# speedinghzl/DSRG

Hardware: AMD Instinct MI355X
Metric: images/sec DSRG train step (VGG16 321x321, 21-class) (higher is better)
Workload: dtype bf16 backbone (fp32 master weights) + f32/f64 supervision path

## Files before the change

### dsrg_amd/_lib.py

```python
import ctypes
import os

import torch

_HERE = os.path.dirname(os.path.abspath(__file__))
LIB_PATH = os.path.join(_HERE, os.environ.get("DSRG_LIB") or "libdsrg_hip.so")

OK, ERR_INVALID, ERR_HIP, ERR_UNSUPPORTED, ERR_NOMEM = 0, -1, -2, -3, -4


class DsrgError(RuntimeError):
    def __init__(self, code, msg):
        RuntimeError.__init__(self, "libdsrg_hip error %d: %s" % (code, msg))
        self.code = code


class CrfParams(ctypes.Structure):
    _fields_ = [("w_bilateral", ctypes.c_float), ("theta_alpha_x", ctypes.c_float),
                ("theta_alpha_y", ctypes.c_float), ("theta_beta_r", ctypes.c_float),
                ("theta_beta_g", ctypes.c_float), ("theta_beta_b", ctypes.c_float),
                ("w_gaussian", ctypes.c_float), ("theta_gamma_x", ctypes.c_float),
                ("theta_gamma_y", ctypes.c_float), ("n_iters", ctypes.c_int32)]

    @classmethod
# ... 58 lines not shown
    "dsrg_train_s_input_batch": (_i, [_i, _vp, _sz] + [ctypes.POINTER(ctypes.c_int32)] * 8 + [_i, _i, _i, _i, ctypes.POINTER(_f),
                                      _vp, _vp, _vp, _vp]),
    "dsrg_train_f_input_batch": (_i, [_i, _vp, _sz] + [ctypes.POINTER(ctypes.c_int32)] * 7 + [_i, _i, ctypes.POINTER(_f), _f, _f,
                                      _vp, _vp, _vp]),
    "dsrg_resnet_stem_packed_bytes": (_sz, []),
    "dsrg_pack_resnet_stem_f32": (_i, [_vp, _vp, _vp, _vp]),
    "dsrg_resnet_stem_bf16": (_i, [_vp, _vp, _vp, _vp, _i, _i, _i, _vp]),
    "dsrg_im2col3x3_nhwc16": (_i, [_vp, _vp, _i, _i, _i, _i, _i, _vp]),
    "dsrg_relu_bwd_bias_bf16": (_i, [_vp, _vp, _vp, _vp, _vp, _i, ctypes.c_long, _i, ctypes.c_float, _vp]),
    "dsrg_col2im3x3_nhwc_bf16": (_i, [_vp, _vp, _i, _i, _i, _i, _i, _vp]),
    "dsrg_avgpool3x3_s1_bf16": (_i, [_vp, _vp, _i, _i, _i, _i, _vp]),
    "dsrg_conv_igemm_backward_residual_bf16": (_i, [_vp] * 8 + [_i, _vp, _sz] + [_i] * 6 + [_vp]),
    "dsrg_pack_conv_weight_scaled_f32": (_i, [_vp, _vp, _vp, _vp, _i, _i, _i, _vp]),
    "dsrg_aspp_shift_sum_f32": (_i, [_vp, _vp, _vp, _vp] + [_i] * 6 + [_vp]),
    "dsrg_aspp_shift_gather_bf16": (_i, [_vp, _vp, _vp] + [_i] * 6 + [_vp]),
    "dsrg_defer_reductions": (_i, [_i]),
    "dsrg_flush_reductions": (_i, [_vp]),
    "dsrg_conv_igemm_residual_bf16": (_i, [_vp] * 6 + [_i] * 8 + [_vp]),
    "dsrg_conv_igemm_split_f32": (_i, [_vp, _vp, _vp, _vp] + [_i] * 8 + [_vp]),
    "dsrg_add_relu_bf16": (_i, [_vp, _vp, _vp, _sz, _vp]),
    "dsrg_relu_mask_bf16": (_i, [_vp, _vp, _vp, _vp, _sz, _vp]),
    "dsrg_bias_grad_bf16": (_i, [_vp, _vp, _vp, _i, ctypes.c_long, _i, _vp]),
    "dsrg_heads_forward_bf16": (_i, [_vp, _i, _vp, _vp, _vp, _i, _i, _i, _i, _vp]),
    "dsrg_conv3x3_direct_bf16": (_i, [_vp, _vp, _vp, _vp, _i, _i, _i, _i, _i, _i, _vp]),
    "dsrg_conv3x3_direct_dgrad_workspace": (_sz, [_i]),
    "dsrg_conv3x3_direct_dgrad_bf16": (_i, [_vp] * 6 + [_sz] + [_i] * 5 + [_vp]),
    "dsrg_conv_igemm_supported": (_i, [_i, _i, _i]),
    "dsrg_conv_igemm_bf16": (_i, [_vp, _vp, _vp, _vp, _vp, _i, _i, _i, _i, _i, _i, _i, _i, ctypes.c_float, ctypes.c_ulonglong, _vp, _sz,
                                  _vp]),
    "dsrg_conv_igemm_workspace": (_sz, []),
    "dsrg_conv_igemm_dgrad_workspace": (_sz, [_i] * 5),
    "dsrg_conv_igemm_dgrad_bf16": (_i, [_vp] * 6 + [_i] * 7 + [_f, _vp, _sz, _vp]),
    "dsrg_conv_igemm_workspace_status": (_i, [_vp, _vp, _vp]),
    "dsrg_pack_conv_weight_f32": (_i, [_vp, _vp, _vp, _i, _i, _i, _vp]),
    "dsrg_sgd_pack_f32": (_i, [_i] + [_vp] * 9 + [_f, _vp]),
    "dsrg_conv_igemm_wgrad_workspace": (_sz, [_i, _i, _i, _i, _i, _i, _i]),
    "dsrg_conv_igemm_wgrad_splits": (_i, [_i] * 7 + [_vp, _vp]),
    "dsrg_conv_igemm_wgrad_bf16": (_i, [_vp, _vp, _vp, _vp, _i, _vp, _sz, _i, _i, _i, _i, _i, _i, _i, _vp]),
    "dsrg_conv_igemm_backward_bf16": (_i, [_vp, _vp, _vp, _vp, _vp, _vp, _i, _vp, _f, _vp, ctypes.c_size_t, _vp, ctypes.c_size_t, _i, _i, _i, _i, _i, _i, _vp]),
    "dsrg_conv3x3_wgrad_workspace": (_sz, [_i, _i, _i, _i, _i]),
    "dsrg_conv3x3_wgrad_bf16": (_i, [_vp, _vp, _vp, _vp, _sz, _i, _i, _i, _i, _i, _vp]),
    "dsrg_conv3x3_wgrad_f32": (_i, [_vp, _vp, _vp, _vp, _sz, _i, _i, _i, _i, _i, _vp]),
    "dsrg_pack_conv_weight_direct_f32": (_i, [_vp, _vp, _vp, _i, _i, _vp]),
    "dsrg_heads_backward_chunks": (_i, [_i]),
    "dsrg_heads_backward_bf16": (_i, [_vp, _i, _vp, _vp, _vp, _sz, _vp, _vp, _i, _i, _i, _i, _vp]),
    "dsrg_heads_backward_relu_workspace": (_sz, [_i] * 3),
    "dsrg_heads_backward_relu_bf16": (_i, [_vp, _i, _vp, _vp, _vp, _sz, _vp, _vp, _f, _vp, _vp, _sz] + [_i] * 4 + [_vp]),
    "dsrg_maxpool3x3_fwd_bf16": (_i, [_vp, _vp, _vp, _i, _i, _i, _i, _i, _i, _i, _vp]),
    "dsrg_maxpool3x3_relu_fwd_bf16": (_i, [_vp, _vp, _vp, _i, _i, _i, _i, _i, _i, _i, _vp]),
    "dsrg_maxpool3x3_bwd_bf16": (_i, [_vp, _vp, _vp, _i, _i, _i, _i, _i, _i, _i, _vp]),
    "dsrg_maxpool3x3_bwd_relu_bf16": (_i, [_vp, _vp, _vp, _vp, _vp, _vp, _i, _i, _i, _i, _i, _i, _i, _vp]),
    "dsrg_supervision_step": (_i, [_vp, _i, _vp, _vp, _i, _i, _vp, _vp, _d, _d, ctypes.POINTER(CrfParams),
                                   _vp, _vp, _vp, _vp, _vp, _vp]),
}

_LIB = None


def lib():
    global _LIB
    if _LIB is None:
        if not os.path.exists(LIB_PATH):
            raise ImportError(
                "%s is missing — build it with `make -C dsrg_amd/csrc` (hipcc --offload-arch=gfx950) or "
                "`python -c 'import __graft_entry__ as g; g.build()'`.  There is no CPU fallback." % LIB_PATH)
        L = ctypes.CDLL(LIB_PATH)
        for name, (res, args) in SIGNATURES.items():
            fn = getattr(L, name)
            fn.restype = res
            fn.argtypes = args
        _LIB = L
    return _LIB


def check(rc):
    if rc != OK:
        raise DsrgError(rc, lib().dsrg_last_error().decode("utf-8", "replace"))


def require_gpu():
    if lib().dsrg_device_count() < 1:
        raise DsrgError(ERR_HIP, "no HIP device visible — the DSRG supervision kernels need an MI355X "
                                 "(gfx950); there is no CPU fallback")
```

### dsrg_amd/backbone.py

```python
import torch
import torch.nn as nn
import torch.nn.functional as F

import os as _os

from . import ops

_WGRAD_MIN_COUT = 512
_GEMM_DGRAD_MAX_MAP = 2048
_GEMM_WGRAD_MAX_MAP = 2048
_IGEMM_MIN_TILES = 64
_IGEMM = _os.environ.get("DSRG_IGEMM", "1") == "1"


def _bf16_run(x):
    return x.dtype == torch.bfloat16 or (torch.is_autocast_enabled() and torch.get_autocast_dtype("cuda") == torch.bfloat16)


def _im2col_gemm(x, weight, bias, dilation, relu, want_cols=False):
    B, C, H, W = x.shape
    cout, k = weight.shape[0], weight.shape[2]
    xn = x.permute(0, 2, 3, 1)
    if not xn.is_contiguous():
        xn = xn.contiguous()
# ... 112 lines not shown
            gw = torch.mm(g2d.t(), x2d).view(cout, x.shape[1], 1, 1)
            gemm_wgrad = True
        elif ctx.direct and g.dtype == torch.bfloat16 and x.dtype == torch.bfloat16 and \
                (x.shape[1], cout) in ((3, 64), (64, 64), (64, 128), (128, 128)):
            gw = ops.conv3x3_wgrad(x, g)
            gemm_wgrad = True
        elif gemm_wgrad:
            cin = x.shape[1]
            if cols is None or cols.dtype != g.dtype:
                cols = ops.im2col3x3_nhwc(x.permute(0, 2, 3, 1).contiguous(), ctx.dilation)
            g2d = g.permute(0, 2, 3, 1).reshape(-1, cout)
            gw = torch.mm(g2d.t(), cols).view(cout, 3, 3, cin).permute(0, 3, 1, 2)
        mask = [ctx.needs_input_grad[0] and not gemm_dgrad, not gemm_wgrad, not fused]
        gx2 = gw2 = gb2 = None
        if any(mask):
            gx2, gw2, gb2 = torch.ops.aten.convolution_backward(
                g, x, weight, None if fused else [weight.shape[0]], [1, 1], [pad, pad],
                [ctx.dilation, ctx.dilation], False, [0, 0], 1, mask)
        return (gx if gemm_dgrad else gx2), (gw if gemm_wgrad else gw2), (gb if fused else gb2), None, None, None, None, None, None, None


class _GradLink:
    __slots__ = ("scale", "gb", "ptr", "version")

    def __init__(self):
        self.scale, self.gb, self.ptr, self.version = 1.0, None, 0, -1

    def leave(self, gx, gb):
        self.gb, self.ptr, self.version = gb, gx.data_ptr(), gx._version

    def take(self, g):
        gb, self.gb = self.gb, None
        if gb is None:
            return None
        if g.data_ptr() == self.ptr and g._version == self.version:
            return gb
        if self.scale != 1.0:
            raise RuntimeError("chain_input: the output of a conv + ReLU + Dropout node declared to have one consumer has several")
        return None


_FUSE_CHAIN = _os.environ.get("DSRG_FUSE_CHAIN", "1") != "0"


def _landed(g, slot):
    return g.detach() if (slot is not None and g is slot) else g


class _IgemmConvFn(torch.autograd.Function):

    @staticmethod
    def forward(ctx, k, dils, relu, drop_p, pool, n, links_in, links_out, *t):
        xs, ws, bs = t[:n], t[n:2 * n], t[2 * n:3 * n]
        xs = [x if x.dtype == torch.bfloat16 else x.bfloat16() for x in xs]
        packs_d = [None] * n
        fb = [b.detach().float().contiguous() for b in bs]
        if drop_p > 0.0 and not relu:
            raise ValueError("_IgemmConvFn: Dropout needs the ReLU in front of it")
        fused_drop = drop_p > 0.0
        scale = 256.0 / (256 - min(255, int(drop_p * 256.0 + 0.5))) if fused_drop else 1.0
        seed = ops.dropout_seed() if fused_drop else 0
        if links_in is not None and not all(lk is not None for lk in links_in):
            links_in = None
        if k == 3:
            need_d = any(ctx.needs_input_grad[8:8 + n]) and ops.conv_igemm_supported(ws[0].shape[0], ws[0].shape[1], 3)
            packs = [ops.pack_conv_weight_pair(w, True, need_d) for w in ws]
            packs_d = [p[1] for p in packs]
            outs = ops.conv_igemm(xs, [p[0] for p in packs], fb, dils, 3, relu, drop_p, seed)
        elif fused_drop:
            packs = [ops.pack_conv_weight_pair(w, True, links_in is not None and _FUSE_CHAIN) for w in ws]
            packs_d = [p[1] for p in packs]
            outs = ops.conv_igemm(xs, [p[0] for p in packs], fb, dils, 1, relu, drop_p, seed)
        else:
            outs = [_im2col_gemm(x, w.to(torch.bfloat16), b.to(torch.bfloat16), 1, relu) for x, w, b in zip(xs, ws, bs)]
        code, pooled = None, None
        if pool is not None:
            pooled, code = ops.maxpool3x3_fwd(outs[0], pool[0], pool[1], relu_input=True)
        ctx.save_for_backward(code, *xs, *ws, *(outs if (relu and pool is None) else ()))
        ctx.out_shape = tuple(outs[0].shape)
        ctx.gw_out = [getattr(w, "_dsrg_grad_out", None) for w in ws]
        ctx.packs_d = packs_d
        ctx.dils, ctx.relu, ctx.scale, ctx.pool, ctx.n, ctx.k = dils, relu, scale, pool, n, k
        ctx.links_in = links_in
        ctx.links_out = links_out if (relu and pool is None) else None
        if ctx.links_out is not None:
            for lk in ctx.links_out:
                lk.scale, lk.gb = scale, None
        return tuple(outs) if pool is None else (pooled,)

    @staticmethod
    def backward(ctx, *gs):
        n = ctx.n
        code, saved = ctx.saved_tensors[0], ctx.saved_tensors[1:]
        xs, ws, ys = saved[:n], saved[n:2 * n], saved[2 * n:] or (None,) * n
        cout, cin = ws[0].shape[0], ws[0].shape[1]
        gms, gbs = [], []
        cl = torch.channels_last
        for i, g in enumerate(gs):
            gm, gb = g, ctx.links_out[i].take(g) if ctx.links_out is not None else None
            if gb is None:
                gm, gb = _relu_bias_backward(g, ctx.pool, code, ctx.out_shape, ctx.relu, ys[i], ctx.scale)
            gms.append(gm); gbs.append(gb)
        need_x = [ctx.needs_input_grad[8 + i] for i in range(n)]
        gxs = [None] * n
        absorb = _FUSE_CHAIN and ctx.links_in is not None and all(need_x) and ops.conv_igemm_supported(cout, cin, ctx.k) and \
            cin >= 256 and all(x.is_contiguous(memory_format=cl) for x in xs)
        if n == 1 and ctx.k == 3 and need_x[0] and ops.conv_igemm_supported(cout, cin, 3) and \
                ops.conv_igemm_wgrad_supported(cin, cout, 3) and xs[0].is_contiguous(memory_format=cl):
            pd = ctx.packs_d[0] if ctx.packs_d[0] is not None else ops.pack_conv_weight(ws[0], for_dgrad=True)
            gx, gw, gb_below = ops.conv_igemm_backward(gms[0], pd, xs[0], ctx.dils[0], xs[0] if absorb else None,
                                                       ctx.links_in[0].scale if absorb else 1.0, gw_out=ctx.gw_out[0])
            if absorb:
                ctx.links_in[0].leave(gx, gb_below)
            return (None,) * 8 + (gx, _landed(gw, ctx.gw_out[0])) + tuple(gbs)
        if absorb:
            packs_d = [p if p is not None else ops.pack_conv_weight(w, for_dgrad=True) for p, w in zip(ctx.packs_d, ws)]
            gxs, gb_below = ops.conv_igemm_dgrad(gms, packs_d, list(xs), ctx.dils, ctx.k, ctx.links_in[0].scale)
            for lk, gx_, gb_ in zip(ctx.links_in, gxs, gb_below):
                lk.leave(gx_, gb_)
        if ctx.k == 1:
            for i in range(n):
                if absorb:
                    break
                if need_x[i]:
                    g2d = gms[i].permute(0, 2, 3, 1).reshape(-1, cout)
                    B_, _, H_, W_ = xs[i].shape
                    gxs[i] = torch.mm(g2d, ws[i].to(torch.bfloat16).reshape(cout, cin)).view(B_, H_, W_, cin).permute(0, 3, 1, 2)
            gws = [_landed(gw, o) for gw, o in zip(ops.conv_igemm_wgrad(list(xs), gms, ctx.dils, 1, outs=ctx.gw_out), ctx.gw_out)]
            return (None,) * 8 + tuple(gxs) + tuple(gws) + tuple(gbs)
        if any(need_x) and not absorb:
            if ops.conv_igemm_supported(cout, cin, 3):
                packs_d = [p if p is not None else ops.pack_conv_weight(w, for_dgrad=True) for p, w in zip(ctx.packs_d, ws)]
                gxs = ops.conv_igemm(gms, packs_d, None, ctx.dils, 3, False)
            else:
                for i in range(n):
                    d = ctx.dils[i]
                    gxs[i] = torch.ops.aten.convolution_backward(gms[i], xs[i], ws[i].to(torch.bfloat16), None, [1, 1], [d, d], [d, d],
                                                                 False, [0, 0], 1, [True, False, False])[0]
        if ops.conv_igemm_wgrad_supported(cin, cout, 3):
            gws = ops.conv_igemm_wgrad(list(xs), gms, ctx.dils, 3, outs=ctx.gw_out)
            gws = [_landed(gw, o) for gw, o in zip(gws, ctx.gw_out)]
        else:
            gws = []
            for i in range(n):
                d = ctx.dils[i]
                gws.append(torch.ops.aten.convolution_backward(gms[i], xs[i], ws[i].to(torch.bfloat16), None, [1, 1], [d, d], [d, d],
                                                               False, [0, 0], 1, [False, True, False])[1].float())
        return (None,) * 8 + tuple(gx if nx else None for gx, nx in zip(gxs, need_x)) + tuple(gws) + tuple(gbs)


class _DirectConvFn(torch.autograd.Function):

    @staticmethod
    def forward(ctx, x, weight, bias, relu, pool, link_in, link_out):
        x = x if x.dtype == torch.bfloat16 else x.bfloat16()
        cl = torch.channels_last
        x = x if x.is_contiguous(memory_format=cl) else x.contiguous(memory_format=cl)
        if weight.shape[1] == 3:
            w16, wd = weight.detach().to(torch.bfloat16), None
        else:
            w16, wd = ops.pack_direct_weight_pair(weight, ctx.needs_input_grad[0])
        out = ops.conv3x3_direct(x, w16, bias.detach(), relu)
        code, pooled = None, None
        if pool is not None:
            pooled, code = ops.maxpool3x3_fwd(out, pool[0], pool[1], relu_input=True)
        ctx.save_for_backward(x, out if (relu and pool is None) else None, code)
        ctx.out_shape = tuple(out.shape)
        ctx.wd = wd
        ctx.gw_out = getattr(weight, "_dsrg_grad_out", None)
        ctx.relu, ctx.pool = relu, pool
        ctx.link_in = link_in if (link_in is not None and link_in.scale == 1.0 and wd is not None) else None
        ctx.link_out = link_out if (relu and pool is None) else None
        if ctx.link_out is not None:
            ctx.link_out.scale, ctx.link_out.gb = 1.0, None
        return out if pool is None else pooled

    @staticmethod
    def backward(ctx, g):
        x, y, code = ctx.saved_tensors
        gb = ctx.link_out.take(g) if ctx.link_out is not None else None
        if gb is None:
            g, gb = _relu_bias_backward(g, ctx.pool, code, ctx.out_shape, ctx.relu, y, 1.0)
        gx = None
        if ctx.needs_input_grad[0]:
            if _FUSE_CHAIN and ctx.link_in is not None:
                gx, gb_below = ops.conv3x3_direct_dgrad(g, ctx.wd, x)
                ctx.link_in.leave(gx, gb_below)
            else:
                gx = ops.conv3x3_direct(g, ctx.wd, None, False)
        gw = ops.conv3x3_wgrad(x, g, torch.float32, out=ctx.gw_out)
        return gx, _landed(gw, ctx.gw_out), gb, None, None, None, None


def _pool_in_node(cout):
    return cout % 8 == 0 and 256 % (cout // 8) == 0


def _direct_route(conv, x, p, pool):
    cin, cout = conv.in_channels, conv.out_channels
    if not (conv.kernel_size == (3, 3) and conv.dilation == (1, 1) and conv.groups == 1 and conv.bias is not None
            and (cin, cout) in ops.WGRAD_CONV_SHAPES and p == 0.0):
        return False
    if not _bf16_run(x):
        return False
    w = conv.weight
    if not (w.dtype == torch.float32 and conv.bias.dtype == torch.float32 and w.is_contiguous(memory_format=torch.channels_last)):
        return False
    if cin == 3 and x.requires_grad and torch.is_grad_enabled():
        return False
    return pool is None or _pool_in_node(cout)


# ... 100 lines not shown
        if _hip_pool_takes(x):
            return _AvgPool3x3Fn.apply(x)
        if x.is_cuda and x.dim() == 4 and not x.is_contiguous():
            x = x.contiguous()
        return super().forward(x)


class MaxPool3x3(nn.MaxPool2d):

    def __init__(self, stride, ceil_mode=False):
        super().__init__(3, stride, 1, ceil_mode=ceil_mode)

    def forward(self, x):
        return _pool3x3(x, self.stride, self.ceil_mode)


def _pool3x3(x, stride, ceil_mode):
    if _hip_pool_takes(x):
        return _MaxPool3x3Fn.apply(x, stride, ceil_mode)
    return F.max_pool2d(x, 3, stride, 1, ceil_mode=ceil_mode)


def _conv_relu(cin, cout, dilation=1, gemm=False, pool=None, chain=False):
    conv = GemmConv2d(cin, cout, 3, padding=dilation, dilation=dilation, fuse_relu=True, gemm=gemm, fuse_pool=pool, chain_input=chain)
    return [conv, FusedReLU()] + ([FusedPool()] if pool is not None else [])


class _HeadsFn(torch.autograd.Function):

    @staticmethod
    def forward(ctx, links, weight, bias, *xs):
        cl = torch.channels_last
        ctx.links = links if (links is not None and all(lk is not None for lk in links) and
                              all(x.is_contiguous(memory_format=cl) for x in xs)) else None
        xs = [x.contiguous(memory_format=cl) for x in xs]
        weight = weight.contiguous()
        ctx.save_for_backward(weight, *xs)
        return ops.heads_forward(xs, weight, bias.contiguous())

    @staticmethod
    def backward(ctx, g):
        weight, *xs = ctx.saved_tensors
        n, O, K = weight.shape
        if _FUSE_CHAIN and ctx.links is not None and all(ctx.needs_input_grad[3:]):
            gxs, gw, gb_below = ops.heads_backward(xs, weight, g, True, ctx.links[0].scale)
            for i, lk in enumerate(ctx.links):
                lk.leave(gxs[i], gb_below[i])
        else:
            gxs, gw = ops.heads_backward(xs, weight, g, need_gx=any(ctx.needs_input_grad[3:]))
        gb1 = g.sum((0, 2, 3))
        return (None, gw, gb1.unsqueeze(0).expand(n, O).contiguous()) + (tuple(gxs) if gxs is not None else (None,) * n)


class _StackKernels(torch.autograd.Function):

    @staticmethod
    def forward(ctx, *ws):
        ctx.layouts = [(tuple(w.shape), tuple(w.stride())) for w in ws]
        return torch.stack([w.reshape(w.shape[0], w.shape[1]) for w in ws])

    @staticmethod
    def backward(ctx, g):
        return tuple(g[i].as_strided(shape, stride) if g[i].is_contiguous() else g[i].reshape(shape)
                     for i, (shape, stride) in enumerate(ctx.layouts))


class VGG16ASPP(nn.Module):

    def __init__(self, num_classes=21, dropout=0.5, gemm_convs=True):
        super().__init__()
        L = []
        p2 = (2, True)
        L += _conv_relu(3, 64) + _conv_relu(64, 64, pool=p2, chain=True)
        L += _conv_relu(64, 128, 1, gemm_convs) + _conv_relu(128, 128, 1, gemm_convs, pool=p2, chain=True)
        L += _conv_relu(128, 256, 1, gemm_convs) + _conv_relu(256, 256, 1, gemm_convs, chain=True) + \
            _conv_relu(256, 256, 1, gemm_convs, pool=p2, chain=True)
        g = gemm_convs
        L += _conv_relu(256, 512, 1, g) + _conv_relu(512, 512, 1, g, chain=True) + _conv_relu(512, 512, 1, g, chain=True) + [MaxPool3x3(1)]
        L += _conv_relu(512, 512, 2, g) + _conv_relu(512, 512, 2, g, chain=True) + _conv_relu(512, 512, 2, g, chain=True) + [MaxPool3x3(1)]
        L += [AvgPool3x3()]
        self.features = nn.Sequential(*L)
        self.branches = nn.ModuleList()
        for d in (6, 12, 18, 24):
            g = gemm_convs
            fc8 = GemmConv2d(1024, num_classes, 1, gemm=g)
            nn.init.normal_(fc8.weight, std=0.01)
            nn.init.zeros_(fc8.bias)
            self.branches.append(nn.Sequential(
                GemmConv2d(512, 1024, 3, padding=d, dilation=d, fuse_relu=True, gemm=g, fuse_dropout=dropout), FusedReLU(),
                FusedDropout(),
                GemmConv2d(1024, 1024, 1, fuse_relu=True, gemm=g, fuse_dropout=dropout), FusedReLU(), FusedDropout(), fc8))

    def forward(self, x):
        f = self.features(x)
        hs = []
        fc6 = [br[0] for br in self.branches]
        if len(fc6) <= 4 and all(_igemm_route(m, f, len(fc6)) and m.stride == (1, 1) and m.padding == m.dilation for m in fc6):
            p = fc6[0].fuse_dropout if self.training else 0.0
            n = len(fc6)
            links = [_GradLink() for _ in range(n)] if torch.is_grad_enabled() else None
            hs = list(_IgemmConvFn.apply(3, [m.dilation[0] for m in fc6], True, p, None, n, None, links, *([f] * n),
                                         *[m.weight for m in fc6], *[m.bias for m in fc6]))
            fc7 = [br[3] for br in self.branches]
            if all(isinstance(m, GemmConv2d) and m.kernel_size == (1, 1) and m.fuse_relu and m.bias is not None and m.gemm
                   and m.in_channels % 256 == 0 and m.out_channels % 256 == 0 for m in fc7):
                p7 = fc7[0].fuse_dropout if self.training else 0.0
                links7 = [_GradLink() for _ in range(n)] if torch.is_grad_enabled() else None
                hs = list(_IgemmConvFn.apply(1, [1] * n, True, p7, None, n, links, links7, *hs, *[m.weight for m in fc7],
                                             *[m.bias for m in fc7]))
                for h, lk in zip(hs, links7 or []):
                    h._dsrg_grad_link = lk
            else:
                for i, br in enumerate(self.branches):
                    for m in list(br)[1:-1]:
                        hs[i] = m(hs[i])
        else:
            for br in self.branches:
                h = f
                for m in list(br)[:-1]:
                    h = m(h)
                hs.append(h)
        heads = [br[-1] for br in self.branches]
        if hs[0].is_cuda and hs[0].dtype == torch.bfloat16 and len(hs) <= 4 and heads[0].out_channels <= 32 \
                and heads[0].in_channels % 256 == 0:
            w = _StackKernels.apply(*[m.weight for m in heads])
            b = torch.stack([m.bias for m in heads])
            links = [getattr(h, "_dsrg_grad_link", None) for h in hs]
            return _HeadsFn.apply(links, w.float(), b.float(), *hs)
        out = None
        with torch.autocast(device_type=hs[0].device.type, enabled=False):
            for m, h in zip(heads, hs):
                s = m(h.float())
                out = s if out is None else out + s
        return out

    def caffe_param_groups(self):
        groups = {}
        for name, p in self.named_parameters():
            is_fc8 = name.startswith("branches") and name.split(".")[2] == "6"
            is_bias = name.endswith("bias")
            key = ((10.0 if is_fc8 else 1.0) * (2.0 if is_bias else 1.0), 0.0 if is_bias else 1.0)
            groups.setdefault(key, []).append(p)
        return [dict(params=ps, lr_mult=k[0], decay_mult=k[1]) for k, ps in groups.items()]


def count_flops_per_image(size=321):
    def pool(n): return -(-(n + 2 - 3) // 2) + 1
    h1 = size; h2 = pool(h1); h3 = pool(h2); h4 = pool(h3)
    macs = 0
    for (cin, cout, h, n) in [(3, 64, h1, 1), (64, 64, h1, 1), (64, 128, h2, 1), (128, 128, h2, 1),
                              (128, 256, h3, 1), (256, 256, h3, 2), (256, 512, h4, 1), (512, 512, h4, 5)]:
        macs += n * cin * cout * 9 * h * h
    macs += 4 * (512 * 1024 * 9 + 1024 * 1024 + 1024 * 21) * h4 * h4
    return 2 * macs


class GraphedForward(object):

    def __init__(self, net, example, amp_dtype=torch.bfloat16, warmup=3, capture_error_mode="global"):
        if net.training:
            raise ValueError("GraphedForward captures an eval-mode forward (dropout would replay one mask)")
        self.net, self.amp = net, amp_dtype
        self.x = example.detach().clone(memory_format=torch.preserve_format)
        warm = torch.cuda.Stream(device=example.device)
        warm.wait_stream(torch.cuda.current_stream())
        with torch.cuda.stream(warm):
            for _ in range(warmup):
                self._fwd()
        torch.cuda.current_stream().wait_stream(warm)
        torch.cuda.synchronize()
        self.graph = torch.cuda.CUDAGraph()
        with torch.cuda.graph(self.graph, capture_error_mode=capture_error_mode):
            self.out = self._fwd()

    def _fwd(self):
        with torch.no_grad(), torch.autocast("cuda", dtype=self.amp, enabled=self.amp is not None):
            return self.net(self.x).contiguous()

    def __call__(self, x=None):
        if x is not None and x.data_ptr() != self.x.data_ptr():
# ... 4 lines not shown
```

### dsrg_amd/csrc/api.hip

```cpp
#include <math.h>
#include <stdarg.h>
#include <stdio.h>
#include <string.h>
#include <mutex>
#include <new>
#include "common.h"

namespace dsrg {

static thread_local char g_err[512] = "";
int set_error(int code, const char *fmt, ...) {
    va_list ap;
    va_start(ap, fmt);
    vsnprintf(g_err, sizeof(g_err), fmt, ap);
    va_end(ap);
    return code;
}

static inline size_t align256(size_t x) { return (x + 255) & ~(size_t)255; }

}

using namespace dsrg;

// ... 522 lines not shown
    return launch_bias_grad(g, bias_grad, partials, partial_blocks, rows, C, static_cast<hipStream_t>(stream));
}
extern "C" int dsrg_heads_forward_bf16(const void *const *x_dev, int n_branches, const float *w_dev, const float *bias_dev,
                                       float *out_dev, int B, int HW, int K, int O, void *stream) {
    if (!x_dev || !w_dev || !out_dev || B < 1 || HW < 1) return set_error(DSRG_ERR_INVALID, "bad argument");
    for (int k = 0; k < n_branches && k < 4; k++)
        if (!x_dev[k]) return set_error(DSRG_ERR_INVALID, "NULL branch input");
    return launch_heads_fwd(x_dev, n_branches, w_dev, bias_dev, out_dev, B, HW, K, O, static_cast<hipStream_t>(stream));
}
extern "C" int dsrg_conv3x3_direct_bf16(const void *x_dev, const void *w_dev, const float *bias_dev, void *y_dev, int B, int H,
                                        int W, int cin, int cout, int relu, void *stream) {
    if (!x_dev || !w_dev || !y_dev || B < 1 || H < 1 || W < 1) return set_error(DSRG_ERR_INVALID, "bad argument");
    return launch_conv3x3_direct(x_dev, w_dev, bias_dev, y_dev, B, H, W, cin, cout, relu, static_cast<hipStream_t>(stream));
}
extern "C" size_t dsrg_conv3x3_direct_dgrad_workspace(int cout) { return conv3x3_direct_colsum_workspace(cout); }
extern "C" int dsrg_conv3x3_direct_dgrad_bf16(const void *g_dev, const void *w_dev, const void *mask_dev, void *gx_dev,
                                              float *bias_grad_dev, void *workspace_dev, size_t workspace_bytes, int B, int H, int W,
                                              int cin, int cout, void *stream) {
    if (!g_dev || !w_dev || !mask_dev || !gx_dev || !bias_grad_dev) return set_error(DSRG_ERR_INVALID, "NULL argument");
    return launch_conv3x3_direct(g_dev, w_dev, nullptr, gx_dev, B, H, W, cin, cout, 0, static_cast<hipStream_t>(stream), mask_dev,
                                 bias_grad_dev, workspace_dev, workspace_bytes);
}
extern "C" int dsrg_conv_igemm_supported(int cin, int cout, int ksize) { return conv_igemm_supported(cin, cout, ksize) ? 1 : 0; }
extern "C" int dsrg_conv_igemm_bf16(const void *const *x_dev, const void *const *w_dev, const float *const *bias_dev,
                                    void *const *y_dev, const int *dilation, int ngroups, int B, int H, int W, int cin, int cout,
                                    int ksize, int relu, float dropout_p, unsigned long long dropout_seed, void *workspace_dev,
                                    size_t workspace_bytes, void *stream) {
    if (!x_dev || !w_dev || !y_dev || B < 1 || H < 1 || W < 1) return set_error(DSRG_ERR_INVALID, "conv_igemm: bad arguments");
    return launch_conv_igemm(x_dev, w_dev, bias_dev, y_dev, dilation, ngroups, B, H, W, cin, cout, ksize, relu, dropout_p,
                             dropout_seed, workspace_dev, workspace_bytes, static_cast<hipStream_t>(stream));
}
extern "C" size_t dsrg_conv_igemm_dgrad_workspace(int ngroups, int B, int H, int W, int cout) {
    return conv_igemm_colsum_workspace(ngroups, B, H, W, cout);
}
extern "C" int dsrg_conv_igemm_dgrad_bf16(const void *const *g_dev, const void *const *w_dev, const void *const *mask_dev,
                                          void *const *gx_dev, float *const *bias_grad_dev, const int *dilation, int ngroups, int B,
                                          int H, int W, int cin, int cout, int ksize, float mask_scale, void *workspace_dev,
                                          size_t workspace_bytes, void *stream) {
    if (!g_dev || !w_dev || !gx_dev || !mask_dev || B < 1 || H < 1 || W < 1)
        return set_error(DSRG_ERR_INVALID, "conv_igemm_dgrad: bad arguments");
    return launch_conv_igemm(g_dev, w_dev, nullptr, gx_dev, dilation, ngroups, B, H, W, cin, cout, ksize, 0, 0.0f, 0ull, nullptr, 0,
                             static_cast<hipStream_t>(stream), mask_dev, mask_scale, bias_grad_dev, workspace_dev, workspace_bytes);
}
extern "C" size_t dsrg_conv_igemm_workspace(void) { return conv_igemm_workspace(); }
extern "C" int dsrg_conv_igemm_workspace_status(const void *workspace_dev, void *stream, int *status_host) {
    if (!workspace_dev || !status_host) return set_error(DSRG_ERR_INVALID, "bad argument");
    return conv_igemm_workspace_status(workspace_dev, static_cast<hipStream_t>(stream), status_host);
}
extern "C" int dsrg_pack_conv_weight_f32(const float *w_dev, void *fwd_dev, void *dgrad_dev, int cout, int cin, int ksize, void *stream) {
    return launch_pack_conv_weight(w_dev, fwd_dev, dgrad_dev, cout, cin, ksize, static_cast<hipStream_t>(stream));
}
namespace dsrg {
int launch_sgd_pack(int n, float *const *p, const float *const *g, float *const *buf, void *const *fwd, void *const *dg, const int *shape,
                    const long long *numel, const float *lr, const float *wd, float momentum, hipStream_t stream);
}
extern "C" int dsrg_sgd_pack_f32(int n, float *const *param_dev, const float *const *grad_dev, float *const *momentum_dev, void *const *fwd_dev,
                                 void *const *dgrad_dev, const int *shape, const long long *numel, const float *lr, const float *weight_decay,
                                 float momentum, void *stream) {
    if (n > 0 && (!param_dev || !numel || ((fwd_dev || dgrad_dev) && !shape)))
        return set_error(DSRG_ERR_INVALID, "sgd_pack: null argument");
    return launch_sgd_pack(n, param_dev, grad_dev, momentum_dev, fwd_dev, dgrad_dev, shape, numel, lr, weight_decay, momentum,
                           static_cast<hipStream_t>(stream));
}
extern "C" size_t dsrg_conv_igemm_wgrad_workspace(int ngroups, int B, int H, int W, int cin, int cout, int ksize) {
    return conv_igemm_wgrad_workspace(ngroups, B, H, W, cin, cout, ksize);
}
extern "C" int dsrg_conv_igemm_wgrad_splits(int ngroups, int B, int H, int W, int cin, int cout, int ksize, const int *dilation,
                                            int *splits_out) {
    return conv_igemm_wgrad_splits(ngroups, B, H, W, cin, cout, ksize, dilation, splits_out);
}
extern "C" int dsrg_conv_igemm_wgrad_bf16(const void *const *x_dev, const void *const *g_dev, void *const *gw_dev, const int *dilation,
                                          int ngroups, void *workspace_dev, size_t workspace_bytes, int B, int H, int W, int cin,
                                          int cout, int ksize, int out_bf16, void *stream) {
    if (!x_dev || !g_dev || !gw_dev || B < 1 || H < 1 || W < 1) return set_error(DSRG_ERR_INVALID, "conv_igemm_wgrad: bad arguments");
    return launch_conv_igemm_wgrad(x_dev, g_dev, gw_dev, dilation, ngroups, workspace_dev, workspace_bytes, B, H, W, cin, cout, ksize,
                                   out_bf16, static_cast<hipStream_t>(stream));
}
namespace dsrg {
int launch_conv_igemm_backward(const void *g, const void *wd, const void *x, const void *mask, void *gx, void *gw, int dil, float *bias_grad,
                               float mask_scale, void *colsum_ws, size_t colsum_ws_bytes, void *wgrad_ws, size_t wgrad_ws_bytes, int B, int H,
                               int W, int cin, int cout, int k, hipStream_t stream);
}
extern "C" int dsrg_conv_igemm_backward_bf16(const void *g_dev, const void *w_dgrad_dev, const void *x_dev, const void *mask_dev, void *gx_dev,
                                             float *gw_dev, int dilation, float *bias_grad_dev, float mask_scale, void *colsum_workspace_dev,
                                             size_t colsum_workspace_bytes, void *wgrad_workspace_dev, size_t wgrad_workspace_bytes, int B,
                                             int H, int W, int cin, int cout, int ksize, void *stream) {
    if (!g_dev || !w_dgrad_dev || !x_dev || !gx_dev || !gw_dev || B < 1 || H < 1 || W < 1 || (bias_grad_dev && !mask_dev))
        return set_error(DSRG_ERR_INVALID, "conv_igemm_backward: bad arguments");
    return dsrg::launch_conv_igemm_backward(g_dev, w_dgrad_dev, x_dev, mask_dev, gx_dev, gw_dev, dilation, bias_grad_dev, mask_scale,
                                            colsum_workspace_dev, colsum_workspace_bytes, wgrad_workspace_dev, wgrad_workspace_bytes, B, H,
                                            W, cin, cout, ksize, static_cast<hipStream_t>(stream));
}
extern "C" int dsrg_conv_igemm_backward_residual_bf16(const void *g_dev, const void *w_dgrad_dev, const void *x_dev, const void *mask_dev,
                                                      const void *res_dev, void *gx_dev, float *gw_dev, const float *gw_scale_dev, int dilation,
                                                      void *wgrad_workspace_dev, size_t wgrad_workspace_bytes, int B, int H, int W, int cin,
                                                      int cout, int ksize, void *stream) {
    if (!g_dev || !w_dgrad_dev || !x_dev || !gx_dev || !gw_dev || B < 1 || H < 1 || W < 1)
        return set_error(DSRG_ERR_INVALID, "conv_igemm_backward_residual: bad arguments");
    return launch_conv_igemm_backward_residual(g_dev, w_dgrad_dev, x_dev, mask_dev, res_dev, gx_dev, gw_dev, gw_scale_dev, dilation,
                                               wgrad_workspace_dev, wgrad_workspace_bytes, B, H, W, cin, cout, ksize,
                                               static_cast<hipStream_t>(stream));
}
extern "C" int dsrg_pack_conv_weight_scaled_f32(const float *w_dev, const float *scale_dev, void *fwd_dev, void *dgrad_dev, int cout, int cin,
                                                int ksize, void *stream) {
    return launch_pack_conv_weight(w_dev, fwd_dev, dgrad_dev, cout, cin, ksize, static_cast<hipStream_t>(stream), 0, scale_dev);
}
extern "C" size_t dsrg_conv3x3_wgrad_workspace(int B, int H, int W, int cin, int cout) {
    return conv3x3_wgrad_workspace(B, H, W, cin, cout);
}
extern "C" int dsrg_conv3x3_wgrad_bf16(const void *x_dev, const void *g_dev, void *gw_dev, void *workspace_dev, size_t workspace_bytes,
                                       int B, int H, int W, int cin, int cout, void *stream) {
    if (!x_dev || !g_dev || !gw_dev || !workspace_dev) return set_error(DSRG_ERR_INVALID, "bad argument");
    return launch_conv3x3_wgrad(x_dev, g_dev, gw_dev, static_cast<float *>(workspace_dev), workspace_bytes, B, H, W, cin, cout,
                                static_cast<hipStream_t>(stream));
}
extern "C" int dsrg_conv3x3_wgrad_f32(const void *x_dev, const void *g_dev, float *gw_dev, void *workspace_dev, size_t workspace_bytes,
                                      int B, int H, int W, int cin, int cout, void *stream) {
    if (!x_dev || !g_dev || !gw_dev || !workspace_dev) return set_error(DSRG_ERR_INVALID, "bad argument");
    return launch_conv3x3_wgrad(x_dev, g_dev, gw_dev, static_cast<float *>(workspace_dev), workspace_bytes, B, H, W, cin, cout,
                                static_cast<hipStream_t>(stream), 1);
}
extern "C" int dsrg_pack_conv_weight_direct_f32(const float *w_dev, void *fwd_dev, void *dgrad_dev, int cout, int cin, void *stream) {
    if ((cin != 64 && cin != 128) || (cout != 64 && cout != 128))
        return set_error(DSRG_ERR_INVALID, "pack_conv_weight_direct: 64 / 128 channels either side (got %d -> %d)", cin, cout);
    return launch_pack_conv_weight(w_dev, fwd_dev, dgrad_dev, cout, cin, 3, static_cast<hipStream_t>(stream), 1);
}
extern "C" int dsrg_heads_backward_chunks(int M) { return heads_bwd_chunks(M); }
extern "C" int dsrg_heads_backward_bf16(const void *const *x_dev, int n_branches, const float *w_dev, const float *g_dev,
                                        void *gx_dev, size_t gx_branch_stride_bytes, float *gw_dev, float *partial_dev, int B,
                                        int HW, int K, int O, void *stream) {
    if (!x_dev || !w_dev || !g_dev || (!gx_dev && !gw_dev) || (gw_dev && !partial_dev) || B < 1 || HW < 1)
        return set_error(DSRG_ERR_INVALID, "bad argument");
    for (int k = 0; k < n_branches && k < 4; k++)
        if (!x_dev[k]) return set_error(DSRG_ERR_INVALID, "NULL branch input");
    return launch_heads_bwd(x_dev, n_branches, w_dev, g_dev, gx_dev, gx_branch_stride_bytes, gw_dev, partial_dev, B, HW, K, O,
                            static_cast<hipStream_t>(stream));
}
extern "C" size_t dsrg_heads_backward_relu_workspace(int n_branches, int M, int K) { return heads_bwd_relu_workspace(n_branches, M, K); }
extern "C" int dsrg_heads_backward_relu_bf16(const void *const *x_dev, int n_branches, const float *w_dev, const float *g_dev,
                                             void *gx_dev, size_t gx_branch_stride_bytes, float *gw_dev, float *partial_dev,
                                             float relu_scale, float *bias_grad_dev, void *workspace_dev, size_t workspace_bytes,
                                             int B, int HW, int K, int O, void *stream) {
    if (!x_dev || !w_dev || !g_dev || !gx_dev || (gw_dev && !partial_dev) || B < 1 || HW < 1 || !(relu_scale > 0.0f) || !bias_grad_dev)
        return set_error(DSRG_ERR_INVALID, "bad argument");
    for (int k = 0; k < n_branches && k < 4; k++)
        if (!x_dev[k]) return set_error(DSRG_ERR_INVALID, "NULL branch input");
    return launch_heads_bwd(x_dev, n_branches, w_dev, g_dev, gx_dev, gx_branch_stride_bytes, gw_dev, partial_dev, B, HW, K, O,
                            static_cast<hipStream_t>(stream), relu_scale, bias_grad_dev, workspace_dev, workspace_bytes);
}
extern "C" int dsrg_maxpool3x3_fwd_bf16(const void *in, void *out, void *code, int B, int H, int W, int OH, int OW, int C,
                                        int stride, void *stream) {
    if (!in || !out || !code) return set_error(DSRG_ERR_INVALID, "NULL argument");
    return launch_maxpool3x3_fwd(in, out, code, B, H, W, OH, OW, C, stride, static_cast<hipStream_t>(stream));
}
extern "C" int dsrg_maxpool3x3_relu_fwd_bf16(const void *in, void *out, void *code, int B, int H, int W, int OH, int OW, int C,
                                             int stride, void *stream) {
    if (!in || !out || !code) return set_error(DSRG_ERR_INVALID, "NULL argument");
    return launch_maxpool3x3_fwd(in, out, code, B, H, W, OH, OW, C, stride, static_cast<hipStream_t>(stream), true);
}
extern "C" int dsrg_maxpool3x3_bwd_bf16(const void *gout, const void *code, void *gin, int B, int H, int W, int OH, int OW,
                                        int C, int stride, void *stream) {
    if (!gout || !code || !gin) return set_error(DSRG_ERR_INVALID, "NULL argument");
    return launch_maxpool3x3_bwd(gout, code, gin, B, H, W, OH, OW, C, stride, static_cast<hipStream_t>(stream));
}

extern "C" int dsrg_maxpool3x3_bwd_relu_bf16(const void *gout, const void *code, const void *relu_out, void *gin, float *bias_grad,
                                             float *partials, int partial_blocks, int B, int H, int W, int OH, int OW, int C,
                                             void *stream) {
    if (!gout || !code || !gin || !bias_grad || !partials) return set_error(DSRG_ERR_INVALID, "NULL argument");
    return launch_maxpool3x3_bwd_relu(gout, code, relu_out, gin, bias_grad, partials, partial_blocks, B, H, W, OH, OW, C,
                                      static_cast<hipStream_t>(stream));
}

extern "C" int dsrg_supervision_step(dsrg_ctx_t c, int B, const float *logits, const float *images, int img_h,
                                     int img_w, const float *labels, const float *cues, double th1, double th2,
                                     const dsrg_crf_params *prm, float *losses, float *grad_logits,
                                     float *probs_out, float *seeds_out, float *logq_out, void *stream) {
    if (!c || !logits || !labels || !cues || !losses || !grad_logits)
        return set_error(DSRG_ERR_INVALID, "NULL argument");
    if (B < 1 || B > c->maxB) return set_error(DSRG_ERR_INVALID, "batch %d outside 1..%d", B, c->maxB);
    const bool prepared = images == nullptr;
    {
        int prc = check_params(prm);
        if (prc) return prc;
    }
    if (!prepared && (img_h < 1 || img_w < 1)) return set_error(DSRG_ERR_INVALID, "bad image size");
    if (prepared) {
        if (c->prepared_B != B || memcmp(&c->prepared_prm, prm, offsetof(dsrg_crf_params, n_iters)) != 0)
            return set_error(DSRG_ERR_INVALID, "images_dev is NULL but dsrg_crf_prepare_batch was not called "
                                               "for this batch size / these kernel parameters");
    }
    hipStream_t s = static_cast<hipStream_t>(stream);
    const int C = c->C, N = c->N;
    const size_t nb = sizeof(float) * (size_t)B * C * N;
    const bool q0 = prm->n_iters > 0;
    int rc = launch_softmax_fwd(B, C, N, logits, c->probs, s, kMinProb, q0 ? c->mf.q : nullptr);
    if (rc) return rc;
    rc = crf_run(c, B, c->probs, colours_float(c, images, img_h, img_w), prm, nullptr, c->refined, c->logq, s, prepared, q0);
    if (prepared) c->prepared_B = 0;
    if (rc) return rc;
    rc = launch_srg(B, C, c->H, c->W, labels, cues, c->refined, th1, th2, c->seeds, c->srg_code, s);
    if (rc) return rc;
    rc = launch_sup_loss_backward(B, C, N, logits, c->probs, c->seeds, c->logq, c->refined, c->stats, grad_logits,
                                  losses, s);
    if (rc) return rc;
    if (probs_out) DSRG_HIP_CHECK(hipMemcpyAsync(probs_out, c->probs, nb, hipMemcpyDeviceToDevice, s));
    if (seeds_out) DSRG_HIP_CHECK(hipMemcpyAsync(seeds_out, c->seeds, nb, hipMemcpyDeviceToDevice, s));
    if (logq_out) DSRG_HIP_CHECK(hipMemcpyAsync(logq_out, c->logq, nb, hipMemcpyDeviceToDevice, s));
    return DSRG_OK;
}

namespace dsrg {
struct LargeCrf;
int large_crf_create(int W, int H, int C, LargeCrf **out, int nimages);
void large_crf_destroy(LargeCrf *c);
int large_crf_set_unary(LargeCrf *c, const float *unary_host);
int large_crf_zero_unary(LargeCrf *c);
int large_crf_set_image(LargeCrf *c, const unsigned char *im_host);
int large_crf_infer(LargeCrf *c, const dsrg_crf_params *prm, int n_iters);
int large_crf_read_q(LargeCrf *c, float *out_host);
int large_crf_read_map(LargeCrf *c, int32_t *labels_host);
int large_crf_read_map_select(LargeCrf *c, const CrfSelArgs &sel, int32_t *labels_host);
int large_crf_lattice_size(LargeCrf *c, int k);
Profiler *large_crf_profiler(LargeCrf *c);
void large_crf_set_stream(LargeCrf *c, hipStream_t s, bool async);
}

struct dsrg_crf_s {
    int W, H, M;
    int nimg;
    bool forced_large;
    dsrg::LargeCrf *large;
    dsrg_ctx_t ctx;
    float *neg_unary;
    float *q;
    float *stage;
    unsigned char *im;
    int32_t *lab;
    bool have_unary, have_pairwise;
    dsrg_crf_params prm;
    hipStream_t stream;
    bool async;
};

static constexpr int kCrfCacheSlots = 4;
static dsrg_crf_s *g_crf_cache[kCrfCacheSlots] = {nullptr, nullptr, nullptr, nullptr};
static std::mutex g_crf_cache_mutex;

static int crf_create(int W, int H, int nlabels, int nimages, dsrg_crf_t *out);
extern "C" int dsrg_crf_create(int W, int H, int nlabels, dsrg_crf_t *out) { return crf_create(W, H, nlabels, 1, out); }
extern "C" int dsrg_crf_create_batch(int W, int H, int nlabels, int nimages, dsrg_crf_t *out) {
    if (nimages < 1) return set_error(DSRG_ERR_INVALID, "bad CRF batch");
    return crf_create(W, H, nlabels, nimages == 1 ? -1 : nimages, out);
}
static int crf_create(int W, int H, int nlabels, int nimages, dsrg_crf_t *out) {
    const bool force_large = nimages != 1;
    if (nimages < 0) nimages = 1;
// ... 192 lines not shown
```

### dsrg_amd/csrc/backbone_ops.hip

```cpp
#include "common.h"
#include <algorithm>
#include <cstring>

namespace dsrg {

__device__ __forceinline__ float bf16_lo(uint32_t w) { return __uint_as_float(w << 16); }
__device__ __forceinline__ float bf16_hi(uint32_t w) { return __uint_as_float(w & 0xffff0000u); }
__device__ __forceinline__ uint32_t f32_to_bf16_rne(float f) {
    uint32_t u = __float_as_uint(f);
    if ((u & 0x7fffffffu) > 0x7f800000u) return (u >> 16) | 0x40u;
    return (u + 0x7fffu + ((u >> 16) & 1u)) >> 16;
}
__device__ __forceinline__ uint32_t pack_bf16(float lo, float hi) { return f32_to_bf16_rne(lo) | (f32_to_bf16_rne(hi) << 16); }

constexpr int kRbThreads = 256;

__global__ __launch_bounds__(kRbThreads) void relu_bwd_bias_kernel(const uint4 *__restrict__ g, const uint4 *__restrict__ y,
                                                                    uint4 *__restrict__ gm, float *__restrict__ part,
                                                                    int rows, int C8, int rows_per_block, float scale) {
    __shared__ float red[kRbThreads][9];
    const int lanes_r = kRbThreads / C8;
    const int cg = threadIdx.x % C8, rl = threadIdx.x / C8;
    float acc[8] = {0.f, 0.f, 0.f, 0.f, 0.f, 0.f, 0.f, 0.f};
    if (rl < lanes_r) {
// ... 510 lines not shown
    DSRG_LAUNCH_CHECK();
    return DSRG_OK;
}

int launch_maxpool3x3_bwd_relu(const void *gout, const void *code, const void *y, void *gin, float *bias_grad, float *part,
                                int part_blocks, int B, int H, int W, int OH, int OW, int C, hipStream_t stream) {
    int rc = pool_check(B, H, W, OH, OW, C, 2);
    if (rc) return rc;
    const int C8 = C / 8;
    if (kRbThreads % C8 != 0) return set_error(DSRG_ERR_UNSUPPORTED, "maxpool3x3_bwd_relu: channels / 8 must divide %d", kRbThreads);
    if (part_blocks < 1) return set_error(DSRG_ERR_INVALID, "maxpool3x3_bwd_relu: no partial-sum blocks");
    const size_t total = (size_t)B * ((H + 1) / 2) * ((W + 1) / 2) * C8;
    size_t ipb = (total + part_blocks - 1) / part_blocks;
    ipb = (ipb + kRbThreads - 1) / kRbThreads * kRbThreads;
    const int nblk = (int)((total + ipb - 1) / ipb);
    if (y)
        hipLaunchKernelGGL(maxpool3x3_s2_bwd_relu_kernel<true>, dim3(nblk), dim3(kRbThreads), 0, stream, (const uint4 *)gout,
                           (const uint2 *)code, (const uint4 *)y, (uint4 *)gin, part, B, H, W, OH, OW, C8, ipb);
    else
        hipLaunchKernelGGL(maxpool3x3_s2_bwd_relu_kernel<false>, dim3(nblk), dim3(kRbThreads), 0, stream, (const uint4 *)gout,
                           (const uint2 *)code, (const uint4 *)nullptr, (uint4 *)gin, part, B, H, W, OH, OW, C8, ipb);
    DSRG_LAUNCH_CHECK();
    if (!defer_reduction(1, part, bias_grad, nblk, C))
        hipLaunchKernelGGL(bias_finalize_kernel, dim3((C + 31) / 32), dim3(256), 0, stream, part, bias_grad, nblk, C);
    DSRG_LAUNCH_CHECK();
    return DSRG_OK;
}

int launch_maxpool3x3_bwd(const void *gout, const void *code, void *gin, int B, int H, int W, int OH, int OW, int C,
                          int stride, hipStream_t stream) {
    int rc = pool_check(B, H, W, OH, OW, C, stride);
    if (rc) return rc;
    if (stride == 2) {
        const size_t blocks2 = (size_t)B * ((H + 1) / 2) * ((W + 1) / 2) * (C / 8);
        hipLaunchKernelGGL(maxpool3x3_s2_bwd_kernel, dim3((unsigned)((blocks2 + 255) / 256)), dim3(256), 0, stream,
                           (const uint4 *)gout, (const uint2 *)code, (uint4 *)gin, B, H, W, OH, OW, C / 8);
        DSRG_LAUNCH_CHECK();
        return DSRG_OK;
    }
    const size_t total = (size_t)B * H * W * (C / 8);
    hipLaunchKernelGGL(maxpool3x3_bwd_kernel, dim3((unsigned)((total + 255) / 256)), dim3(256), 0, stream, (const uint4 *)gout,
                       (const uint2 *)code, (uint4 *)gin, B, H, W, OH, OW, C / 8, stride);
    DSRG_LAUNCH_CHECK();
    return DSRG_OK;
}



namespace {
typedef float f32x16 __attribute__((ext_vector_type(16)));
constexpr int kHeadOutPad = 32;
struct HeadArgs {
    const uint16_t *x[4];
    const float *w;
    const float *bias;
    float *out;
    int nbr, M, K, O, HW;
};
__device__ __forceinline__ void bf16x8_to_f32(const uint4 &v, float (&f)[8]) {
    f[0] = bf16_lo(v.x); f[1] = bf16_hi(v.x); f[2] = bf16_lo(v.y); f[3] = bf16_hi(v.y);
    f[4] = bf16_lo(v.z); f[5] = bf16_hi(v.z); f[6] = bf16_lo(v.w); f[7] = bf16_hi(v.w);
}
}

struct HeadMask {
    const uint16_t *y[4];
    float *part;
    float scale;
    int tiles;
};
template <bool MASK>
__global__ __launch_bounds__(256) void heads_bwd_dx_kernel(const float *__restrict__ g, const float *__restrict__ w,
                                                           uint4 *__restrict__ gx, int M, int K, int O, int HW, size_t branch_stride,
                                                           HeadMask hm) {
    __shared__ __attribute__((aligned(16))) float gs[32][16];
    __shared__ __attribute__((aligned(16))) float cs_l[MASK ? 128 : 1][8];
    const int k = blockIdx.y, t = threadIdx.x;
    const int K8 = K / 8, T = MASK ? hm.tiles : 1;
    uint4 *dst = reinterpret_cast<uint4 *>(reinterpret_cast<unsigned char *>(gx) + (size_t)k * branch_stride);
    for (int cg0 = 0; cg0 < K8; cg0 += 128) {
        const int cg = cg0 + (t & 127), rh = t >> 7;
        const bool live = cg < K8;
        float cs[8] = {0, 0, 0, 0, 0, 0, 0, 0};
        for (int ti = 0; ti < T; ti++) {
            const int m0 = (blockIdx.x * T + ti) * 16;
            if (m0 >= M) break;
            if (MASK || cg0 > 0) __syncthreads();
            for (int e = t; e < 32 * 16; e += 256) {
                const int o = e >> 4, r = e & 15, m = m0 + r;
                float v = 0.0f;
                if (o < O && m < M) { const int b = m / HW, hw = m - b * HW; v = g[((size_t)b * O + o) * HW + hw]; }
                gs[o][r] = v;
            }
            __syncthreads();
            if (!live) continue;
            float acc[8][8];
#pragma unroll
            for (int r = 0; r < 8; r++)
#pragma unroll
                for (int c = 0; c < 8; c++) acc[r][c] = 0.0f;
            const float *wk = w + (size_t)k * O * K + (size_t)cg * 8;
#pragma unroll 7
            for (int o = 0; o < O; o++) {
                const float4 w0 = *reinterpret_cast<const float4 *>(wk + (size_t)o * K), w1 = *reinterpret_cast<const float4 *>(wk + (size_t)o * K + 4);
                const float4 g0 = *reinterpret_cast<const float4 *>(&gs[o][rh * 8]), g1 = *reinterpret_cast<const float4 *>(&gs[o][rh * 8 + 4]);
                const float wf[8] = {w0.x, w0.y, w0.z, w0.w, w1.x, w1.y, w1.z, w1.w};
                const float gf[8] = {g0.x, g0.y, g0.z, g0.w, g1.x, g1.y, g1.z, g1.w};
#pragma unroll
                for (int r = 0; r < 8; r++)
#pragma unroll
                    for (int c = 0; c < 8; c++) acc[r][c] = __builtin_fmaf(gf[r], wf[c], acc[r][c]);
            }
            uint4 yk[4];
#pragma unroll
            for (int r = 0; r < 8; r++) {
                const int m = m0 + rh * 8 + r;
                if (MASK && (r & 3) == 0) {
#pragma unroll
                    for (int r2 = 0; r2 < 4; r2++) {
                        const int m2 = m + r2;
                        yk[r2] = m2 < M ? *reinterpret_cast<const uint4 *>(hm.y[k] + (size_t)m2 * K + (size_t)cg * 8) : make_uint4(0, 0, 0, 0);
                    }
                }
                uint32_t o4[4];
#pragma unroll
                for (int e = 0; e < 4; e++) {
                    if (MASK) {
                        const uint4 yr = yk[r & 3];
                        const uint32_t y = e == 0 ? yr.x : e == 1 ? yr.y : e == 2 ? yr.z : yr.w;
                        const uint32_t keep = ((int16_t)(y & 0xffffu) > 0 ? 0x0000ffffu : 0u) | ((int32_t)y >= 0x10000 ? 0xffff0000u : 0u);
                        o4[e] = pack_bf16(acc[r][2 * e] * hm.scale, acc[r][2 * e + 1] * hm.scale) & keep;
                        cs[2 * e] += __uint_as_float(o4[e] << 16);
                        cs[2 * e + 1] += __uint_as_float(o4[e] & 0xffff0000u);
                    } else {
                        o4[e] = pack_bf16(acc[r][2 * e], acc[r][2 * e + 1]);
                    }
                }
                if (m < M) dst[(size_t)m * K8 + cg] = make_uint4(o4[0], o4[1], o4[2], o4[3]);
            }
        }
        if (MASK) {
            __syncthreads();
            if (rh == 1 && live) {
                *reinterpret_cast<float4 *>(&cs_l[t & 127][0]) = make_float4(cs[0], cs[1], cs[2], cs[3]);
                *reinterpret_cast<float4 *>(&cs_l[t & 127][4]) = make_float4(cs[4], cs[5], cs[6], cs[7]);
            }
            __syncthreads();
            if (rh == 0 && live) {
                float *p = hm.part + ((size_t)k * gridDim.x + blockIdx.x) * K + (size_t)cg * 8;
                const float4 a0 = *reinterpret_cast<const float4 *>(&cs_l[t][0]), a1 = *reinterpret_cast<const float4 *>(&cs_l[t][4]);
                *reinterpret_cast<float4 *>(p) = make_float4(cs[0] + a0.x, cs[1] + a0.y, cs[2] + a0.z, cs[3] + a0.w);
                *reinterpret_cast<float4 *>(p + 4) = make_float4(cs[4] + a1.x, cs[5] + a1.y, cs[6] + a1.z, cs[7] + a1.w);
            }
        }
    }
}

template <int O, bool MASK>
__global__ __launch_bounds__(256) void heads_bwd_dx_rows_kernel(const float *__restrict__ g, const float *__restrict__ w,
                                                                unsigned char *__restrict__ gx, int M, int K, int HW, size_t branch_stride,
                                                                HeadMask hm, int rows_per_wg) {
    constexpr int OP = (O + 3) & ~3;
    extern __shared__ __attribute__((aligned(16))) float gs_rows[];
    const int k = blockIdx.y, t = threadIdx.x;
    const int c = blockIdx.z * 1024 + 4 * t;
    const int r0 = blockIdx.x * rows_per_wg, r1 = min(M, r0 + rows_per_wg), nr = r1 - r0;
    for (int e = t; e < nr * OP; e += 256) {
        const int o = e / nr, r = e - o * nr, m = r0 + r;
        float v = 0.0f;
        if (o < O) { const int b = m / HW, hw = m - b * HW; v = g[((size_t)b * O + o) * HW + hw]; }
        gs_rows[r * OP + o] = v;
    }
    float wr[O][4];
#pragma unroll
    for (int o = 0; o < O; o++) {
        const float4 v = *reinterpret_cast<const float4 *>(w + ((size_t)k * O + o) * K + c);
        wr[o][0] = v.x; wr[o][1] = v.y; wr[o][2] = v.z; wr[o][3] = v.w;
    }
    __syncthreads();
    unsigned char *dst = gx + (size_t)k * branch_stride;
    const uint16_t *yk = MASK ? hm.y[k] : nullptr;
    float cs[4] = {0.0f, 0.0f, 0.0f, 0.0f};
    constexpr int R = 4;
    uint2 yn[R];
    auto fetch_masks = [&](int r) {
#pragma unroll
        for (int j = 0; j < R; j++) yn[j] = r + j < nr ? *reinterpret_cast<const uint2 *>(yk + (size_t)(r0 + r + j) * K + c) : make_uint2(0u, 0u);
    };
    if (MASK) fetch_masks(0);
    for (int r = 0; r < nr; r += R) {
        uint2 y[R];
        if (MASK) {
#pragma unroll
            for (int j = 0; j < R; j++) y[j] = yn[j];
            if (r + R < nr) fetch_masks(r + R);
        }
        float acc[R][4];
#pragma unroll
        for (int j = 0; j < R; j++) {
            const float *gr = gs_rows + min(r + j, nr - 1) * OP;
            float gv[OP];
#pragma unroll
            for (int q = 0; q < OP / 4; q++) {
                const float4 v = *reinterpret_cast<const float4 *>(gr + 4 * q);
                gv[4 * q] = v.x; gv[4 * q + 1] = v.y; gv[4 * q + 2] = v.z; gv[4 * q + 3] = v.w;
            }
#pragma unroll
            for (int e = 0; e < 4; e++) acc[j][e] = 0.0f;
#pragma unroll
            for (int o = 0; o < O; o++)
#pragma unroll
                for (int e = 0; e < 4; e++) acc[j][e] = __builtin_fmaf(gv[o], wr[o][e], acc[j][e]);
        }
#pragma unroll
        for (int j = 0; j < R; j++) {
            uint32_t o2[2];
#pragma unroll
            for (int e = 0; e < 2; e++) {
                if (MASK) {
                    const uint32_t yy = e == 0 ? y[j].x : y[j].y;
                    const uint32_t keep = ((int16_t)(yy & 0xffffu) > 0 ? 0x0000ffffu : 0u) | ((int32_t)yy >= 0x10000 ? 0xffff0000u : 0u);
                    o2[e] = pack_bf16(acc[j][2 * e] * hm.scale, acc[j][2 * e + 1] * hm.scale) & keep;
                    cs[2 * e] += __uint_as_float(o2[e] << 16);
                    cs[2 * e + 1] += __uint_as_float(o2[e] & 0xffff0000u);
                } else {
                    o2[e] = pack_bf16(acc[j][2 * e], acc[j][2 * e + 1]);
                }
            }
            if (r + j < nr) *reinterpret_cast<uint2 *>(dst + ((size_t)(r0 + r + j) * K + c) * 2) = make_uint2(o2[0], o2[1]);
// ... 19 lines not shown
        const int q = q0 + wave;
        const bool live = q < nq;
        const uint16_t *xq = a.x[k] + (size_t)(live ? q : 0) * 256 + j * 8;
        for (int mb = mbeg; mb < mend; mb += kDwRows) {
            __syncthreads();
            for (int e = threadIdx.x; e < kDwRows * 32; e += 256) {
                const int o = e / kDwRows, r = e % kDwRows, m = mb + r;
                float v = 0.0f;
                if (o < a.O && m < mend) { const int b = m / a.HW, hw = m - b * a.HW; v = g[((size_t)b * a.O + o) * a.HW + hw]; }
                gs[r][o] = v;
            }
            __syncthreads();
            if (live) {
                constexpr int G = 8;
                uint4 xv[G];
                auto fetch = [&](int r2base) {
#pragma unroll
                    for (int u = 0; u < G; u++) {
                        const int m = min(mb + r2base + 2 * u + half, mend - 1);
                        xv[u] = *reinterpret_cast<const uint4 *>(xq + (size_t)m * a.K);
                    }
                };
                fetch(0);
                for (int r2 = 0; r2 < kDwRows; r2 += 2 * G) {
                    float xf[G][8], gv[G];
#pragma unroll
                    for (int u = 0; u < G; u++) {
                        bf16x8_to_f32(xv[u], xf[u]);
                        gv[u] = gs[r2 + 2 * u + half][j];
                    }
                    if (r2 + 2 * G < kDwRows) fetch(r2 + 2 * G);
#pragma unroll
                    for (int u = 0; u < G; u++)
#pragma unroll
                        for (int t = 0; t < 8; t++) acc[t] = __builtin_amdgcn_mfma_f32_32x32x2f32(gv[u], xf[u][t], acc[t], 0, 0, 0);
                }
            }
        }
        float *pp = partial + (((size_t)rc * a.nbr + k) * a.O) * a.K + (size_t)(live ? q : 0) * 256 + j * 8;
#pragma unroll
        for (int r = 0; r < 16; r++) {
            const int o = (r & 3) + 8 * (r >> 2) + 4 * half;
            if (live && o < a.O) {
                *reinterpret_cast<float4 *>(pp + (size_t)o * a.K) = make_float4(acc[0][r], acc[1][r], acc[2][r], acc[3][r]);
                *reinterpret_cast<float4 *>(pp + (size_t)o * a.K + 4) = make_float4(acc[4][r], acc[5][r], acc[6][r], acc[7][r]);
            }
        }
#pragma unroll
        for (int t = 0; t < 8; t++)
#pragma unroll
            for (int r = 0; r < 16; r++) acc[t][r] = 0.0f;
    }
}
__global__ void heads_bwd_dw_reduce_kernel(const float *__restrict__ partial, float *__restrict__ gw, int nchunks, size_t n) {
    const size_t i = (size_t)blockIdx.x * blockDim.x + threadIdx.x;
    if (i >= n) return;
    float s = 0.0f;
    for (int c = 0; c < nchunks; c++) s += partial[(size_t)c * n + i];
    gw[i] = s;
}

namespace {
typedef __attribute__((ext_vector_type(8))) __bf16 hbf16x8;
typedef __attribute__((ext_vector_type(2))) __bf16 hbf16x2;
typedef __attribute__((ext_vector_type(2))) float hf32x2;
typedef __attribute__((__vector_size__(4 * sizeof(__bf16)))) __bf16 hbf16x4v;
#define DSRG_LDS_AS __attribute__((address_space(3)))
__device__ __forceinline__ uint32_t cvt_pk_bf16(float lo, float hi) {
    hf32x2 v = {lo, hi};
    hbf16x2 b = __builtin_convertvector(v, hbf16x2);
    return *reinterpret_cast<uint32_t *>(&b);
}
__device__ __forceinline__ void split3(const float (&f)[8], hbf16x8 &t0, hbf16x8 &t1, hbf16x8 &t2) {
    uint32_t p0[4], p1[4], p2[4];
#pragma unroll
    for (int i = 0; i < 4; i++) {
        float a = f[2 * i], b = f[2 * i + 1];
        p0[i] = cvt_pk_bf16(a, b);
        a -= bf16_lo(p0[i]); b -= bf16_hi(p0[i]);
        p1[i] = cvt_pk_bf16(a, b);
        a -= bf16_lo(p1[i]); b -= bf16_hi(p1[i]);
        p2[i] = cvt_pk_bf16(a, b);
    }
    uint4 q0 = make_uint4(p0[0], p0[1], p0[2], p0[3]), q1 = make_uint4(p1[0], p1[1], p1[2], p1[3]), q2 = make_uint4(p2[0], p2[1], p2[2], p2[3]);
    t0 = *reinterpret_cast<hbf16x8 *>(&q0); t1 = *reinterpret_cast<hbf16x8 *>(&q1); t2 = *reinterpret_cast<hbf16x8 *>(&q2);
}
__device__ __forceinline__ hbf16x8 tr_frag16(DSRG_LDS_AS unsigned char *p, int stride4) {
    hbf16x4v lo = __builtin_amdgcn_ds_read_tr16_b64_v4bf16(reinterpret_cast<DSRG_LDS_AS hbf16x4v *>(p));
    hbf16x4v hi = __builtin_amdgcn_ds_read_tr16_b64_v4bf16(reinterpret_cast<DSRG_LDS_AS hbf16x4v *>(p + stride4));
    return __builtin_shufflevector(lo, hi, 0, 1, 2, 3, 4, 5, 6, 7);
}
}

template <int R>
__global__ __launch_bounds__(256) void heads_fwd_split_kernel(HeadArgs a) {
    __shared__ float part[R][4][16][64];
    const int lane = threadIdx.x & 63, wave = threadIdx.x >> 6;
    const int m0 = blockIdx.x * (32 * R);
    const int row = lane & 31, half = lane >> 5;
    f32x16 acc[R][3];
#pragma unroll
    for (int t = 0; t < R; t++)
#pragma unroll
        for (int q = 0; q < 3; q++)
#pragma unroll
            for (int r = 0; r < 16; r++) acc[t][q][r] = 0.0f;
    if (wave < a.nbr) {
        const uint16_t *xp[R];
#pragma unroll
        for (int t = 0; t < R; t++) xp[t] = a.x[wave] + (size_t)min(m0 + 32 * t + row, a.M - 1) * a.K + half * 8;
        const float *wp = a.w + ((size_t)wave * a.O + min(row, a.O - 1)) * a.K + half * 8;
        constexpr int G = 4;
        uint4 xv[G][R];
        float4 wv[G][2];
#pragma unroll
        for (int u = 0; u < G; u++) {
#pragma unroll
            for (int t = 0; t < R; t++) xv[u][t] = *reinterpret_cast<const uint4 *>(xp[t] + u * 16);
            wv[u][0] = *reinterpret_cast<const float4 *>(wp + u * 16);
            wv[u][1] = *reinterpret_cast<const float4 *>(wp + u * 16 + 4);
        }
        for (int kb = 0; kb < a.K; kb += 16 * G) {
#pragma unroll
            for (int u = 0; u < G; u++) {
                hbf16x8 xa[R];
#pragma unroll
                for (int t = 0; t < R; t++) xa[t] = *reinterpret_cast<hbf16x8 *>(&xv[u][t]);
                const float wf[8] = {wv[u][0].x, wv[u][0].y, wv[u][0].z, wv[u][0].w, wv[u][1].x, wv[u][1].y, wv[u][1].z, wv[u][1].w};
                const int kn = kb + 16 * G + u * 16;
                if (kn < a.K) {
#pragma unroll
                    for (int t = 0; t < R; t++) xv[u][t] = *reinterpret_cast<const uint4 *>(xp[t] + kn);
                    wv[u][0] = *reinterpret_cast<const float4 *>(wp + kn);
                    wv[u][1] = *reinterpret_cast<const float4 *>(wp + kn + 4);
                }
                hbf16x8 w0, w1, w2;
                split3(wf, w0, w1, w2);
#pragma unroll
                for (int t = 0; t < R; t++) {
                    acc[t][0] = __builtin_amdgcn_mfma_f32_32x32x16_bf16(xa[t], w0, acc[t][0], 0, 0, 0);
                    acc[t][1] = __builtin_amdgcn_mfma_f32_32x32x16_bf16(xa[t], w1, acc[t][1], 0, 0, 0);
                    acc[t][2] = __builtin_amdgcn_mfma_f32_32x32x16_bf16(xa[t], w2, acc[t][2], 0, 0, 0);
                }
            }
        }
    }
#pragma unroll
    for (int t = 0; t < R; t++)
#pragma unroll
        for (int r = 0; r < 16; r++) part[t][wave][r][lane] = acc[t][0][r] + (acc[t][1][r] + acc[t][2][r]);
    __syncthreads();
    const int col = threadIdx.x >> 3, r4 = (threadIdx.x & 7) * 4;
    if (col < a.O) {
#pragma unroll
        for (int t = 0; t < R; t++)
#pragma unroll
            for (int q = 0; q < 4; q++) {
                const int rr = r4 + q, m = m0 + 32 * t + rr;
                if (m >= a.M) break;
                const int hf = (rr >> 2) & 1, reg = (rr & 3) + 4 * (rr >> 3), ln = col + 32 * hf;
                float s = 0.0f;
                for (int k = 0; k < a.nbr; k++) {
                    const float sk = part[t][k][reg][ln] + (a.bias ? a.bias[k * a.O + col] : 0.0f);
                    s = k == 0 ? sk : s + sk;
                }
                const int b = m / a.HW, hw = m - b * a.HW;
                a.out[((size_t)b * a.O + col) * a.HW + hw] = s;
            }
    }
}

constexpr int kDwRows2 = 32, kDwGPitch = 36;
__global__ __launch_bounds__(256, 2) void heads_bwd_dw_split_kernel(HeadArgs a, const float *__restrict__ g, float *__restrict__ partial,
                                                                 int rows_per_chunk) {
    extern __shared__ __attribute__((aligned(16))) unsigned char dw_lds[];
    const int xstride = a.K * 2 + 64, K8 = a.K / 8;
    unsigned char *xt = dw_lds;
    float *gs = reinterpret_cast<float *>(dw_lds + kDwRows2 * xstride);
    const int lane = threadIdx.x & 63, wave = threadIdx.x >> 6, k = blockIdx.y, rc = blockIdx.x;
    const int mbeg = rc * rows_per_chunk, mend = min(a.M, mbeg + rows_per_chunk);
    const int i16 = lane & 15, gq = lane >> 4;
    const int rowsel = (gq >> 1) * 8 + (i16 >> 2), colsel = (gq & 1) * 16 + 4 * (i16 & 3);
    const int nq = a.K / 256;
    const uint16_t *xk = a.x[k];
    for (int q0 = 0; q0 < nq; q0 += 4) {
        const int q = q0 + wave;
        const bool live = q < nq;
        f32x16 acc[8];
#pragma unroll
        for (int t = 0; t < 8; t++)
#pragma unroll
            for (int r = 0; r < 16; r++) acc[t][r] = 0.0f;
        DSRG_LDS_AS unsigned char *xb = (DSRG_LDS_AS unsigned char *)xt + rowsel * xstride + ((live ? q : 0) * 256 + colsel) * 2;
        for (int mb = mbeg; mb < mend; mb += kDwRows2) {
            __syncthreads();
            for (int e = threadIdx.x; e < kDwRows2 * 32; e += 256) {
                const int o = e / kDwRows2, r = e % kDwRows2, m = mb + r;
                float v = 0.0f;
                if (o < a.O && m < mend) { const int b = m / a.HW, hw = m - b * a.HW; v = g[((size_t)b * a.O + o) * a.HW + hw]; }
                gs[o * kDwGPitch + r] = v;
            }
#pragma unroll 8
            for (int v = threadIdx.x; v < kDwRows2 * K8; v += 256) {
                const int r = v / K8, cg = v - r * K8, m = min(mb + r, mend - 1);
                *reinterpret_cast<uint4 *>(xt + r * xstride + cg * 16) = *reinterpret_cast<const uint4 *>(xk + (size_t)m * a.K + cg * 8);
            }
            __syncthreads();
            if (live) {
#pragma unroll
                for (int s2 = 0; s2 < kDwRows2 / 16; s2++) {
                    const float *gp = gs + (lane & 31) * kDwGPitch + s2 * 16 + (lane >> 5) * 8;
                    const float4 g0 = *reinterpret_cast<const float4 *>(gp), g1 = *reinterpret_cast<const float4 *>(gp + 4);
                    const float gf[8] = {g0.x, g0.y, g0.z, g0.w, g1.x, g1.y, g1.z, g1.w};
                    hbf16x8 a0, a1, a2, bx[8];
                    split3(gf, a0, a1, a2);
#pragma unroll
                    for (int t = 0; t < 8; t++) bx[t] = tr_frag16(xb + s2 * 16 * xstride + t * 64, 4 * xstride);
#pragma unroll
                    for (int t = 0; t < 8; t++) acc[t] = __builtin_amdgcn_mfma_f32_32x32x16_bf16(a0, bx[t], acc[t], 0, 0, 0);
#pragma unroll
                    for (int t = 0; t < 8; t++) acc[t] = __builtin_amdgcn_mfma_f32_32x32x16_bf16(a1, bx[t], acc[t], 0, 0, 0);
#pragma unroll
                    for (int t = 0; t < 8; t++) acc[t] = __builtin_amdgcn_mfma_f32_32x32x16_bf16(a2, bx[t], acc[t], 0, 0, 0);
                }
            }
        }
        if (live) {
            float *pp = partial + (((size_t)rc * a.nbr + k) * a.O) * a.K + (size_t)q * 256 + (lane & 31);
#pragma unroll
            for (int t = 0; t < 8; t++)
#pragma unroll
                for (int r = 0; r < 16; r++) {
                    const int o = (r & 3) + 8 * (r >> 2) + 4 * (lane >> 5);
                    if (o < a.O) pp[(size_t)o * a.K + t * 32] = acc[t][r];
                }
        }
    }
}

static int heads_check(int nbr, int K, int O) {
    if (nbr < 1 || nbr > 4 || O < 1 || O > kHeadOutPad || K < 256 || K % 256 != 0)
        return set_error(DSRG_ERR_UNSUPPORTED, "heads: 1..4 branches, <= %d outputs, K a multiple of 256", kHeadOutPad);
    return DSRG_OK;
}

int launch_heads_fwd(const void *const *x, int nbr, const float *w, const float *bias, float *out, int B, int HW, int K, int O,
                     hipStream_t stream) {
    int rc = heads_check(nbr, K, O);
    if (rc) return rc;
    HeadArgs a;
    for (int k = 0; k < 4; k++) a.x[k] = static_cast<const uint16_t *>(x[k < nbr ? k : 0]);
    a.w = w; a.bias = bias; a.out = out; a.nbr = nbr; a.M = B * HW; a.K = K; a.O = O; a.HW = HW;
    hipLaunchKernelGGL(heads_fwd_split_kernel<2>, dim3((a.M + 63) / 64), dim3(256), 0, stream, a);
    DSRG_LAUNCH_CHECK();
    return DSRG_OK;
}

int heads_bwd_chunks(int M) { int c = (M + 255) / 256; return c < 1 ? 1 : (c > 128 ? 128 : c); }

constexpr int kHeadMaskTiles = 8;
constexpr int kHeadStripRows = 64;
static bool head_strips(int K, int O) { return O == 21 && K % 1024 == 0; }
size_t heads_bwd_relu_workspace(int nbr, int M, int K) {
    const size_t rows = std::max((size_t)((M + 16 * kHeadMaskTiles - 1) / (16 * kHeadMaskTiles)), (size_t)((M + kHeadStripRows - 1) / kHeadStripRows));
    return (size_t)nbr * rows * (size_t)K * sizeof(float);
}

int launch_heads_bwd(const void *const *x, int nbr, const float *w, const float *g, void *gx, size_t gx_branch_stride,
                     float *gw, float *partial, int B, int HW, int K, int O, hipStream_t stream, float relu_scale, float *bias_grad,
                     void *colsum_ws, size_t colsum_ws_bytes) {
    int rc = heads_check(nbr, K, O);
    if (rc) return rc;
    const int M = B * HW;
    if (gx && relu_scale > 0.0f) {
        HeadMask hm;
        for (int k = 0; k < 4; k++) hm.y[k] = static_cast<const uint16_t *>(x[k < nbr ? k : 0]);
        hm.tiles = kHeadMaskTiles; hm.scale = relu_scale;
        const int nblk = (M + 16 * kHeadMaskTiles - 1) / (16 * kHeadMaskTiles);
        if (!bias_grad || !colsum_ws || colsum_ws_bytes < heads_bwd_relu_workspace(nbr, M, K))
            return set_error(DSRG_ERR_INVALID, "heads backward: bias gradient / scratch of the absorbed ReLU missing or too small");
        hm.part = static_cast<float *>(colsum_ws);
        int nblk_s = nblk;
        if (head_strips(K, O)) {
            nblk_s = (M + kHeadStripRows - 1) / kHeadStripRows;
            hipLaunchKernelGGL((heads_bwd_dx_rows_kernel<21, true>), dim3(nblk_s, nbr, K / 1024), dim3(256),
                               (size_t)kHeadStripRows * 24 * sizeof(float), stream, g, w, static_cast<unsigned char *>(gx), M, K, HW,
                               gx_branch_stride, hm, kHeadStripRows);
        } else {
            hipLaunchKernelGGL(heads_bwd_dx_kernel<true>, dim3(nblk, nbr), dim3(256), 0, stream, g, w, static_cast<uint4 *>(gx), M, K, O, HW,
                               gx_branch_stride, hm);
        }
        DSRG_LAUNCH_CHECK();
        const float *parts[4];
        float *outs[4];
        for (int k = 0; k < nbr; k++) { parts[k] = hm.part + (size_t)k * nblk_s * K; outs[k] = bias_grad + (size_t)k * K; }
        if (int rc2 = launch_igemm_colsum(parts, outs, nbr, nblk_s, K, stream)) return rc2;
    } else if (gx) {
        HeadMask hm;
        memset(&hm, 0, sizeof(hm));
        if (head_strips(K, O))
            hipLaunchKernelGGL((heads_bwd_dx_rows_kernel<21, false>), dim3((M + kHeadStripRows - 1) / kHeadStripRows, nbr, K / 1024),
                               dim3(256), (size_t)kHeadStripRows * 24 * sizeof(float), stream, g, w, static_cast<unsigned char *>(gx), M, K, HW,
                               gx_branch_stride, hm, kHeadStripRows);
        else
            hipLaunchKernelGGL(heads_bwd_dx_kernel<false>, dim3((M + 15) / 16, nbr), dim3(256), 0, stream, g, w, static_cast<uint4 *>(gx), M,
                               K, O, HW, gx_branch_stride, hm);
        DSRG_LAUNCH_CHECK();
    }
    if (gw) {
        HeadArgs a;
        for (int k = 0; k < 4; k++) a.x[k] = static_cast<const uint16_t *>(x[k < nbr ? k : 0]);
        a.w = w; a.bias = nullptr; a.out = nullptr; a.nbr = nbr; a.M = M; a.K = K; a.O = O; a.HW = HW;
        const int nch = heads_bwd_chunks(M), rows = ((M + nch - 1) / nch + 1) & ~1;
        const size_t lds = (size_t)kDwRows2 * (K * 2 + 64) + 32 * kDwGPitch * sizeof(float);
        if (lds > 160 * 1024) {
            hipLaunchKernelGGL(heads_bwd_dw_kernel, dim3(nch, nbr), dim3(256), 0, stream, a, g, partial, rows);
        } else {
            static LdsGrant grant;
            if (int rc2 = ensure_dynamic_lds(reinterpret_cast<const void *>(&heads_bwd_dw_split_kernel), lds, grant)) return rc2;
            hipLaunchKernelGGL(heads_bwd_dw_split_kernel, dim3(nch, nbr), dim3(256), lds, stream, a, g, partial, rows);
        }
        DSRG_LAUNCH_CHECK();
        const size_t n = (size_t)nbr * O * K;
        hipLaunchKernelGGL(heads_bwd_dw_reduce_kernel, dim3((unsigned)((n + 255) / 256)), dim3(256), 0, stream, partial, gw, nch, n);
        DSRG_LAUNCH_CHECK();
    }
    return DSRG_OK;
}

}
```

### dsrg_amd/csrc/common.h

```cpp
#pragma once
#include <hip/hip_runtime.h>
#include <stdint.h>
#include <stddef.h>
#include <atomic>
#include "../../include/dsrg_hip.h"

namespace dsrg {

int set_error(int code, const char *fmt, ...);
#define DSRG_HIP_CHECK(expr)                                                              \
    do {                                                                                  \
        hipError_t _e = (expr);                                                           \
        if (_e != hipSuccess)                                                             \
            return ::dsrg::set_error(DSRG_ERR_HIP, "%s failed: %s (%s:%d)", #expr,        \
                                     hipGetErrorString(_e), __FILE__, __LINE__);          \
    } while (0)
#define DSRG_LAUNCH_CHECK() DSRG_HIP_CHECK(hipGetLastError())

__device__ __forceinline__ void colsum_block(const float *__restrict__ p, float *__restrict__ out, int rows, int cout, int bx, float (*red)[64]) {
    const int cl = threadIdx.x & 63, c = bx * 64 + cl, q = threadIdx.x >> 6;
    float s0 = 0.0f, s1 = 0.0f;
    int r = q;
    for (; r + 16 < rows; r += 32) {
        s0 += p[(size_t)r * cout + c];
// ... 118 lines not shown
    const unsigned char *im_u8 = nullptr;
    const float *images = nullptr;
    int Hi = 0, Wi = 0;
    unsigned char *im_out = nullptr;
};

struct LatticeFeat {
    float sx, sy, sr, sg, sb;
    float scale[5];
    int W, H;
};

size_t lattice_bytes(int d, int N, int nlat);
void lattice_carve(LatticeView &L, void *base, int d, int N, int nlat);
void lattice_feat_init(LatticeFeat &F, int d, int W, int H, float sx, float sy, float sr, float sg, float sb);

int launch_lattice_build(const LatticeView &L, const LatticeFeat &F, const LatticeColours &col, int nlat,
                         hipStream_t stream);
bool lattice_supported(int d, int N);

struct MeanfieldBufs {
    float *q;
    float *msg_g;
    float *msg_b;
};
constexpr int kLatticeLocal = 16;
struct Profiler {
    hipEvent_t *start, *stop;
    int cap, used;
    bool active;
};
int launch_meanfield(const LatticeView &Lg, const LatticeView &Lb, const MeanfieldBufs &buf, int B, int C,
                     const float *neg_unary, float wg, float wb, int n_iters, float *q_out,
                     double *refined_out, float *logq_out, bool gauss_local, hipStream_t stream, Profiler *prof = nullptr,
                     bool q0_ready = false);
int filter_plan_query(const LatticeView &Lg, const LatticeView &Lb, const MeanfieldBufs &buf, int B, int C, bool gauss_local,
                      int out[4]);
int launch_lattice_norm_pass(const LatticeView &L, int nlat, hipStream_t stream);
int launch_filter_once(const LatticeView &Lg, const LatticeView &Lb, const MeanfieldBufs &buf, int B, int C, int kind,
                       const float *q_in, float *out, bool gauss_local, hipStream_t stream);

int launch_clip_min(float *p, size_t n, hipStream_t stream);

int launch_softmax_fwd(int B, int C, int HW, const float *x, float *p, hipStream_t stream, float floor_at = 0.0f,
                       float *q0 = nullptr);
int launch_softmax_bwd(int B, int C, int HW, const float *x, const float *g, float *dx, hipStream_t stream);
int launch_crf_bwd(size_t n, const double *refined, const float *td, float *bd, hipStream_t stream);
int launch_seed_loss(int B, int C, int HW, const float *p, const float *S, float *loss, float *grad,
                     hipStream_t stream);
int launch_constrain_loss(int B, int C, int HW, const float *p, const float *lq, float *loss, float *gp,
                          float *glq, hipStream_t stream);
int launch_sup_loss_backward(int B, int C, int HW, const float *logits, const float *probs, const float *seeds,
                             const float *logq, const double *refined, double *stats, float *grad_logits,
                             float *losses, hipStream_t stream);
int launch_lf_to_planes(int N, int M, const float *in, float *out, int negate, hipStream_t stream);
int launch_planes_to_lf(int N, int M, const float *in, float *out, hipStream_t stream);
int launch_argmax_planes(int N, int M, const float *q, int32_t *lab, hipStream_t stream);
int launch_select_planes(int N, int M, const float *q, int32_t *lab, const CrfSelArgs &sel, hipStream_t stream);
int launch_train_gt_unary_batch(int G, int C, const float *scores, int h, int w, const int32_t *H, const int32_t *W, float eps,
                                const int32_t *select, const int32_t *nselect, int select_stride, float ignore_below,
                                float *workspace, float *const *unary, float *const *probs, int32_t *const *labels,
                                hipStream_t stream);
int launch_seed_loss_plain(int B, int C, int HW, const float *p, const float *S, float *loss, float *grad, hipStream_t stream);
int launch_expand_loss(int B, int C, int HW, const float *p, const float *stat, double q_fg, double q_bg, float *loss,
                       float *grad, double *terms, hipStream_t stream);
int launch_confusion(size_t n, const unsigned char *gt, const unsigned char *pred, int nclass, int rule_lt,
                     unsigned long long *hist, hipStream_t stream);
int launch_multiscale_unary(int K, int C, const float *const *scores, const int32_t *h, const int32_t *w, int H, int W, float eps,
                            float *unary, int32_t *amax, float *sum_out, hipStream_t stream);
int launch_multiscale_unary_batch(int G, int K, int C, const float *const *scores, const int32_t *h, const int32_t *w,
                                  const int32_t *H, const int32_t *W, float eps, float *const *unary, int32_t *const *amax,
                                  float *const *sum_out, hipStream_t stream);
int launch_preprocess_ms_batch(int G, int Gcap, int K, const unsigned char *const *images, const int32_t *H, const int32_t *W,
                               const int32_t *sizes, const float *mean, float *const *out, hipStream_t stream);
int launch_train_s_input_batch(int B, const unsigned char *stage, size_t stage_bytes, const int32_t *image_off, const int32_t *H,
                               const int32_t *W, const int32_t *cue_off, const int32_t *ncues, const int32_t *label_off,
                               const int32_t *nlabels, const int32_t *mirror, int S, int C, int Hm, int Wm, const float *mean,
                               float *images, float *cues, float *labels, hipStream_t stream);
int launch_train_f_input_batch(int B, const unsigned char *stage, size_t stage_bytes, const int32_t *image_off, const int32_t *label_off,
                               const int32_t *H, const int32_t *W, const int32_t *top, const int32_t *left, const int32_t *mirror,
                               int ch, int cw, const float *mean, float scale, float ignore_label, float *data, float *label,
                               hipStream_t stream);
size_t resnet_stem_packed_bytes();
int launch_pack_resnet_stem(const float *w, const float *scale, void *packed, hipStream_t stream);
int launch_resnet_stem(const float *x, const void *packed, const float *shift, void *y, int B, int H, int W, hipStream_t stream);
int launch_im2col3x3(const void *in, void *out, int B, int H, int W, int C, int dil, hipStream_t stream);
int launch_col2im3x3(const void *cols, void *out, int B, int H, int W, int C, int dil, hipStream_t stream);
int launch_relu_bwd_bias(const void *g, const void *y, void *gm, float *bias_grad, float *part, int part_blocks,
                         long rows, int C, float scale, hipStream_t stream);
int launch_avgpool3x3_s1(const void *in, void *out, int B, int H, int W, int C, hipStream_t stream);
int launch_bias_grad(const void *g, float *bias_grad, float *part, int part_blocks, long rows, int C, hipStream_t stream);
int launch_heads_fwd(const void *const *x, int nbr, const float *w, const float *bias, float *out, int B, int HW, int K, int O,
                     hipStream_t stream);
bool conv3x3_direct_supported(int cin, int cout);
size_t conv3x3_wgrad_workspace(int B, int H, int W, int cin, int cout);
int launch_conv3x3_wgrad(const void *x, const void *g, void *gw, float *workspace, size_t workspace_bytes, int B, int H, int W,
                         int cin, int cout, hipStream_t stream, int out_f32 = 0);
int launch_conv3x3_direct(const void *x, const void *w, const float *bias, void *y, int B, int H, int W, int cin, int cout,
                          int relu, hipStream_t stream, const void *mask = nullptr, float *colsum = nullptr,
                          void *colsum_ws = nullptr, size_t colsum_ws_bytes = 0);
size_t conv3x3_direct_colsum_workspace(int cout);
bool conv_igemm_supported(int cin, int cout, int k);
int launch_conv_igemm_residual(const void *x, const void *w, const float *bias, const void *res, const void *mask, void *y, int dil, int B,
                               int H, int W, int cin, int cout, int k, int relu, hipStream_t stream);
int launch_conv_igemm_split(const void *x3, const void *w, const float *bias, float *y, int dil, int B, int H, int W, int cin, int cout, int k,
                            int relu, hipStream_t stream);
int launch_conv_igemm(const void *const *x, const void *const *w, const float *const *bias, void *const *y, const int *dil,
                      int ngroups, int B, int H, int W, int cin, int cout, int k, int relu, float drop_p, unsigned long long seed,
                      void *workspace, size_t workspace_bytes, hipStream_t stream, const void *const *mask = nullptr,
                      float out_scale = 1.0f, float *const *colsum = nullptr, void *colsum_ws = nullptr, size_t colsum_ws_bytes = 0);
size_t conv_igemm_colsum_workspace(int ngroups, int B, int H, int W, int cout);
size_t conv_igemm_workspace();
int conv_igemm_workspace_status(const void *workspace, hipStream_t stream, int *status);
size_t conv_igemm_wgrad_workspace(int ngroups, int B, int H, int W, int cin, int cout, int k);
int conv_igemm_wgrad_splits(int ngroups, int B, int H, int W, int cin, int cout, int k, const int *dil, int *splits);
int launch_conv_igemm_wgrad(const void *const *x, const void *const *g, void *const *gw, const int *dil, int ngroups, void *workspace,
                            size_t workspace_bytes, int B, int H, int W, int cin, int cout, int k, int out_bf16, hipStream_t stream);
int launch_pack_conv_weight(const float *w, void *fwd, void *dgrad, int cout, int cin, int k, hipStream_t stream, int plain = 0,
                            const float *scale = nullptr);
int launch_conv_igemm_backward_residual(const void *g, const void *wd, const void *x, const void *mask, const void *res, void *gx, void *gw,
                                        const float *gw_scale, int dil, void *wgrad_ws, size_t wgrad_ws_bytes, int B, int H, int W, int cin,
                                        int cout, int k, hipStream_t stream);
int heads_bwd_chunks(int M);
int launch_heads_bwd(const void *const *x, int nbr, const float *w, const float *g, void *gx, size_t gx_branch_stride,
                     float *gw, float *partial, int B, int HW, int K, int O, hipStream_t stream, float relu_scale = 0.0f,
                     float *bias_grad = nullptr, void *colsum_ws = nullptr, size_t colsum_ws_bytes = 0);
size_t heads_bwd_relu_workspace(int nbr, int M, int K);
int launch_add_relu(const void *a, const void *b, void *y, size_t n, hipStream_t stream);
int launch_aspp_shift_sum(const void *yp, const float *bias, float *out, const int *offsets, int J, int O, int CT, int B, int H, int W,
                          hipStream_t stream);
int launch_aspp_shift_gather(const float *g, void *gp, const int *offsets, int J, int O, int CT, int B, int H, int W, hipStream_t stream);
int launch_relu_mask(const void *g, const void *g2, const void *y, void *gm, size_t n, hipStream_t stream);
int launch_igemm_colsum(const float *const *parts, float *const *outs, int ngroups, int rows, int cout, hipStream_t stream);
int launch_maxpool3x3_bwd_relu(const void *gout, const void *code, const void *y, void *gin, float *bias_grad, float *part,
                                int part_blocks, int B, int H, int W, int OH, int OW, int C, hipStream_t stream);
int launch_maxpool3x3_fwd(const void *in, void *out, void *code, int B, int H, int W, int OH, int OW, int C, int stride,
                          hipStream_t stream, bool relu_in = false);
int launch_maxpool3x3_bwd(const void *gout, const void *code, void *gin, int B, int H, int W, int OH, int OW, int C,
                          int stride, hipStream_t stream);

#ifdef __HIPCC__
__device__ __forceinline__ float exp_cr(float x) { return (float)exp((double)x); }

using rsrc_t = decltype(__builtin_amdgcn_make_buffer_rsrc((void *)nullptr, (short)0, 0, 0));
__device__ __forceinline__ rsrc_t make_rsrc(const void *p, size_t bytes) {
    const uint64_t a = reinterpret_cast<uint64_t>(p);
    const uint32_t lo = __builtin_amdgcn_readfirstlane((uint32_t)a);
    const uint32_t hi = __builtin_amdgcn_readfirstlane((uint32_t)(a >> 32));
    const uint32_t nb = __builtin_amdgcn_readfirstlane((uint32_t)bytes);
    void *q = reinterpret_cast<void *>(((uint64_t)hi << 32) | lo);
    return __builtin_amdgcn_make_buffer_rsrc(q, (short)0, (int)nb, 0x00020000);
}
__device__ __forceinline__ uint32_t ld_u32(rsrc_t r, uint32_t voff, uint32_t soff = 0) {
    return __builtin_amdgcn_raw_buffer_load_b32(r, voff, soff, 0);
}
__device__ __forceinline__ float ld_f32(rsrc_t r, uint32_t voff, uint32_t soff = 0) {
    return __uint_as_float(__builtin_amdgcn_raw_buffer_load_b32(r, voff, soff, 0));
}
__device__ __forceinline__ uint32_t ld_u16(rsrc_t r, uint32_t voff, uint32_t soff = 0) {
    return (uint32_t)__builtin_amdgcn_raw_buffer_load_b16(r, voff, soff, 0);
}
template <int U>
__device__ __forceinline__ void stage16_to_lds(unsigned char *dst, const void *src, uint32_t nbytes, int tid) {
    using v4 = decltype(__builtin_amdgcn_raw_buffer_load_b128(rsrc_t(), 0, 0, 0));
    const rsrc_t r = make_rsrc(src, nbytes);
    for (uint32_t base = 0; base < nbytes; base += 1024u * 16u * U) {
        v4 x[U];
#pragma unroll
        for (int u = 0; u < U; u++) x[u] = __builtin_amdgcn_raw_buffer_load_b128(r, (uint32_t)tid * 16u, base + (uint32_t)u * (1024u * 16u), 0);
#pragma unroll
        for (int u = 0; u < U; u++) {
            const uint32_t off = base + (uint32_t)u * (1024u * 16u) + (uint32_t)tid * 16u;
            if (off < nbytes) *reinterpret_cast<v4 *>(dst + off) = x[u];
        }
    }
}

#endif

int launch_srg(int B, int C, int H, int W, const float *labels, const float *cues, const double *refined,
// ... 4 lines not shown
```

### dsrg_amd/csrc/layers.hip

```cpp
#include <math.h>
#include "common.h"

namespace dsrg {

__global__ void clip_min_kernel(float *__restrict__ p, size_t n) {
    size_t i = (size_t)blockIdx.x * blockDim.x + threadIdx.x;
    const size_t stride = (size_t)gridDim.x * blockDim.x;
    for (; i < n; i += stride) {
        const float v = p[i];
        if (v < kMinProb) p[i] = kMinProb;
    }
}
int launch_clip_min(float *p, size_t n, hipStream_t stream) {
    const int threads = 256;
    const int blocks = (int)((n + threads - 1) / threads < 2048 ? (n + threads - 1) / threads : 2048);
    hipLaunchKernelGGL(clip_min_kernel, dim3(blocks > 0 ? blocks : 1), dim3(threads), 0, stream, p, n);
    DSRG_LAUNCH_CHECK();
    return DSRG_OK;
}

constexpr int kSmParts = 4, kSmPix = 64;
template <int CT>
__global__ __launch_bounds__(kSmParts * kSmPix) void softmax_fwd_kernel(int B, int C, int HW, const float *__restrict__ x,
                                                                         float *__restrict__ p, float floor_at,
// ... 266 lines not shown
        size_t blocks = (n + 255) / 256;
        if (blocks > 2048) blocks = 2048;
        hipLaunchKernelGGL(constrain_bwd_kernel, dim3((unsigned)blocks), dim3(256), 0, stream, n, (float)inv, p, lq,
                           gp, glq);
        DSRG_LAUNCH_CHECK();
    }
    return DSRG_OK;
}

constexpr int kStatSplit = 8;
__global__ __launch_bounds__(1024) void sup_stats_kernel(int C, int HW, const float *__restrict__ probs,
                                                         const float *__restrict__ seeds,
                                                         const float *__restrict__ logq,
                                                         double *__restrict__ stats ) {
    __shared__ double scratch[5 * 16];
    const int b = blockIdx.x / kStatSplit, part = blockIdx.x % kStatSplit;
    const float *pb = probs + (size_t)b * C * HW, *Sb = seeds + (size_t)b * C * HW, *lb = logq + (size_t)b * C * HW;
    double st[5] = {0, 0, 0, 0, 0};
    const int n = C * HW;
    constexpr int U = 5;
    for (int i0 = part * 1024 * U + threadIdx.x; i0 < n; i0 += kStatSplit * 1024 * U) {
        float s[U], p[U], q[U];
#pragma unroll
        for (int u = 0; u < U; u++) {
            const int i = min(i0 + u * 1024, n - 1);
            s[u] = Sb[i]; p[u] = pb[i]; q[u] = lb[i];
        }
#pragma unroll
        for (int u = 0; u < U; u++) {
            const int i = i0 + u * 1024;
            if (i < n) {
                if (s[u] != 0.0f) {
                    const double t = (double)s[u] * (double)logf(p[u]);
                    if (i < HW) { st[0] += s[u]; st[2] += t; } else { st[1] += s[u]; st[3] += t; }
                }
                float dp, dlq;
                st[4] += (double)constrain_term(p[u], q[u], dp, dlq);
            }
        }
    }
    block_reduce_sum<5>(st, scratch);
    if (threadIdx.x == 0)
        for (int k = 0; k < 5; k++) stats[((size_t)b * kStatSplit + part) * 5 + k] = st[k];
}
constexpr int kGradParts = 4, kGradPix = 64;
template <int CT>
__global__ __launch_bounds__(kGradParts * kGradPix) void sup_grad_kernel(int B, int C, int HW, const float *__restrict__ logits,
                                                       const float *__restrict__ probs,
                                                       const float *__restrict__ seeds,
                                                       const float *__restrict__ logq,
                                                       const double *__restrict__ refined,
                                                       const double *__restrict__ stats,
                                                       float *__restrict__ grad_logits,
                                                       float *__restrict__ losses) {
    constexpr int P = kGradParts, LPP = (CT + P - 1) / P;
    const int lane = threadIdx.x & 63, part = threadIdx.x & (P - 1), lane0 = lane & ~(P - 1);
    const int idx = blockIdx.x * kGradPix + (int)(threadIdx.x / P);
    const bool live = idx < B * HW;
    const int b = live ? idx / HW : 0, i = live ? idx - b * HW : 0;
    const size_t base = (size_t)b * C * HW + i;
    float s[LPP], pv[LPP], lq[LPP], sd[LPP];
    double rf[LPP];
#pragma unroll
    for (int t = 0; t < LPP; t++) {
        const size_t o = base + (size_t)min(part + t * P, C - 1) * HW;
        s[t] = logits[o]; pv[t] = probs[o]; lq[t] = logq[o]; sd[t] = seeds[o]; rf[t] = refined[o];
    }
    double cnt_bg = 0.0, cnt_fg = 0.0;
    for (int sp = 0; sp < kStatSplit; sp++) {
        cnt_bg += stats[((size_t)b * kStatSplit + sp) * 5 + 0];
        cnt_fg += stats[((size_t)b * kStatSplit + sp) * 5 + 1];
    }
    if (blockIdx.x == 0) {
        __shared__ double term_s[kGradParts * kGradPix], term_c[kGradParts * kGradPix];
        double ls = 0.0, lc = 0.0;
        for (int b0 = 0; b0 < B; b0 += kGradParts * kGradPix) {
            const int bb = b0 + (int)threadIdx.x;
            if (bb < B) {
                double st[5] = {0, 0, 0, 0, 0};
                for (int sp = 0; sp < kStatSplit; sp++)
                    for (int k = 0; k < 5; k++) st[k] += stats[((size_t)bb * kStatSplit + sp) * 5 + k];
                const double dbg = st[0] > 1e-4 ? st[0] : 1e-4, dfg = st[1] > 1e-4 ? st[1] : 1e-4;
                term_s[threadIdx.x] = -(st[2] / dbg) / B - (st[3] / dfg) / B;
                term_c[threadIdx.x] = st[4];
            }
            __syncthreads();
            if (threadIdx.x == 0)
                for (int k = 0; k < min(kGradParts * kGradPix, B - b0); k++) { ls += term_s[k]; lc += term_c[k]; }
            __syncthreads();
        }
        if (threadIdx.x == 0) {
            losses[0] = (float)ls;
            losses[1] = (float)(lc / ((double)B * (double)HW));
        }
    }
    const float dbg = (float)(cnt_bg > 1e-4 ? cnt_bg : 1e-4), dfg = (float)(cnt_fg > 1e-4 ? cnt_fg : 1e-4);
    const float inv = (float)(1.0 / ((double)B * (double)HW));
    float mx = -INFINITY;
#pragma unroll
    for (int t = 0; t < LPP; t++) { s[t] = (part + t * P < C) ? s[t] : -INFINITY; mx = fmaxf(mx, s[t]); }
#pragma unroll
    for (int m = 1; m < P; m <<= 1) mx = fmaxf(mx, __shfl_xor(mx, m, 64));
    float g[LPP];
#pragma unroll
    for (int t = 0; t < LPP; t++) {
        const int c = part + t * P;
        s[t] = exp_cr(s[t] - mx);
        float dp, dlq;
        constrain_term(pv[t], lq[t], dp, dlq);
        const float gseed = -sd[t] / (pv[t] * (c == 0 ? dbg : dfg) * (float)B);
        const float gcrf = (float)((1.0 - rf[t]) * (double)(dlq * inv));
        g[t] = gseed + dp * inv + gcrf;
    }
    float z = 0.0f;
#pragma unroll
    for (int t = 0; t < LPP; t++)
#pragma unroll
        for (int q = 0; q < P; q++) {
            const float e = __shfl(s[t], lane0 + q, 64);
            if (t * P + q < C) z = z + e;
        }
    float Z = 0.0f, sg = 0.0f;
#pragma unroll
    for (int t = 0; t < LPP; t++) s[t] = s[t] / z;
#pragma unroll
    for (int t = 0; t < LPP; t++)
#pragma unroll
        for (int q = 0; q < P; q++) {
            const float sv = __shfl(s[t], lane0 + q, 64), pr = __shfl(s[t] * g[t], lane0 + q, 64);
            if (t * P + q < C) { Z += sv + kMinProb; sg += pr; }
        }
    if (!live) return;
#pragma unroll
    for (int t = 0; t < LPP; t++) {
        const int c = part + t * P;
        if (c < C) grad_logits[base + (size_t)c * HW] = s[t] * (g[t] - sg) / Z;
    }
}
int launch_sup_loss_backward(int B, int C, int HW, const float *logits, const float *probs, const float *seeds,
                             const float *logq, const double *refined, double *stats, float *grad_logits,
                             float *losses, hipStream_t stream) {
    if (C < 1 || C > kMaxLabels) return set_error(DSRG_ERR_UNSUPPORTED, "1 <= C <= %d required", kMaxLabels);
    hipLaunchKernelGGL(sup_stats_kernel, dim3(B * kStatSplit), dim3(1024), 0, stream, C, HW, probs, seeds, logq, stats);
    DSRG_LAUNCH_CHECK();
    const int threads = kGradParts * kGradPix, blocks = (B * HW + kGradPix - 1) / kGradPix;
    if (C <= 21)
        hipLaunchKernelGGL(sup_grad_kernel<21>, dim3(blocks), dim3(threads), 0, stream, B, C, HW, logits, probs, seeds,
                           logq, refined, stats, grad_logits, losses);
    else
        hipLaunchKernelGGL(sup_grad_kernel<kMaxLabels>, dim3(blocks), dim3(threads), 0, stream, B, C, HW, logits,
                           probs, seeds, logq, refined, stats, grad_logits, losses);
    DSRG_LAUNCH_CHECK();
    return DSRG_OK;
}

__global__ void lf_to_planes_kernel(int N, int M, const float *__restrict__ in, float *__restrict__ out, int negate) {
    const int idx = blockIdx.x * blockDim.x + threadIdx.x;
    if (idx >= N * M) return;
    const int c = idx / N, i = idx - c * N;
    const float v = in[(size_t)i * M + c];
    out[idx] = negate ? -v : v;
}
__global__ void planes_to_lf_kernel(int N, int M, const float *__restrict__ in, float *__restrict__ out) {
    const int idx = blockIdx.x * blockDim.x + threadIdx.x;
    if (idx >= N * M) return;
    const int i = idx / M, c = idx - i * M;
    out[idx] = in[(size_t)c * N + i];
}
__global__ void argmax_planes_kernel(int N, int M, const float *__restrict__ q, int32_t *__restrict__ lab) {
    const int i = blockIdx.x * blockDim.x + threadIdx.x;
    if (i >= N) return;
    int m = 0;
    float best = q[i];
    for (int c = 1; c < M; c++) {
        const float v = q[(size_t)c * N + i];
        if (v > best) { best = v; m = c; }
    }
    lab[i] = m;
}
__global__ void select_planes_kernel(int N, int M, const float *__restrict__ q, int32_t *__restrict__ lab, CrfSelArgs s) {
    const int i = blockIdx.x * blockDim.x + threadIdx.x;
    if (i >= N) return;
    int m = select_label(q + i, (size_t)N, s.sel[0], s.n[0]);
    if (s.ignore_below > 0.0f && max_label_value(q + i, (size_t)N, M) < s.ignore_below) m = kIgnoreLabel;
    lab[i] = m;
}
int launch_lf_to_planes(int N, int M, const float *in, float *out, int negate, hipStream_t stream) {
    hipLaunchKernelGGL(lf_to_planes_kernel, dim3((N * M + 255) / 256), dim3(256), 0, stream, N, M, in, out, negate);
    DSRG_LAUNCH_CHECK();
    return DSRG_OK;
}
int launch_planes_to_lf(int N, int M, const float *in, float *out, hipStream_t stream) {
    hipLaunchKernelGGL(planes_to_lf_kernel, dim3((N * M + 255) / 256), dim3(256), 0, stream, N, M, in, out);
    DSRG_LAUNCH_CHECK();
    return DSRG_OK;
}
int launch_argmax_planes(int N, int M, const float *q, int32_t *lab, hipStream_t stream) {
    hipLaunchKernelGGL(argmax_planes_kernel, dim3((N + 255) / 256), dim3(256), 0, stream, N, M, q, lab);
    DSRG_LAUNCH_CHECK();
    return DSRG_OK;
}
int launch_select_planes(int N, int M, const float *q, int32_t *lab, const CrfSelArgs &sel, hipStream_t stream) {
    hipLaunchKernelGGL(select_planes_kernel, dim3((N + 255) / 256), dim3(256), 0, stream, N, M, q, lab, sel);
    DSRG_LAUNCH_CHECK();
// ... 79 lines not shown
```

### dsrg_amd/csrc/sgd_pack.hip

```cpp
#include "common.h"
#include <cstring>

namespace dsrg {
namespace {
typedef __attribute__((ext_vector_type(2))) __bf16 bf16x2_t;
typedef __attribute__((ext_vector_type(2))) float f32x2_t;
__device__ __forceinline__ uint32_t pack2_bf16(float lo, float hi) {
    f32x2_t v = {lo, hi};
    bf16x2_t b = __builtin_convertvector(v, bf16x2_t);
    return *reinterpret_cast<uint32_t *>(&b);
}

constexpr int kSgdTensors = 16;
struct SgdTensor {
    float *p;
    const float *g;
    float *buf;
    uint16_t *fwd, *dg;
    uint32_t n;
    uint32_t cout, cin, taps;
    uint32_t first_block;
    float lr, wd;
    int plain;
    int g_split;
};
struct SgdArgs {
    SgdTensor t[kSgdTensors];
    int n;
    float momentum;
};

__device__ __forceinline__ float4 sgd4(float4 w, float4 g, float4 &b, float m, float lr, float wd) {
    float4 d = make_float4(g.x + wd * w.x, g.y + wd * w.y, g.z + wd * w.z, g.w + wd * w.w);
    b = make_float4(m * b.x + d.x, m * b.y + d.y, m * b.z + d.z, m * b.w + d.w);
    return make_float4(w.x - lr * b.x, w.y - lr * b.y, w.z - lr * b.z, w.w - lr * b.w);
}

__device__ __forceinline__ float4 load_grad4(const float *g, int split) {
    if (split) return make_float4(g[0], g[1], g[2], g[3]);
    return *reinterpret_cast<const float4 *>(g);
}

__global__ __launch_bounds__(256) void sgd_pack_kernel(SgdArgs a) {
    __shared__ uint16_t tile[64][64 + 4];
    int ti = 0;
    for (int k = 1; k < a.n; k++)
        if (a.t[k].first_block <= blockIdx.x) ti = k;
    const SgdTensor T = a.t[ti];
    const uint32_t blk = blockIdx.x - T.first_block;
    const int t = threadIdx.x;
    const float m = a.momentum, lr = T.lr, wd = T.wd;
    if (!T.fwd && !T.dg) {
        if (!T.g) return;
        const size_t base = (size_t)blk * 4096;
        if (T.plain) {
            for (size_t q = base + t; q < T.n && q < base + 4096; q += 256) {
                const float d = T.g[q] + wd * T.p[q], b = m * T.buf[q] + d;
                T.buf[q] = b;
                T.p[q] = T.p[q] - lr * b;
            }
            return;
        }
#pragma unroll
        for (int i = 0; i < 4; i++) {
            const size_t e = base + (size_t)(i * 256 + t) * 4;
            if (e + 3 < T.n) {
                const float4 w = *reinterpret_cast<const float4 *>(T.p + e), g = load_grad4(T.g + e, T.g_split);
                float4 b = *reinterpret_cast<const float4 *>(T.buf + e);
                const float4 nw = sgd4(w, g, b, m, lr, wd);
                *reinterpret_cast<float4 *>(T.buf + e) = b;
                *reinterpret_cast<float4 *>(T.p + e) = nw;
            } else {
                for (size_t q = e; q < T.n && q < e + 4; q++) {
                    const float d = T.g[q] + wd * T.p[q], b = m * T.buf[q] + d;
                    T.buf[q] = b;
                    T.p[q] = T.p[q] - lr * b;
                }
            }
        }
        return;
    }
    const uint32_t cbs = T.cin >> 6, obs = T.cout >> 6;
    const uint32_t tap = blk % T.taps, cb = (blk / T.taps) % cbs, ob = blk / (T.taps * cbs);
    if (ob >= obs) return;
    const int r = t >> 4, q = t & 15;
#pragma unroll
    for (int i = 0; i < 4; i++) {
        const uint32_t o = r + 16 * i;
        const size_t src = ((size_t)(ob * 64 + o) * T.taps + tap) * T.cin + cb * 64 + q * 4;
        float4 w = *reinterpret_cast<const float4 *>(T.p + src);
        if (T.g) {
            const float4 g = load_grad4(T.g + src, T.g_split);
            float4 b = *reinterpret_cast<const float4 *>(T.buf + src);
            w = sgd4(w, g, b, m, lr, wd);
            *reinterpret_cast<float4 *>(T.buf + src) = b;
            *reinterpret_cast<float4 *>(T.p + src) = w;
        }
        const uint2 pk = make_uint2(pack2_bf16(w.x, w.y), pack2_bf16(w.z, w.w));
        if (T.fwd)
            *reinterpret_cast<uint2 *>(T.fwd + (T.plain ? src : (((size_t)(ob * 64 + o) * cbs + cb) * T.taps + tap) * 64 + q * 4)) = pk;
        *reinterpret_cast<uint2 *>(&tile[o][q * 4]) = pk;
    }
    if (!T.dg) return;
    __syncthreads();
#pragma unroll
    for (int i = 0; i < 4; i++) {
        const uint32_t c = r + 16 * i;
        const uint32_t lo = (uint32_t)tile[q * 4 + 0][c] | ((uint32_t)tile[q * 4 + 1][c] << 16);
        const uint32_t hi = (uint32_t)tile[q * 4 + 2][c] | ((uint32_t)tile[q * 4 + 3][c] << 16);
        const size_t dst = T.plain ? ((size_t)(cb * 64 + c) * T.taps + (T.taps - 1 - tap)) * T.cout + ob * 64 + q * 4
                                   : (((size_t)(cb * 64 + c) * obs + ob) * T.taps + (T.taps - 1 - tap)) * 64 + q * 4;
        *reinterpret_cast<uint2 *>(T.dg + dst) = make_uint2(lo, hi);
    }
}
}

int launch_sgd_pack(int n, float *const *p, const float *const *g, float *const *buf, void *const *fwd, void *const *dg,
                    const int *shape, const long long *numel, const float *lr, const float *wd, float momentum, hipStream_t stream) {
    if (n < 0) return set_error(DSRG_ERR_INVALID, "sgd_pack: bad count");
    for (int i0 = 0; i0 < n; i0 += kSgdTensors) {
        SgdArgs a;
        memset(&a, 0, sizeof(a));
        a.momentum = momentum;
        uint32_t blocks = 0;
        for (int i = i0; i < n && i < i0 + kSgdTensors; i++) {
            SgdTensor &T = a.t[a.n++];
            T.p = p[i]; T.g = g ? g[i] : nullptr; T.buf = buf ? buf[i] : nullptr;
            T.fwd = fwd ? static_cast<uint16_t *>(fwd[i]) : nullptr; T.dg = dg ? static_cast<uint16_t *>(dg[i]) : nullptr;
            T.lr = lr ? lr[i] : 0.0f; T.wd = wd ? wd[i] : 0.0f;
            if (!T.p || numel[i] < 1 || numel[i] > 0x7fffffffLL || (T.g && !T.buf))
                return set_error(DSRG_ERR_INVALID, "sgd_pack: tensor %d: null parameter, bad size or a gradient without a momentum buffer", i);
            const uintptr_t low = reinterpret_cast<uintptr_t>(T.p) | reinterpret_cast<uintptr_t>(T.buf);
            if (((low | reinterpret_cast<uintptr_t>(T.g)) & 3) || ((low & 15) && (T.fwd || T.dg)))
                return set_error(DSRG_ERR_INVALID, "sgd_pack: tensor %d is not aligned (4 bytes; parameter and momentum of a packed kernel: 16)", i);
            T.g_split = (reinterpret_cast<uintptr_t>(T.g) & 15) != 0;
            T.n = (uint32_t)numel[i];
            T.first_block = blocks;
            if (T.fwd || T.dg) {
                T.cout = (uint32_t)shape[4 * i]; T.cin = (uint32_t)shape[4 * i + 1]; T.taps = (uint32_t)shape[4 * i + 2]; T.plain = shape[4 * i + 3];
                if (T.cout < 64 || T.cout % 64 || T.cin < 64 || T.cin % 64 || (T.taps != 1 && T.taps != 9) ||
                    (long long)T.cout * T.cin * T.taps != numel[i])
                    return set_error(DSRG_ERR_INVALID, "sgd_pack: tensor %d: a packed kernel needs 64 | cout, 64 | cin, 1 or 9 taps (got %u, %u, %u)",
                                     i, T.cout, T.cin, T.taps);
                blocks += (T.cout / 64) * (T.cin / 64) * T.taps;
            } else {
                T.plain = (low & 15) != 0;
                blocks += (uint32_t)((numel[i] + 4095) / 4096);
            }
        }
        hipLaunchKernelGGL(sgd_pack_kernel, dim3(blocks), dim3(256), 0, stream, a);
        DSRG_LAUNCH_CHECK();
    }
    return DSRG_OK;
}

}
```

### dsrg_amd/ops.py

```python
import contextlib
import ctypes
import os
import threading
import weakref as _weakref

import torch

from . import _lib
from ._lib import CrfParams, check
from .crf import select_arrays


def _stream():
    return ctypes.c_void_p(torch.cuda.current_stream().cuda_stream)


def _ptr(t):
    return ctypes.c_void_p(t.data_ptr()) if t is not None else None


def _f32c(t, name):
    if not (t.is_cuda and t.dtype == torch.float32 and t.is_contiguous()):
        raise ValueError("%s must be a contiguous float32 CUDA tensor" % name)
    return t
# ... 469 lines not shown
    nbytes = stage.numel() if nbytes is None else int(nbytes)
    if not 0 <= nbytes <= stage.numel():
        raise ValueError("the staging buffer holds %d bytes, the batch states %d" % (stage.numel(), nbytes))
    return nbytes


def _out_arg(out, shape, name, dev):
    if out is None:
        return torch.empty(shape, dtype=torch.float32, device=dev)
    _f32c(out, name)
    if tuple(out.shape) != tuple(shape):
        raise ValueError("%s must be %s, got %s" % (name, tuple(shape), tuple(out.shape)))
    return out


def train_s_input_batch(stage, desc, size=321, num_classes=21, map_size=(41, 41), mean=MEAN_PIXEL, out=None, nbytes=None):
    nbytes = _stage_arg(stage, nbytes)
    B = len(desc["H"])
    S, C, (Hm, Wm) = int(size), int(num_classes), (int(map_size[0]), int(map_size[1]))
    if len(mean) != 3:
        raise ValueError("mean must hold 3 values")
    keys = ("image_off", "H", "W", "cue_off", "ncues", "label_off", "nlabels", "mirror")
    if any(len(desc[k]) != B for k in keys):
        raise ValueError("every descriptor list must hold one entry per image")
    out = (None, None, None) if out is None else out
    images = _out_arg(out[0], (B, 3, S, S), "out[0]", stage.device)
    labels = _out_arg(out[1], (B, 1, 1, C), "out[1]", stage.device)
    cues = _out_arg(out[2], (B, C, Hm, Wm), "out[2]", stage.device)
    check(_lib.lib().dsrg_train_s_input_batch(B, _ptr(stage), nbytes, *[_i32s(desc[k]) for k in keys], S, C, Hm, Wm,
                                              (ctypes.c_float * 3)(*[float(m) for m in mean]), _ptr(images), _ptr(cues), _ptr(labels),
                                              _stream()))
    return images, labels, cues


def train_f_input_batch(stage, desc, crop_size, mean, scale=1.0, ignore_label=255, out=None, nbytes=None):
    nbytes = _stage_arg(stage, nbytes)
    B = len(desc["H"])
    ch, cw = int(crop_size[0]), int(crop_size[1])
    if len(mean) != 3:
        raise ValueError("mean must hold 3 values")
    keys = ("image_off", "label_off", "H", "W", "top", "left", "mirror")
    if any(len(desc[k]) != B for k in keys):
        raise ValueError("every descriptor list must hold one entry per image")
    out = (None, None) if out is None else out
    data = _out_arg(out[0], (B, 3, ch, cw), "out[0]", stage.device)
    label = _out_arg(out[1], (B, 1, ch, cw), "out[1]", stage.device)
    check(_lib.lib().dsrg_train_f_input_batch(B, _ptr(stage), nbytes, *[_i32s(desc[k]) for k in keys], ch, cw,
                                              (ctypes.c_float * 3)(*[float(m) for m in mean]), float(scale), float(ignore_label),
                                              _ptr(data), _ptr(label), _stream()))
    return data, label


def supervision_step(logits, images, labels, cues, th1=0.99, th2=0.85, scale_factor=12.0, maxiter=10,
                     ctx=None, want_blobs=False, prepared=False):
    _f32c(logits, "logits"), _f32c(images, "images"), _f32c(labels, "labels"), _f32c(cues, "cues")
    B, C, H, W = logits.shape
    if images.dim() != 4 or images.shape[0] != B or images.shape[1] != 3:
        raise ValueError("images must be (B,3,Hi,Wi) with the batch size of logits")
    if labels.numel() != B * C or tuple(cues.shape) != (B, C, H, W):
        raise ValueError("labels must hold B*C values and cues must have the shape of logits")
    if not lds_path_supports(H, W):
        probs = softmax_forward(logits)
        refined, logq = _crf_refine_large(probs, images, scale_factor, maxiter, True)
        seeds = srg_grow(labels.reshape(B, -1).contiguous(), cues, refined, th1, th2)
        l_seed, g_seed = seed_loss(probs, seeds)
        l_con, g_p, g_q = constrain_loss(probs, logq)
        grad = softmax_backward(logits, g_seed + g_p + crf_layer_backward(refined, g_q))
        losses = torch.stack([l_seed.reshape(()), l_con.reshape(())]).float()
        return losses, grad, (dict(probs=probs, seeds=seeds, logq=logq, refined=refined) if want_blobs else None)
    ctx = ctx or get_context(B, C, H, W)
    losses = torch.empty(2, dtype=torch.float32, device=logits.device)
    grad = torch.empty_like(logits)
    blobs = None
    if want_blobs:
        blobs = dict(probs=torch.empty_like(logits), seeds=torch.empty_like(logits), logq=torch.empty_like(logits))
    prm = CrfParams.from_crf_args(maxiter, scale_factor)
    check(_lib.lib().dsrg_supervision_step(
        ctx._h, B, _ptr(logits), None if prepared else _ptr(images), images.shape[2], images.shape[3],
        _ptr(labels), _ptr(cues),
        float(th1), float(th2), ctypes.byref(prm), _ptr(losses), _ptr(grad),
        _ptr(blobs["probs"]) if blobs else None, _ptr(blobs["seeds"]) if blobs else None,
        _ptr(blobs["logq"]) if blobs else None, _stream()))
    return losses, grad, blobs


def im2col3x3_nhwc(x_nhwc, dilation):
    es = x_nhwc.element_size()
    if not (x_nhwc.is_cuda and x_nhwc.is_contiguous() and es in (2, 4)):
        raise ValueError("x must be a contiguous 2- or 4-byte CUDA tensor in NHWC order")
    B, H, W, C = x_nhwc.shape
    out = torch.empty((B * H * W, 9 * C), dtype=x_nhwc.dtype, device=x_nhwc.device)
    check(_lib.lib().dsrg_im2col3x3_nhwc16(_ptr(x_nhwc), _ptr(out), B, H, W, C * (es // 2), int(dilation), _stream()))
    return out


def col2im3x3_nhwc(cols, B, H, W, C, dilation):
    if not (cols.is_cuda and cols.is_contiguous() and cols.dtype == torch.bfloat16 and cols.shape == (B * H * W, 9 * C)):
        raise ValueError("cols must be a contiguous (B*H*W, 9*C) bf16 CUDA tensor")
    out = torch.empty((B, C, H, W), dtype=cols.dtype, device=cols.device, memory_format=torch.channels_last)
    check(_lib.lib().dsrg_col2im3x3_nhwc_bf16(_ptr(cols), _ptr(out), B, H, W, C, int(dilation), _stream()))
    return out


_PARTIAL_BLOCKS = 512


def relu_bwd_bias(g, y, scale=1.0, gb_out=None):
    B, C, H, W = y.shape
    cl = torch.channels_last
    if not (g.is_cuda and g.dtype == torch.bfloat16 and y.dtype == torch.bfloat16 and y.is_contiguous(memory_format=cl)):
        raise ValueError("relu_bwd_bias needs bf16 channels_last CUDA tensors")
    g = g.contiguous(memory_format=cl)
    gm = torch.empty_like(y)
    gb = _bias_grad_dest(gb_out, (C,), y.device)
    part = _reduction_scratch(y.device, 4 * _PARTIAL_BLOCKS * C, "rows").view(torch.float32)
    check(_lib.lib().dsrg_relu_bwd_bias_bf16(_ptr(g), _ptr(y), _ptr(gm), _ptr(gb), _ptr(part), _PARTIAL_BLOCKS,
                                             B * H * W, C, float(scale), _stream()))
    return gm, gb


def bias_grad(g):
    B, C, H, W = g.shape
    if not (g.is_cuda and g.dtype == torch.bfloat16):
        raise ValueError("bias_grad needs a bf16 CUDA tensor")
    g = g.contiguous(memory_format=torch.channels_last)
    gb = _bias_grad_dest(None, (C,), g.device)
    part = _reduction_scratch(g.device, 4 * _PARTIAL_BLOCKS * C, "rows").view(torch.float32)
    if C % 8 == 0:
        check(_lib.lib().dsrg_relu_bwd_bias_bf16(_ptr(g), None, None, _ptr(gb), _ptr(part), _PARTIAL_BLOCKS,
                                                 B * H * W, C, 1.0, _stream()))
    else:
        check(_lib.lib().dsrg_bias_grad_bf16(_ptr(g), _ptr(gb), _ptr(part), _PARTIAL_BLOCKS, B * H * W, C, _stream()))
    return gb


def avgpool3x3_s1(x):
# ... 108 lines not shown

def _packs_kept(weight):
    return _packs_claimed(weight) and weight.is_cuda and not torch.cuda.is_current_stream_capturing()


def _packs_keep(weight, plain, fwd, dg):
    if not _packs_kept(weight):
        return
    if weight.data_ptr() not in _weight_packs:
        for k in [k for k, e in _weight_packs.items() if e.ref() is None]:
            del _weight_packs[k]
    e = _WeightPacks()
    e.ref, e.version, e.fwd, e.dg, e.plain = _weakref.ref(weight), weight._version, fwd, dg, plain
    _weight_packs[weight.data_ptr()] = e


def _packs_for(weight, plain, want_fwd, want_dgrad, fwd_shape, dg_shape, fwd_cl=False):
    e = _packs_entry(weight, plain) if _packs_kept(weight) else None
    if e is not None and e.version == weight._version and (e.fwd is not None or not want_fwd) and (e.dg is not None or not want_dgrad):
        return (e.fwd if want_fwd else None), (e.dg if want_dgrad else None), True
    mf = torch.channels_last if fwd_cl else torch.contiguous_format
    fwd = (e.fwd if e is not None and e.fwd is not None else torch.empty(fwd_shape, dtype=torch.bfloat16, device=weight.device, memory_format=mf)) \
        if (want_fwd or (e is not None and e.fwd is not None)) else None
    dg = (e.dg if e is not None and e.dg is not None else torch.empty(dg_shape, dtype=torch.bfloat16, device=weight.device, memory_format=mf)) \
        if (want_dgrad or (e is not None and e.dg is not None)) else None
    return fwd, dg, False


_CHECK_PACKS = int(os.environ.get("DSRG_CHECK_PACKS", "0") or 0)
_check_packs_calls = [0]


def _check_kept_packs(weight, fwd, dg, pack):
    if _CHECK_PACKS <= 0:
        return
    _check_packs_calls[0] += 1
    if _check_packs_calls[0] % _CHECK_PACKS:
        return
    f2 = torch.empty_like(fwd) if fwd is not None else None
    d2 = torch.empty_like(dg) if dg is not None else None
    pack(f2, d2)
    if (f2 is not None and not torch.equal(f2, fwd)) or (d2 is not None and not torch.equal(d2, dg)):
        raise RuntimeError("DSRG_CHECK_PACKS: the kept bf16 kernels of a %s parameter no longer match its float32 value — it was "
                           "written behind the version counter's back (param.data, a foreign kernel, torch._fused_sgd_); call "
                           "dsrg_amd.ops.forget_weight_packs([param]) after such a write" % (tuple(weight.shape),))


def sgd_pack_step(params, grads, bufs, lrs, wds, momentum):
    import numpy as np
    n = len(params)
    if n == 0:
        return
    ptr = lambda ts: np.array([0 if t is None else t.data_ptr() for t in ts], dtype=np.uint64)
    fwd, dg, shape, entries = [None] * n, [None] * n, np.zeros((n, 4), dtype=np.int32), []
    for i, p in enumerate(params):
        e = _weight_packs.get(p.data_ptr())
        if e is None or e.ref() is None or e.ref().data_ptr() != p.data_ptr() or e.ref().shape != p.shape:
            continue
        fwd[i], dg[i] = e.fwd, e.dg
        shape[i] = (p.shape[0], p.shape[1], p.shape[2] * p.shape[3], e.plain)
        entries.append((e, p))
    pp, gp, bp, fp, dp = ptr(params), ptr(grads), ptr(bufs), ptr(fwd), ptr(dg)
    numel = np.array([p.numel() for p in params], dtype=np.int64)
    lr, wd = np.asarray(lrs, dtype=np.float32), np.asarray(wds, dtype=np.float32)
    a = lambda x: x.ctypes.data
    check(_lib.lib().dsrg_sgd_pack_f32(n, a(pp), a(gp), a(bp), a(fp), a(dp), a(shape), a(numel), a(lr), a(wd), float(momentum), _stream()))
    torch.autograd.graph.increment_version(list(params))
    for e, p in entries:
        e.version = p._version


def sgd_pack_eligible(p, g, b):
    return p.is_cuda and p.dtype == torch.float32 and g.dtype == torch.float32 and b.dtype == torch.float32 and g.is_cuda and \
        g.shape == p.shape and all(n == 1 or (sg == sp and sb == sp) for n, sp, sg, sb in zip(p.shape, p.stride(), g.stride(), b.stride())) and \
        (p.is_contiguous() or (p.dim() == 4 and p.is_contiguous(memory_format=torch.channels_last))) and \
        ((p.data_ptr() | b.data_ptr()) % 16 == 0 or p.data_ptr() not in _weight_packs)


def pack_direct_weight_pair(weight, want_dgrad=True):
    cout, cin = weight.shape[0], weight.shape[1]
    cl = torch.channels_last
    if not (weight.is_cuda and weight.dtype == torch.float32 and weight.is_contiguous(memory_format=cl) and tuple(weight.shape[2:]) == (3, 3)
            and cin in DIRECT_CONV_CHANNELS and cout in DIRECT_CONV_CHANNELS):
        raise ValueError("pack_direct_weight_pair needs a float32 channels_last (cout,cin,3,3) CUDA parameter with 64 / 128 channels")
    fwd, dg, fresh = _packs_for(weight, 1, True, want_dgrad, (cout, cin, 3, 3), (cin, cout, 3, 3), fwd_cl=True)
    pack = lambda f, d: check(_lib.lib().dsrg_pack_conv_weight_direct_f32(_ptr(weight.detach()), _ptr(f), _ptr(d), cout, cin, _stream()))
    if not fresh:
        pack(fwd, dg)
        _packs_keep(weight, 1, fwd, dg)
    else:
        _check_kept_packs(weight, fwd, dg, pack)
    return fwd, (dg if want_dgrad else None)


def conv3x3_wgrad(x, g, out_dtype=torch.bfloat16, out=None):
    B, cin, H, W = x.shape
    cout = g.shape[1]
    cl = torch.channels_last
    if not (x.is_cuda and x.dtype == torch.bfloat16 and g.dtype == torch.bfloat16 and tuple(g.shape) == (B, cout, H, W)
            and (cin, cout) in WGRAD_CONV_SHAPES):
        raise ValueError("conv3x3_wgrad needs bf16 CUDA tensors with (cin, cout) in %s" % (WGRAD_CONV_SHAPES,))
    x = x.contiguous(memory_format=cl)
    g = g.contiguous(memory_format=cl)
    ws = _stream_scratch("wgrad3x3", x.device, _lib.lib().dsrg_conv3x3_wgrad_workspace(B, H, W, cin, cout))
    if out_dtype not in (torch.bfloat16, torch.float32):
        raise ValueError("conv3x3_wgrad: bf16 or float32 output")
    gw = _dest(out, (cout, cin, 3, 3), out_dtype, x.device, True)
    fn = _lib.lib().dsrg_conv3x3_wgrad_f32 if out_dtype == torch.float32 else _lib.lib().dsrg_conv3x3_wgrad_bf16
    check(fn(_ptr(x), _ptr(g), _ptr(gw), _ptr(ws), ws.numel(), B, H, W, cin, cout, _stream()))
    return gw


def conv_igemm_supported(cin, cout, k):
    return bool(_lib.lib().dsrg_conv_igemm_supported(int(cin), int(cout), int(k)))


def set_igemm_variant(v):
    _lib.lib().dsrg_debug_set_igemm_variant(int(v))


def pack_conv_weight(weight, for_dgrad=False, dtype=torch.bfloat16):
    k = weight.shape[2]
    if for_dgrad:
        weight = weight.flip(2, 3).transpose(0, 1) if k > 1 else weight.transpose(0, 1)
    o, c = weight.shape[0], weight.shape[1]
    out = torch.empty((o, c // 64, k * k, 64), dtype=dtype, device=weight.device)
    if weight.is_contiguous(memory_format=torch.channels_last) and not weight.is_contiguous():
        out.copy_(weight.permute(0, 2, 3, 1).reshape(o, k * k, c // 64, 64).permute(0, 2, 1, 3))
    else:
# ... 237 lines not shown
                                       _ptr(ws), ws.numel(), B, H, W, cin, cout, ksize, int(out_dtype == torch.bfloat16), _stream()))
    return gws


def conv_igemm_wgrad_splits(n, B, H, W, cin, cout, ksize, dilations):
    taps = int(ksize) * int(ksize)
    out = (ctypes.c_int * (n * taps))()
    check(_lib.lib().dsrg_conv_igemm_wgrad_splits(int(n), int(B), int(H), int(W), int(cin), int(cout), int(ksize),
                                                   (ctypes.c_int * n)(*[int(d) for d in dilations]), out))
    return [list(out[g * taps:(g + 1) * taps]) for g in range(n)]


def heads_forward(xs, weight, bias):
    B, K, H, W = xs[0].shape
    n, O = weight.shape[0], weight.shape[1]
    cl = torch.channels_last
    xs = [x.contiguous(memory_format=cl) for x in xs]
    if not all(x.is_cuda and x.dtype == torch.bfloat16 and x.shape == xs[0].shape for x in xs) or len(xs) != n:
        raise ValueError("heads_forward needs n bf16 CUDA activations of one shape")
    _f32c(weight, "weight")
    if bias is not None:
        _f32c(bias, "bias")
    out = torch.empty((B, O, H, W), dtype=torch.float32, device=xs[0].device)
    ptrs = (ctypes.c_void_p * 4)(*([x.data_ptr() for x in xs] + [None] * (4 - n)))
    check(_lib.lib().dsrg_heads_forward_bf16(ptrs, n, _ptr(weight), _ptr(bias), _ptr(out), B, H * W, K, O, _stream()))
    return out


def heads_backward(xs, weight, g, need_gx=True, relu_scale=0.0):
    B, K, H, W = xs[0].shape
    n, O = weight.shape[0], weight.shape[1]
    cl = torch.channels_last
    xs = [x.contiguous(memory_format=cl) for x in xs]
    _f32c(weight, "weight")
    g = g.contiguous()
    _f32c(g, "g")
    L = _lib.lib()
    M = B * H * W
    gx = torch.empty((n, B, H, W, K), dtype=torch.bfloat16, device=g.device) if need_gx else None
    gw = torch.empty((n, O, K), dtype=torch.float32, device=g.device)
    part = torch.empty(L.dsrg_heads_backward_chunks(M) * n * O * K, dtype=torch.float32, device=g.device)
    ptrs = (ctypes.c_void_p * 4)(*([x.data_ptr() for x in xs] + [None] * (4 - n)))
    if relu_scale > 0.0 and need_gx:
        gb = _bias_grad_dest(None, (n, K), g.device)
        ws = _reduction_scratch(g.device, L.dsrg_heads_backward_relu_workspace(n, M, K))
        check(L.dsrg_heads_backward_relu_bf16(ptrs, n, _ptr(weight), _ptr(g), _ptr(gx), M * K * 2, _ptr(gw), _ptr(part),
                                              float(relu_scale), _ptr(gb), _ptr(ws), ws.numel(), B, H * W, K, O, _stream()))
        return [gx[k].permute(0, 3, 1, 2) for k in range(n)], gw, gb
    check(L.dsrg_heads_backward_bf16(ptrs, n, _ptr(weight), _ptr(g), _ptr(gx), M * K * 2, _ptr(gw), _ptr(part), B, H * W, K, O,
                                     _stream()))
    return ([gx[k].permute(0, 3, 1, 2) for k in range(n)] if need_gx else None), gw


def maxpool3x3_out_size(n, stride, ceil_mode):
    num = n + 2 - 3
    o = (-(-num // stride) if ceil_mode else num // stride) + 1
    if (o - 1) * stride >= n + 1:
        o -= 1
    return o


def resnet_stem_pack(weight, scale):
    if not (weight.is_cuda and weight.dtype == torch.float32 and tuple(weight.shape) == (64, 3, 7, 7)):
        raise ValueError("resnet_stem_pack needs a (64,3,7,7) float32 CUDA kernel")
    if tuple(scale.shape) != (64,):
        raise ValueError("resnet_stem_pack needs 64 scales")
    w = weight.detach().contiguous()
    nbytes = _lib.lib().dsrg_resnet_stem_packed_bytes()
    packed = torch.empty((64, nbytes // 128), dtype=torch.bfloat16, device=weight.device)
    check(_lib.lib().dsrg_pack_resnet_stem_f32(_ptr(w), _ptr(_f32c(scale.detach(), "scale")), _ptr(packed), _stream()))
    return packed


def resnet_stem(x, packed, shift):
    if not (x.dim() == 4 and x.shape[1] == 3):
        raise ValueError("resnet_stem needs a (B,3,H,W) input")
    x = _f32c(x, "x")
    B, _, H, W = x.shape
    if not (packed.is_cuda and packed.dtype == torch.bfloat16 and packed.is_contiguous()
            and packed.numel() * 2 == _lib.lib().dsrg_resnet_stem_packed_bytes()):
        raise ValueError("resnet_stem needs a kernel packed by resnet_stem_pack")
    if tuple(shift.shape) != (64,):
        raise ValueError("resnet_stem needs 64 shifts")
    OHc, OWc = (H - 1) // 2 + 1, (W - 1) // 2 + 1
    PH, PW = maxpool3x3_out_size(OHc, 2, True), maxpool3x3_out_size(OWc, 2, True)
    y = torch.empty((B, 64, PH, PW), dtype=torch.bfloat16, device=x.device, memory_format=torch.channels_last)
    check(_lib.lib().dsrg_resnet_stem_bf16(_ptr(x), _ptr(packed), _ptr(_f32c(shift, "shift")), _ptr(y), B, H, W, _stream()))
    return y


def maxpool3x3_fwd(x, stride, ceil_mode, relu_input=False):
    B, C, H, W = x.shape
    OH, OW = maxpool3x3_out_size(H, stride, ceil_mode), maxpool3x3_out_size(W, stride, ceil_mode)
    out = torch.empty((B, C, OH, OW), dtype=x.dtype, device=x.device, memory_format=torch.channels_last)
    code = torch.empty((B, OH, OW, C), dtype=torch.uint8, device=x.device)
    fn = _lib.lib().dsrg_maxpool3x3_relu_fwd_bf16 if relu_input else _lib.lib().dsrg_maxpool3x3_fwd_bf16
    check(fn(_ptr(x), _ptr(out), _ptr(code), B, H, W, OH, OW, C, stride, _stream()))
    return out, code


def maxpool3x3_bwd(gout, code, in_shape, stride):
    B, C, H, W = in_shape
    OH, OW = gout.shape[2], gout.shape[3]
    gout = gout.contiguous(memory_format=torch.channels_last)
    gin = torch.empty((B, C, H, W), dtype=gout.dtype, device=gout.device, memory_format=torch.channels_last)
    check(_lib.lib().dsrg_maxpool3x3_bwd_bf16(_ptr(gout), _ptr(code), _ptr(gin), B, H, W, OH, OW, C, stride, _stream()))
    return gin


def maxpool3x3_bwd_relu(gout, code, relu_out, stride=2, gb_out=None):
    have_y = torch.is_tensor(relu_out)
    B, C, H, W = relu_out.shape if have_y else relu_out
    OH, OW = gout.shape[2], gout.shape[3]
    cl = torch.channels_last
    if stride != 2 or not (gout.is_cuda and gout.dtype == torch.bfloat16 and C % 8 == 0 and 256 % (C // 8) == 0) or (
            have_y and not (relu_out.is_cuda and relu_out.dtype == torch.bfloat16 and relu_out.is_contiguous(memory_format=cl))):
        raise ValueError("maxpool3x3_bwd_relu: stride 2, bf16 channels_last, channels / 8 a divisor of 256")
    gout = gout.contiguous(memory_format=cl)
    gin = torch.empty((B, C, H, W), dtype=torch.bfloat16, device=gout.device, memory_format=cl)
    gb = _bias_grad_dest(gb_out, (C,), gout.device)
    part = _reduction_scratch(gout.device, 4 * _PARTIAL_BLOCKS * C, "rows").view(torch.float32)
    check(_lib.lib().dsrg_maxpool3x3_bwd_relu_bf16(_ptr(gout), _ptr(code), _ptr(relu_out) if have_y else None, _ptr(gin), _ptr(gb), _ptr(part),
                                                   _PARTIAL_BLOCKS, B, H, W, OH, OW, C, _stream()))
    return gin, gb


class DSRGSupervision(torch.autograd.Function):

    @staticmethod
    def forward(ctx, logits, images, labels, cues, th1, th2, scale_factor, maxiter, prepared=False):
        losses, grad, _ = supervision_step(logits.contiguous(), images, labels, cues, th1, th2, scale_factor, maxiter,
                                           prepared=prepared)
        ctx.save_for_backward(grad)
        ctx.mark_non_differentiable(losses)
        return losses.sum(), losses

    @staticmethod
    def backward(ctx, g_total, _g_losses):
        (grad,) = ctx.saved_tensors
        return grad * g_total, None, None, None, None, None, None, None, None


def dsrg_supervision_loss(logits, images, labels, cues, th1=0.99, th2=0.85, scale_factor=12.0, maxiter=10,
                          prepared=False):
    return DSRGSupervision.apply(logits, images, labels, cues, th1, th2, scale_factor, maxiter, prepared)
```

### dsrg_amd/trainer.py

```python
import os

import torch

from .backbone import VGG16ASPP
from .ops import dsrg_supervision_loss


_SGD_PACK = os.environ.get("DSRG_SGD_PACK", "1") != "0"


class CaffeSGD(object):

    def __init__(self, groups, base_lr=5e-4, momentum=0.9, weight_decay=5e-4, gamma=0.33, stepsize=1000):
        self.groups = groups
        self.base_lr, self.momentum, self.wd, self.gamma, self.stepsize = base_lr, momentum, weight_decay, gamma, stepsize
        self.iter = 0
        for g in self.groups:
            g["bufs"] = [torch.zeros_like(p, memory_format=torch.preserve_format) for p in g["params"]]
            g["buf_lr"] = None
        if _SGD_PACK:
            from .ops import keep_weight_packs
            keep_weight_packs([p for g in self.groups for p in g["params"] if p.is_cuda], self)

    def lr(self):
# ... 101 lines not shown
        net = net.to(device)
        if channels_last:
            net = net.to(memory_format=torch.channels_last)
        self.net = net
        self.reducer = None
        if (world_size > 1) if ddp is None else ddp:
            from .reducer import BucketedAllReduce
            self.reducer = BucketedAllReduce(list(net.parameters()), bucket_cap_mb=bucket_cap_mb)
        self.opt = CaffeSGD(net.caffe_param_groups())
        self.defer_bias = device.type == "cuda" and os.environ.get("DSRG_DEFER_REDUCTIONS", "1") != "0"
        if snapshot is not None:
            self.load(snapshot)
        self.dropout_stream_seed = seed + 1 + distributed_rank()
        torch.manual_seed(self.dropout_stream_seed)

    def save(self, prefix="models/model-s"):
        from .checkpoint import save_snapshot
        return save_snapshot(self, prefix)

    def load(self, state_path):
        from .checkpoint import load_snapshot
        it = load_snapshot(self, state_path)
        if self.device.type == "cuda":
            from .ops import forget_weight_packs
            forget_weight_packs(self.net.parameters())
        return it

    def reduce_losses(self, losses):
        import torch.distributed as dist
        if not (dist.is_available() and dist.is_initialized()) or dist.get_world_size() == 1:
            return losses
        out = losses.detach().clone()
        dist.all_reduce(out, op=dist.ReduceOp.SUM)
        return out / dist.get_world_size()

    def weights_checksum(self):
        return params_checksum(list(self.net.parameters()) + [b for g in self.opt.groups for b in g["bufs"]])

    def weights_equal_across_ranks(self):
        import torch.distributed as dist
        mine = self.weights_checksum()
        if not (dist.is_available() and dist.is_initialized()) or dist.get_world_size() == 1:
            return True, [[int(v) for v in mine.cpu()]]
        parts = [torch.zeros_like(mine) for _ in range(dist.get_world_size())]
        dist.all_gather(parts, mine)
        words = [[int(v) for v in p.cpu()] for p in parts]
        return all(w == words[0] for w in words), words

    def step(self, images, labels, cues):
        if self.reducer is not None:
            self.reducer.prepare()
        else:
            self.opt.zero_grad()
        x = images.contiguous(memory_format=torch.channels_last) if self.channels_last else images
        if self.overlap_build:
            from .ops import crf_prepare
            main = torch.cuda.current_stream()
            self.side.wait_stream(main)
            with torch.cuda.stream(self.side):
                crf_prepare(images, cues.shape[1], cues.shape[2], cues.shape[3])
        with torch.autocast(self.device.type, dtype=self.amp_dtype, enabled=self.amp_dtype is not None):
            logits = self.net(x)
        logits = logits.float().contiguous()
        if self.overlap_build:
            torch.cuda.current_stream().wait_stream(self.side)
            total, losses = self.loss_fn(logits, images, labels, cues, prepared=True)
        else:
            total, losses = self.loss_fn(logits, images, labels, cues)
        from .ops import deferred_reductions
        with deferred_reductions(self.defer_bias):
            total.backward()
        if self.reducer is not None:
            self.reducer.finish()
        self.opt.step()
        return losses
```

### include/dsrg_hip.h

```cpp
#ifndef DSRG_HIP_H
#define DSRG_HIP_H

#include <stddef.h>
#include <stdint.h>

#ifdef __cplusplus
extern "C" {
#endif

#pragma GCC visibility push(default)

#define DSRG_OK 0
#define DSRG_ERR_INVALID (-1)
#define DSRG_ERR_HIP (-2)
#define DSRG_ERR_UNSUPPORTED (-3)
#define DSRG_ERR_NOMEM (-4)

const char *dsrg_last_error(void);
int dsrg_device_count(void);
int dsrg_host_register(void *host, size_t bytes);
int dsrg_host_unregister(void *host);

typedef struct dsrg_crf_s *dsrg_crf_t;

// ... 146 lines not shown
                                  void *y_dev, int dilation, int B, int H, int W, int cin, int cout, int ksize, int relu, void *stream);
int dsrg_aspp_shift_sum_f32(const void *y_dev, const float *bias_dev, float *out_dev, const int *offsets, int npairs, int outputs,
                            int channels, int B, int H, int W, void *stream);
int dsrg_aspp_shift_gather_bf16(const float *g_dev, void *gp_dev, const int *offsets, int npairs, int outputs, int channels, int B, int H,
                                int W, void *stream);
int dsrg_defer_reductions(int on);
int dsrg_flush_reductions(void *stream);
int dsrg_conv_igemm_workspace_status(const void *workspace_dev, void *stream, int *status_host);
int dsrg_pack_conv_weight_f32(const float *w_dev, void *fwd_dev, void *dgrad_dev, int cout, int cin, int ksize, void *stream);
int dsrg_pack_conv_weight_scaled_f32(const float *w_dev, const float *scale_dev, void *fwd_dev, void *dgrad_dev, int cout, int cin,
                                     int ksize, void *stream);
int dsrg_sgd_pack_f32(int n, float *const *param_dev, const float *const *grad_dev, float *const *momentum_dev, void *const *fwd_dev,
                      void *const *dgrad_dev, const int *shape, const long long *numel, const float *lr, const float *weight_decay,
                      float momentum, void *stream);
size_t dsrg_conv_igemm_wgrad_workspace(int ngroups, int B, int H, int W, int cin, int cout, int ksize);
int dsrg_conv_igemm_wgrad_splits(int ngroups, int B, int H, int W, int cin, int cout, int ksize, const int *dilation, int *splits_out);
int dsrg_conv_igemm_wgrad_bf16(const void *const *x_dev, const void *const *g_dev, void *const *gw_dev, const int *dilation,
                               int ngroups, void *workspace_dev, size_t workspace_bytes, int B, int H, int W, int cin, int cout,
                               int ksize, int out_bf16, void *stream);
int dsrg_conv_igemm_backward_bf16(const void *g_dev, const void *w_dgrad_dev, const void *x_dev, const void *mask_dev, void *gx_dev,
                                  float *gw_dev, int dilation, float *bias_grad_dev, float mask_scale, void *colsum_workspace_dev,
                                  size_t colsum_workspace_bytes, void *wgrad_workspace_dev, size_t wgrad_workspace_bytes, int B, int H,
                                  int W, int cin, int cout, int ksize, void *stream);
int dsrg_conv_igemm_backward_residual_bf16(const void *g_dev, const void *w_dgrad_dev, const void *x_dev, const void *mask_dev,
                                           const void *res_dev, void *gx_dev, float *gw_dev, const float *gw_scale_dev, int dilation,
                                           void *wgrad_workspace_dev, size_t wgrad_workspace_bytes, int B, int H, int W, int cin, int cout,
                                           int ksize, void *stream);
int dsrg_heads_forward_bf16(const void *const *x_dev, int n_branches, const float *w_dev, const float *bias_dev,
                            float *out_dev, int B, int HW, int K, int O, void *stream);
int dsrg_heads_backward_chunks(int M);
int dsrg_heads_backward_bf16(const void *const *x_dev, int n_branches, const float *w_dev, const float *g_dev,
                             void *gx_dev, size_t gx_branch_stride_bytes, float *gw_dev, float *partial_dev, int B,
                             int HW, int K, int O, void *stream);
size_t dsrg_heads_backward_relu_workspace(int n_branches, int M, int K);
int dsrg_heads_backward_relu_bf16(const void *const *x_dev, int n_branches, const float *w_dev, const float *g_dev,
                                  void *gx_dev, size_t gx_branch_stride_bytes, float *gw_dev, float *partial_dev,
                                  float relu_scale, float *bias_grad_dev, void *workspace_dev, size_t workspace_bytes, int B,
                                  int HW, int K, int O, void *stream);
int dsrg_maxpool3x3_fwd_bf16(const void *in_dev, void *out_dev, void *code_dev, int B, int H, int W, int OH, int OW, int C,
                             int stride, void *stream);
int dsrg_maxpool3x3_relu_fwd_bf16(const void *in_dev, void *out_dev, void *code_dev, int B, int H, int W, int OH, int OW, int C,
                                  int stride, void *stream);
int dsrg_maxpool3x3_bwd_bf16(const void *gout_dev, const void *code_dev, void *gin_dev, int B, int H, int W, int OH, int OW,
                             int C, int stride, void *stream);
int dsrg_maxpool3x3_bwd_relu_bf16(const void *gout_dev, const void *code_dev, const void *relu_out_dev, void *gin_dev,
                                  float *bias_grad_dev, float *partials_dev, int partial_blocks, int B, int H, int W, int OH,
                                  int OW, int C, void *stream);

int dsrg_supervision_step(dsrg_ctx_t ctx, int B, const float *logits_dev, const float *images_dev,
                          int img_h, int img_w, const float *labels_dev, const float *cues_dev,
                          double th1, double th2, const dsrg_crf_params *params,
                          float *losses_dev, float *grad_logits_dev,
                          float *probs_dev, float *seeds_dev, float *logq_dev, void *stream);

#pragma GCC visibility pop

#ifdef __cplusplus
}
#endif
#endif
```

Baseline: 2020.

## Fuse small glue ops: pointer-based ASPP heads, image cast, grad sum, loss total

Adds several small fused kernels that remove glue work in the train step. The ASPP head kernels now read per-branch weight and bias pointers, so stacking and casting head weights each step is no longer needed. The fp32 NCHW image is cast to bf16 NHWC in one kernel, shared-input dgrads from parallel branches are summed in a bf16 kernel, the supervision kernel writes the summed loss directly, and SGD can emit bf16 weight casts. The gain is fewer launches and copies, at the cost of more code paths and more fallback conditions to keep correct.

```diff
diff --git a/dsrg_amd/_lib.py b/dsrg_amd/_lib.py
--- a/dsrg_amd/_lib.py
+++ b/dsrg_amd/_lib.py
@@ -134,6 +134,13 @@
     "dsrg_maxpool3x3_bwd_relu_bf16": (_i, [_vp, _vp, _vp, _vp, _vp, _vp, _i, _i, _i, _i, _i, _i, _i, _vp]),
     "dsrg_supervision_step": (_i, [_vp, _i, _vp, _vp, _i, _i, _vp, _vp, _d, _d, ctypes.POINTER(CrfParams),
                                    _vp, _vp, _vp, _vp, _vp, _vp]),
+    "dsrg_supervision_step_total": (_i, [_vp, _i, _vp, _vp, _i, _i, _vp, _vp, _d, _d, ctypes.POINTER(CrfParams),
+                                         _vp, _vp, _vp, _vp, _vp, _vp, _vp]),
+    "dsrg_heads_forward_ptrs_bf16": (_i, [_vp, _i, _vp, _vp, _vp, _i, _i, _i, _i, _vp]),
+    "dsrg_heads_backward_ptrs_bf16": (_i, [_vp, _i, _vp, _vp, _vp, _sz, _vp, _vp, _f, _vp, _vp, _sz] + [_i] * 4 + [_vp]),
+    "dsrg_image_nchw_to_nhwc_bf16": (_i, [_vp, _vp, _i, _i, _i, _vp]),
+    "dsrg_sum_bf16": (_i, [_vp, _i, _vp, _sz, _vp]),
+    "dsrg_sgd_pack_cast_f32": (_i, [_i] + [_vp] * 10 + [_f, _vp]),
 }
 
 _LIB = None
diff --git a/dsrg_amd/backbone.py b/dsrg_amd/backbone.py
--- a/dsrg_amd/backbone.py
+++ b/dsrg_amd/backbone.py
@@ -188,6 +188,9 @@
     @staticmethod
     def forward(ctx, k, dils, relu, drop_p, pool, n, links_in, links_out, *t):
         xs, ws, bs = t[:n], t[n:2 * n], t[2 * n:3 * n]
+        ctx.same_x = n > 1 and xs[0].dtype == torch.bfloat16 and all(
+            x.data_ptr() == xs[0].data_ptr() and x.shape == xs[0].shape and x.stride() == xs[0].stride() and x.dtype == xs[0].dtype
+            and x._version == xs[0]._version for x in xs[1:])
         xs = [x if x.dtype == torch.bfloat16 else x.bfloat16() for x in xs]
         packs_d = [None] * n
         fb = [b.detach().float().contiguous() for b in bs]
@@ -282,18 +285,29 @@
                 d = ctx.dils[i]
                 gws.append(torch.ops.aten.convolution_backward(gms[i], xs[i], ws[i].to(torch.bfloat16), None, [1, 1], [d, d], [d, d],
                                                                False, [0, 0], 1, [False, True, False])[1].float())
+        if ctx.same_x and all(need_x) and _sum_takes(gxs):
+            gxs = [ops.sum_bf16(list(gxs))] + [None] * (n - 1)
         return (None,) * 8 + tuple(gx if nx else None for gx, nx in zip(gxs, need_x)) + tuple(gws) + tuple(gbs)
 
 
+def _sum_takes(gs):
+    g0 = gs[0]
+    return 2 <= len(gs) <= 4 and all(g is not None and g.is_cuda and g.dtype == torch.bfloat16 and g.shape == g0.shape and
+                                     g.stride() == g0.stride() for g in gs) and g0.numel() > 0 and g0.numel() % 8 == 0 and \
+        (g0.is_contiguous() or (g0.dim() == 4 and g0.is_contiguous(memory_format=torch.channels_last)))
+
+
 class _DirectConvFn(torch.autograd.Function):
 
     @staticmethod
     def forward(ctx, x, weight, bias, relu, pool, link_in, link_out):
+        cl = torch.channels_last
+        if ops.image_takes_fused_cast(x):
+            x = ops.image_to_bf16_nhwc(x)
         x = x if x.dtype == torch.bfloat16 else x.bfloat16()
-        cl = torch.channels_last
         x = x if x.is_contiguous(memory_format=cl) else x.contiguous(memory_format=cl)
         if weight.shape[1] == 3:
-            w16, wd = weight.detach().to(torch.bfloat16), None
+            w16, wd = ops.cast_weight_kept(weight), None
         else:
             w16, wd = ops.pack_direct_weight_pair(weight, ctx.needs_input_grad[0])
         out = ops.conv3x3_direct(x, w16, bias.detach(), relu)
@@ -500,6 +514,37 @@
         return (None, gw, gb1.unsqueeze(0).expand(n, O).contiguous()) + (tuple(gxs) if gxs is not None else (None,) * n)
 
 
+class _HeadsPtrFn(torch.autograd.Function):
+
+    @staticmethod
+    def forward(ctx, links, n, *t):
+        ws, bs, xs = t[:n], t[n:2 * n], t[2 * n:]
+        cl = torch.channels_last
+        ctx.links = links if (links is not None and all(lk is not None for lk in links) and
+                              all(x.is_contiguous(memory_format=cl) for x in xs)) else None
+        xs = [x.contiguous(memory_format=cl) for x in xs]
+        ctx.n = n
+        ctx.gw_out = [getattr(w, "_dsrg_grad_out", None) for w in ws]
+        ctx.save_for_backward(*ws, *xs)
+        return ops.heads_forward_ptrs(xs, [w.detach() for w in ws], [b.detach() for b in bs])
+
+    @staticmethod
+    def backward(ctx, g):
+        n = ctx.n
+        ws, xs = ctx.saved_tensors[:n], ctx.saved_tensors[n:]
+        O = ws[0].shape[0]
+        need_x = ctx.needs_input_grad[2 + 2 * n:]
+        if _FUSE_CHAIN and ctx.links is not None and all(need_x):
+            gxs, gws, gb_below = ops.heads_backward_ptrs(xs, ws, g, True, ctx.links[0].scale, gw_outs=ctx.gw_out)
+            for i, lk in enumerate(ctx.links):
+                lk.leave(gxs[i], gb_below[i])
+        else:
+            gxs, gws = ops.heads_backward_ptrs(xs, ws, g, need_gx=any(need_x), gw_outs=ctx.gw_out)
+        gb = g.sum((0, 2, 3)).unsqueeze(0).expand(n, O).contiguous()
+        gws = [_landed(gw, o) for gw, o in zip(gws, ctx.gw_out)]
+        return (None, None) + tuple(gws) + tuple(gb[i] for i in range(n)) + (tuple(gxs) if gxs is not None else (None,) * n)
+
+
 class _StackKernels(torch.autograd.Function):
 
     @staticmethod
@@ -571,9 +616,11 @@
         heads = [br[-1] for br in self.branches]
         if hs[0].is_cuda and hs[0].dtype == torch.bfloat16 and len(hs) <= 4 and heads[0].out_channels <= 32 \
                 and heads[0].in_channels % 256 == 0:
+            links = [getattr(h, "_dsrg_grad_link", None) for h in hs]
+            if all(m.bias is not None for m in heads) and ops.heads_kernels_in_place([m.weight for m in heads], [m.bias for m in heads]):
+                return _HeadsPtrFn.apply(links, len(heads), *[m.weight for m in heads], *[m.bias for m in heads], *hs)
             w = _StackKernels.apply(*[m.weight for m in heads])
             b = torch.stack([m.bias for m in heads])
-            links = [getattr(h, "_dsrg_grad_link", None) for h in hs]
             return _HeadsFn.apply(links, w.float(), b.float(), *hs)
         out = None
         with torch.autocast(device_type=hs[0].device.type, enabled=False):
diff --git a/dsrg_amd/csrc/api.hip b/dsrg_amd/csrc/api.hip
--- a/dsrg_amd/csrc/api.hip
+++ b/dsrg_amd/csrc/api.hip
@@ -598,15 +598,22 @@
 }
 namespace dsrg {
 int launch_sgd_pack(int n, float *const *p, const float *const *g, float *const *buf, void *const *fwd, void *const *dg, const int *shape,
-                    const long long *numel, const float *lr, const float *wd, float momentum, hipStream_t stream);
+                    const long long *numel, const float *lr, const float *wd, float momentum, hipStream_t stream,
+                    void *const *cast = nullptr);
 }
 extern "C" int dsrg_sgd_pack_f32(int n, float *const *param_dev, const float *const *grad_dev, float *const *momentum_dev, void *const *fwd_dev,
                                  void *const *dgrad_dev, const int *shape, const long long *numel, const float *lr, const float *weight_decay,
                                  float momentum, void *stream) {
+    return dsrg_sgd_pack_cast_f32(n, param_dev, grad_dev, momentum_dev, fwd_dev, dgrad_dev, nullptr, shape, numel, lr, weight_decay,
+                                  momentum, stream);
+}
+extern "C" int dsrg_sgd_pack_cast_f32(int n, float *const *param_dev, const float *const *grad_dev, float *const *momentum_dev,
+                                      void *const *fwd_dev, void *const *dgrad_dev, void *const *cast_dev, const int *shape,
+                                      const long long *numel, const float *lr, const float *weight_decay, float momentum, void *stream) {
     if (n > 0 && (!param_dev || !numel || ((fwd_dev || dgrad_dev) && !shape)))
         return set_error(DSRG_ERR_INVALID, "sgd_pack: null argument");
     return launch_sgd_pack(n, param_dev, grad_dev, momentum_dev, fwd_dev, dgrad_dev, shape, numel, lr, weight_decay, momentum,
-                           static_cast<hipStream_t>(stream));
+                           static_cast<hipStream_t>(stream), cast_dev);
 }
 extern "C" size_t dsrg_conv_igemm_wgrad_workspace(int ngroups, int B, int H, int W, int cin, int cout, int ksize) {
     return conv_igemm_wgrad_workspace(ngroups, B, H, W, cin, cout, ksize);
@@ -694,6 +701,34 @@
     return launch_heads_bwd(x_dev, n_branches, w_dev, g_dev, gx_dev, gx_branch_stride_bytes, gw_dev, partial_dev, B, HW, K, O,
                             static_cast<hipStream_t>(stream), relu_scale, bias_grad_dev, workspace_dev, workspace_bytes);
 }
+extern "C" int dsrg_heads_forward_ptrs_bf16(const void *const *x_dev, int n_branches, const float *const *w_dev,
+                                            const float *const *bias_dev, float *out_dev, int B, int HW, int K, int O, void *stream) {
+    if (!x_dev || !w_dev || !out_dev || B < 1 || HW < 1 || n_branches < 1 || n_branches > 4) return set_error(DSRG_ERR_INVALID, "bad argument");
+    for (int k = 0; k < n_branches; k++)
+        if (!x_dev[k] || !w_dev[k]) return set_error(DSRG_ERR_INVALID, "NULL branch input or kernel");
+    return launch_heads_fwd_ptrs(x_dev, n_branches, w_dev, bias_dev, out_dev, B, HW, K, O, static_cast<hipStream_t>(stream));
+}
+extern "C" int dsrg_heads_backward_ptrs_bf16(const void *const *x_dev, int n_branches, const float *const *w_dev, const float *g_dev,
+                                             void *gx_dev, size_t gx_branch_stride_bytes, float *const *gw_dev, float *partial_dev,
+                                             float relu_scale, float *bias_grad_dev, void *workspace_dev, size_t workspace_bytes,
+                                             int B, int HW, int K, int O, void *stream) {
+    if (!x_dev || !w_dev || !g_dev || (!gx_dev && !gw_dev) || (gw_dev && !partial_dev) || B < 1 || HW < 1 || n_branches < 1 ||
+        n_branches > 4 || (relu_scale > 0.0f && (!gx_dev || !bias_grad_dev)))
+        return set_error(DSRG_ERR_INVALID, "bad argument");
+    for (int k = 0; k < n_branches; k++)
+        if (!x_dev[k] || !w_dev[k] || (gw_dev && !gw_dev[k])) return set_error(DSRG_ERR_INVALID, "NULL branch input, kernel or gradient");
+    return launch_heads_bwd_ptrs(x_dev, n_branches, w_dev, g_dev, gx_dev, gx_branch_stride_bytes, gw_dev, partial_dev, B, HW, K, O,
+                                 static_cast<hipStream_t>(stream), relu_scale > 0.0f ? relu_scale : 0.0f, bias_grad_dev, workspace_dev,
+                                 workspace_bytes);
+}
+extern "C" int dsrg_image_nchw_to_nhwc_bf16(const float *x_dev, void *y_dev, int B, int H, int W, void *stream) {
+    if (!x_dev || !y_dev) return set_error(DSRG_ERR_INVALID, "NULL argument");
+    return launch_image_nhwc_bf16(x_dev, y_dev, B, H, W, static_cast<hipStream_t>(stream));
+}
+extern "C" int dsrg_sum_bf16(const void *const *g_dev, int n, void *out_dev, size_t numel, void *stream) {
+    if (!g_dev) return set_error(DSRG_ERR_INVALID, "NULL argument");
+    return launch_sum_bf16(g_dev, n, out_dev, numel, static_cast<hipStream_t>(stream));
+}
 extern "C" int dsrg_maxpool3x3_fwd_bf16(const void *in, void *out, void *code, int B, int H, int W, int OH, int OW, int C,
                                         int stride, void *stream) {
     if (!in || !out || !code) return set_error(DSRG_ERR_INVALID, "NULL argument");
@@ -722,6 +757,13 @@
                                      int img_w, const float *labels, const float *cues, double th1, double th2,
                                      const dsrg_crf_params *prm, float *losses, float *grad_logits,
                                      float *probs_out, float *seeds_out, float *logq_out, void *stream) {
+    return dsrg_supervision_step_total(c, B, logits, images, img_h, img_w, labels, cues, th1, th2, prm, losses, nullptr, grad_logits,
+                                       probs_out, seeds_out, logq_out, stream);
+}
+extern "C" int dsrg_supervision_step_total(dsrg_ctx_t c, int B, const float *logits, const float *images, int img_h,
+                                           int img_w, const float *labels, const float *cues, double th1, double th2,
+                                           const dsrg_crf_params *prm, float *losses, float *total, float *grad_logits,
+                                           float *probs_out, float *seeds_out, float *logq_out, void *stream) {
     if (!c || !logits || !labels || !cues || !losses || !grad_logits)
         return set_error(DSRG_ERR_INVALID, "NULL argument");
     if (B < 1 || B > c->maxB) return set_error(DSRG_ERR_INVALID, "batch %d outside 1..%d", B, c->maxB);
@@ -748,7 +790,7 @@
     rc = launch_srg(B, C, c->H, c->W, labels, cues, c->refined, th1, th2, c->seeds, c->srg_code, s);
     if (rc) return rc;
     rc = launch_sup_loss_backward(B, C, N, logits, c->probs, c->seeds, c->logq, c->refined, c->stats, grad_logits,
-                                  losses, s);
+                                  losses, s, total);
     if (rc) return rc;
     if (probs_out) DSRG_HIP_CHECK(hipMemcpyAsync(probs_out, c->probs, nb, hipMemcpyDeviceToDevice, s));
     if (seeds_out) DSRG_HIP_CHECK(hipMemcpyAsync(seeds_out, c->seeds, nb, hipMemcpyDeviceToDevice, s));
diff --git a/dsrg_amd/csrc/backbone_ops.hip b/dsrg_amd/csrc/backbone_ops.hip
--- a/dsrg_amd/csrc/backbone_ops.hip
+++ b/dsrg_amd/csrc/backbone_ops.hip
@@ -586,8 +586,8 @@
 constexpr int kHeadOutPad = 32;
 struct HeadArgs {
     const uint16_t *x[4];
-    const float *w;
-    const float *bias;
+    const float *w[4];
+    const float *bias[4];
     float *out;
     int nbr, M, K, O, HW;
 };
@@ -598,13 +598,14 @@
 }
 
 struct HeadMask {
+    const float *w[4];
     const uint16_t *y[4];
     float *part;
     float scale;
     int tiles;
 };
 template <bool MASK>
-__global__ __launch_bounds__(256) void heads_bwd_dx_kernel(const float *__restrict__ g, const float *__restrict__ w,
+__global__ __launch_bounds__(256) void heads_bwd_dx_kernel(const float *__restrict__ g,
                                                            uint4 *__restrict__ gx, int M, int K, int O, int HW, size_t branch_stride,
                                                            HeadMask hm) {
     __shared__ __attribute__((aligned(16))) float gs[32][16];
@@ -633,7 +634,7 @@
             for (int r = 0; r < 8; r++)
 #pragma unroll
                 for (int c = 0; c < 8; c++) acc[r][c] = 0.0f;
-            const float *wk = w + (size_t)k * O * K + (size_t)cg * 8;
+            const float *__restrict__ wk = hm.w[k] + (size_t)cg * 8;
 #pragma unroll 7
             for (int o = 0; o < O; o++) {
                 const float4 w0 = *reinterpret_cast<const float4 *>(wk + (size_t)o * K), w1 = *reinterpret_cast<const float4 *>(wk + (size_t)o * K + 4);
@@ -691,7 +692,7 @@
 }
 
 template <int O, bool MASK>
-__global__ __launch_bounds__(256) void heads_bwd_dx_rows_kernel(const float *__restrict__ g, const float *__restrict__ w,
+__global__ __launch_bounds__(256) void heads_bwd_dx_rows_kernel(const float *__restrict__ g,
                                                                 unsigned char *__restrict__ gx, int M, int K, int HW, size_t branch_stride,
                                                                 HeadMask hm, int rows_per_wg) {
     constexpr int OP = (O + 3) & ~3;
@@ -706,9 +707,10 @@
         gs_rows[r * OP + o] = v;
     }
     float wr[O][4];
+    const float *__restrict__ wk = hm.w[k];
 #pragma unroll
     for (int o = 0; o < O; o++) {
-        const float4 v = *reinterpret_cast<const float4 *>(w + ((size_t)k * O + o) * K + c);
+        const float4 v = *reinterpret_cast<const float4 *>(wk + (size_t)o * K + c);
         wr[o][0] = v.x; wr[o][1] = v.y; wr[o][2] = v.z; wr[o][3] = v.w;
     }
     __syncthreads();
@@ -834,12 +836,33 @@
             for (int r = 0; r < 16; r++) acc[t][r] = 0.0f;
     }
 }
-__global__ void heads_bwd_dw_reduce_kernel(const float *__restrict__ partial, float *__restrict__ gw, int nchunks, size_t n) {
+constexpr int kHeadReduceBatch = 16;
+struct HeadGw { float *p[4]; };
+__global__ __launch_bounds__(256) void heads_bwd_dw_reduce_kernel(const float *__restrict__ partial, HeadGw gw, int nchunks, size_t n,
+                                                                  size_t per_branch) {
     const size_t i = (size_t)blockIdx.x * blockDim.x + threadIdx.x;
     if (i >= n) return;
+    const float *__restrict__ p = partial + i;
     float s = 0.0f;
-    for (int c = 0; c < nchunks; c++) s += partial[(size_t)c * n + i];
-    gw[i] = s;
+    int c = 0;
+    for (; c + kHeadReduceBatch <= nchunks; c += kHeadReduceBatch) {
+        float v[kHeadReduceBatch];
+#pragma unroll
+        for (int u = 0; u < kHeadReduceBatch; u++) v[u] = p[(size_t)(c + u) * n];
+#pragma unroll
+        for (int u = 0; u < kHeadReduceBatch; u++) s += v[u];
+    }
+    if (c < nchunks) {
+        float v[kHeadReduceBatch];
+#pragma unroll
+        for (int u = 0; u < kHeadReduceBatch; u++) v[u] = c + u < nchunks ? p[(size_t)(c + u) * n] : 0.0f;
+#pragma unroll
+        for (int u = 0; u < kHeadReduceBatch; u++)
+            if (c + u < nchunks) s += v[u];
+    }
+    const size_t k = i / per_branch;
+    float *dst = k == 0 ? gw.p[0] : k == 1 ? gw.p[1] : k == 2 ? gw.p[2] : gw.p[3];
+    dst[i - k * per_branch] = s;
 }
 
 namespace {
@@ -891,7 +914,7 @@
         const uint16_t *xp[R];
 #pragma unroll
         for (int t = 0; t < R; t++) xp[t] = a.x[wave] + (size_t)min(m0 + 32 * t + row, a.M - 1) * a.K + half * 8;
-        const float *wp = a.w + ((size_t)wave * a.O + min(row, a.O - 1)) * a.K + half * 8;
+        const float *wp = a.w[wave] + (size_t)min(row, a.O - 1) * a.K + half * 8;
         constexpr int G = 4;
         uint4 xv[G][R];
         float4 wv[G][2];
@@ -943,7 +966,7 @@
                 const int hf = (rr >> 2) & 1, reg = (rr & 3) + 4 * (rr >> 3), ln = col + 32 * hf;
                 float s = 0.0f;
                 for (int k = 0; k < a.nbr; k++) {
-                    const float sk = part[t][k][reg][ln] + (a.bias ? a.bias[k * a.O + col] : 0.0f);
+                    const float sk = part[t][k][reg][ln] + (a.bias[k] ? a.bias[k][col] : 0.0f);
                     s = k == 0 ? sk : s + sk;
                 }
                 const int b = m / a.HW, hw = m - b * a.HW;
@@ -1026,16 +1049,29 @@
     return DSRG_OK;
 }
 
+int launch_heads_fwd_ptrs(const void *const *x, int nbr, const float *const *w, const float *const *bias, float *out, int B, int HW,
+                          int K, int O, hipStream_t stream) {
+    int rc = heads_check(nbr, K, O);
+    if (rc) return rc;
+    HeadArgs a;
+    for (int k = 0; k < 4; k++) {
+        a.x[k] = static_cast<const uint16_t *>(x[k < nbr ? k : 0]);
+        a.w[k] = w[k < nbr ? k : 0];
+        a.bias[k] = bias ? bias[k < nbr ? k : 0] : nullptr;
+    }
+    a.out = out; a.nbr = nbr; a.M = B * HW; a.K = K; a.O = O; a.HW = HW;
+    hipLaunchKernelGGL(heads_fwd_split_kernel<2>, dim3((a.M + 63) / 64), dim3(256), 0, stream, a);
+    DSRG_LAUNCH_CHECK();
+    return DSRG_OK;
+}
+
 int launch_heads_fwd(const void *const *x, int nbr, const float *w, const float *bias, float *out, int B, int HW, int K, int O,
                      hipStream_t stream) {
     int rc = heads_check(nbr, K, O);
     if (rc) return rc;
-    HeadArgs a;
-    for (int k = 0; k < 4; k++) a.x[k] = static_cast<const uint16_t *>(x[k < nbr ? k : 0]);
-    a.w = w; a.bias = bias; a.out = out; a.nbr = nbr; a.M = B * HW; a.K = K; a.O = O; a.HW = HW;
-    hipLaunchKernelGGL(heads_fwd_split_kernel<2>, dim3((a.M + 63) / 64), dim3(256), 0, stream, a);
-    DSRG_LAUNCH_CHECK();
-    return DSRG_OK;
+    const float *wk[4], *bk[4];
+    for (int k = 0; k < nbr; k++) { wk[k] = w + (size_t)k * O * K; bk[k] = bias ? bias + (size_t)k * O : nullptr; }
+    return launch_heads_fwd_ptrs(x, nbr, wk, bias ? bk : nullptr, out, B, HW, K, O, stream);
 }
 
 int heads_bwd_chunks(int M) { int c = (M + 255) / 256; return c < 1 ? 1 : (c > 128 ? 128 : c); }
@@ -1048,14 +1084,16 @@
     return (size_t)nbr * rows * (size_t)K * sizeof(float);
 }
 
-int launch_heads_bwd(const void *const *x, int nbr, const float *w, const float *g, void *gx, size_t gx_branch_stride,
-                     float *gw, float *partial, int B, int HW, int K, int O, hipStream_t stream, float relu_scale, float *bias_grad,
-                     void *colsum_ws, size_t colsum_ws_bytes) {
+int launch_heads_bwd_ptrs(const void *const *x, int nbr, const float *const *w, const float *g, void *gx, size_t gx_branch_stride,
+                          float *const *gw, float *partial, int B, int HW, int K, int O, hipStream_t stream, float relu_scale,
+                          float *bias_grad, void *colsum_ws, size_t colsum_ws_bytes) {
     int rc = heads_check(nbr, K, O);
     if (rc) return rc;
     const int M = B * HW;
+    HeadMask hm;
+    memset(&hm, 0, sizeof(hm));
+    for (int k = 0; k < 4; k++) hm.w[k] = w[k < nbr ? k : 0];
     if (gx && relu_scale > 0.0f) {
-        HeadMask hm;
         for (int k = 0; k < 4; k++) hm.y[k] = static_cast<const uint16_t *>(x[k < nbr ? k : 0]);
         hm.tiles = kHeadMaskTiles; hm.scale = relu_scale;
         const int nblk = (M + 16 * kHeadMaskTiles - 1) / (16 * kHeadMaskTiles);
@@ -1066,10 +1104,10 @@
         if (head_strips(K, O)) {
             nblk_s = (M + kHeadStripRows - 1) / kHeadStripRows;
             hipLaunchKernelGGL((heads_bwd_dx_rows_kernel<21, true>), dim3(nblk_s, nbr, K / 1024), dim3(256),
-                               (size_t)kHeadStripRows * 24 * sizeof(float), stream, g, w, static_cast<unsigned char *>(gx), M, K, HW,
+                               (size_t)kHeadStripRows * 24 * sizeof(float), stream, g, static_cast<unsigned char *>(gx), M, K, HW,
                                gx_branch_stride, hm, kHeadStripRows);
         } else {
-            hipLaunchKernelGGL(heads_bwd_dx_kernel<true>, dim3(nblk, nbr), dim3(256), 0, stream, g, w, static_cast<uint4 *>(gx), M, K, O, HW,
+            hipLaunchKernelGGL(heads_bwd_dx_kernel<true>, dim3(nblk, nbr), dim3(256), 0, stream, g, static_cast<uint4 *>(gx), M, K, O, HW,
                                gx_branch_stride, hm);
         }
         DSRG_LAUNCH_CHECK();
@@ -1078,21 +1116,20 @@
         for (int k = 0; k < nbr; k++) { parts[k] = hm.part + (size_t)k * nblk_s * K; outs[k] = bias_grad + (size_t)k * K; }
         if (int rc2 = launch_igemm_colsum(parts, outs, nbr, nblk_s, K, stream)) return rc2;
     } else if (gx) {
-        HeadMask hm;
-        memset(&hm, 0, sizeof(hm));
         if (head_strips(K, O))
             hipLaunchKernelGGL((heads_bwd_dx_rows_kernel<21, false>), dim3((M + kHeadStripRows - 1) / kHeadStripRows, nbr, K / 1024),
-                               dim3(256), (size_t)kHeadStripRows * 24 * sizeof(float), stream, g, w, static_cast<unsigned char *>(gx), M, K, HW,
+                               dim3(256), (size_t)kHeadStripRows * 24 * sizeof(float), stream, g, static_cast<unsigned char *>(gx), M, K, HW,
                                gx_branch_stride, hm, kHeadStripRows);
         else
-            hipLaunchKernelGGL(heads_bwd_dx_kernel<false>, dim3((M + 15) / 16, nbr), dim3(256), 0, stream, g, w, static_cast<uint4 *>(gx), M,
+            hipLaunchKernelGGL(heads_bwd_dx_kernel<false>, dim3((M + 15) / 16, nbr), dim3(256), 0, stream, g, static_cast<uint4 *>(gx), M,
                                K, O, HW, gx_branch_stride, hm);
         DSRG_LAUNCH_CHECK();
     }
     if (gw) {
         HeadArgs a;
+        memset(&a, 0, sizeof(a));
         for (int k = 0; k < 4; k++) a.x[k] = static_cast<const uint16_t *>(x[k < nbr ? k : 0]);
-        a.w = w; a.bias = nullptr; a.out = nullptr; a.nbr = nbr; a.M = M; a.K = K; a.O = O; a.HW = HW;
+        a.nbr = nbr; a.M = M; a.K = K; a.O = O; a.HW = HW;
         const int nch = heads_bwd_chunks(M), rows = ((M + nch - 1) / nch + 1) & ~1;
         const size_t lds = (size_t)kDwRows2 * (K * 2 + 64) + 32 * kDwGPitch * sizeof(float);
         if (lds > 160 * 1024) {
@@ -1104,10 +1141,94 @@
         }
         DSRG_LAUNCH_CHECK();
         const size_t n = (size_t)nbr * O * K;
-        hipLaunchKernelGGL(heads_bwd_dw_reduce_kernel, dim3((unsigned)((n + 255) / 256)), dim3(256), 0, stream, partial, gw, nch, n);
+        HeadGw dst;
+        for (int k = 0; k < 4; k++) dst.p[k] = gw[k < nbr ? k : 0];
+        hipLaunchKernelGGL(heads_bwd_dw_reduce_kernel, dim3((unsigned)((n + 255) / 256)), dim3(256), 0, stream, partial, dst, nch, n,
+                           (size_t)O * K);
         DSRG_LAUNCH_CHECK();
     }
     return DSRG_OK;
 }
 
-}
+int launch_heads_bwd(const void *const *x, int nbr, const float *w, const float *g, void *gx, size_t gx_branch_stride,
+                     float *gw, float *partial, int B, int HW, int K, int O, hipStream_t stream, float relu_scale, float *bias_grad,
+                     void *colsum_ws, size_t colsum_ws_bytes) {
+    int rc = heads_check(nbr, K, O);
+    if (rc) return rc;
+    const float *wk[4];
+    float *gwk[4];
+    for (int k = 0; k < nbr; k++) { wk[k] = w + (size_t)k * O * K; gwk[k] = gw ? gw + (size_t)k * O * K : nullptr; }
+    return launch_heads_bwd_ptrs(x, nbr, wk, g, gx, gx_branch_stride, gw ? gwk : nullptr, partial, B, HW, K, O, stream, relu_scale,
+                                 bias_grad, colsum_ws, colsum_ws_bytes);
+}
+
+namespace {
+__device__ __forceinline__ uint32_t f32_to_bf16_torch(float f) {
+    const uint32_t u = __float_as_uint(f);
+    if ((u & 0x7fffffffu) > 0x7f800000u) return 0x7fc0u;
+    return (u + 0x7fffu + ((u >> 16) & 1u)) >> 16;
+}
+struct SumArgs { const uint4 *g[4]; int n; };
+}
+
+__global__ __launch_bounds__(256) void image_nhwc_bf16_kernel(const float *__restrict__ x, uint16_t *__restrict__ y, size_t npix, int HW) {
+    const size_t q = (size_t)blockIdx.x * blockDim.x + threadIdx.x, p0 = 2 * q;
+    if (p0 >= npix) return;
+    const size_t b0 = p0 / HW, i0 = p0 - b0 * HW;
+    const float *x0 = x + b0 * 3 * HW + i0;
+    const uint32_t r0 = f32_to_bf16_torch(x0[0]), g0 = f32_to_bf16_torch(x0[HW]), c0 = f32_to_bf16_torch(x0[2 * (size_t)HW]);
+    if (p0 + 1 >= npix) {
+        y[3 * p0] = (uint16_t)r0; y[3 * p0 + 1] = (uint16_t)g0; y[3 * p0 + 2] = (uint16_t)c0;
+        return;
+    }
+    const size_t p1 = p0 + 1, b1 = p1 / HW, i1 = p1 - b1 * HW;
+    const float *x1 = x + b1 * 3 * HW + i1;
+    const uint32_t r1 = f32_to_bf16_torch(x1[0]), g1 = f32_to_bf16_torch(x1[HW]), c1 = f32_to_bf16_torch(x1[2 * (size_t)HW]);
+    uint32_t *d = reinterpret_cast<uint32_t *>(y + 3 * p0);
+    d[0] = r0 | (g0 << 16); d[1] = c0 | (r1 << 16); d[2] = g1 | (c1 << 16);
+}
+
+int launch_image_nhwc_bf16(const float *x, void *y, int B, int H, int W, hipStream_t stream) {
+    if (B < 1 || H < 1 || W < 1 || (long long)H * W > 0x7fffffffLL) return set_error(DSRG_ERR_INVALID, "image cast: bad shape");
+    const size_t npix = (size_t)B * H * W, threads = (npix + 1) / 2;
+    hipLaunchKernelGGL(image_nhwc_bf16_kernel, dim3((unsigned)((threads + 255) / 256)), dim3(256), 0, stream, x, static_cast<uint16_t *>(y),
+                       npix, H * W);
+    DSRG_LAUNCH_CHECK();
+    return DSRG_OK;
+}
+
+__global__ __launch_bounds__(256) void sum_bf16_kernel(SumArgs a, uint4 *__restrict__ out, size_t n8) {
+    const size_t i = (size_t)blockIdx.x * blockDim.x + threadIdx.x;
+    if (i >= n8) return;
+    uint4 v[4];
+#pragma unroll
+    for (int k = 0; k < 4; k++)
+        if (k < a.n) v[k] = a.g[k][i];
+    uint32_t s[4] = {v[0].x, v[0].y, v[0].z, v[0].w};
+#pragma unroll
+    for (int k = 1; k < 4; k++) {
+        if (k >= a.n) break;
+        const uint32_t t[4] = {v[k].x, v[k].y, v[k].z, v[k].w};
+#pragma unroll
+        for (int e = 0; e < 4; e++)
+            s[e] = f32_to_bf16_torch(bf16_lo(s[e]) + bf16_lo(t[e])) | (f32_to_bf16_torch(bf16_hi(s[e]) + bf16_hi(t[e])) << 16);
+    }
+    out[i] = make_uint4(s[0], s[1], s[2], s[3]);
+}
+
+int launch_sum_bf16(const void *const *g, int n, void *out, size_t numel, hipStream_t stream) {
+    if (n < 2 || n > 4 || numel < 8 || numel % 8) return set_error(DSRG_ERR_INVALID, "sum_bf16: 2..4 tensors, a multiple of 8 elements");
+    SumArgs a;
+    a.n = n;
+    for (int k = 0; k < 4; k++) {
+        a.g[k] = static_cast<const uint4 *>(g[k < n ? k : 0]);
+        if (!a.g[k] || (reinterpret_cast<uintptr_t>(a.g[k]) & 15)) return set_error(DSRG_ERR_INVALID, "sum_bf16: tensor %d is null or not 16-byte aligned", k);
+    }
+    if (!out || (reinterpret_cast<uintptr_t>(out) & 15)) return set_error(DSRG_ERR_INVALID, "sum_bf16: output is null or not 16-byte aligned");
+    const size_t n8 = numel / 8;
+    hipLaunchKernelGGL(sum_bf16_kernel, dim3((unsigned)((n8 + 255) / 256)), dim3(256), 0, stream, a, static_cast<uint4 *>(out), n8);
+    DSRG_LAUNCH_CHECK();
+    return DSRG_OK;
+}
+
+}
diff --git a/dsrg_amd/csrc/common.h b/dsrg_amd/csrc/common.h
--- a/dsrg_amd/csrc/common.h
+++ b/dsrg_amd/csrc/common.h
@@ -194,7 +194,7 @@
                           float *glq, hipStream_t stream);
 int launch_sup_loss_backward(int B, int C, int HW, const float *logits, const float *probs, const float *seeds,
                              const float *logq, const double *refined, double *stats, float *grad_logits,
-                             float *losses, hipStream_t stream);
+                             float *losses, hipStream_t stream, float *total = nullptr);
 int launch_lf_to_planes(int N, int M, const float *in, float *out, int negate, hipStream_t stream);
 int launch_planes_to_lf(int N, int M, const float *in, float *out, hipStream_t stream);
 int launch_argmax_planes(int N, int M, const float *q, int32_t *lab, hipStream_t stream);
@@ -268,6 +268,13 @@
                      float *gw, float *partial, int B, int HW, int K, int O, hipStream_t stream, float relu_scale = 0.0f,
                      float *bias_grad = nullptr, void *colsum_ws = nullptr, size_t colsum_ws_bytes = 0);
 size_t heads_bwd_relu_workspace(int nbr, int M, int K);
+int launch_heads_fwd_ptrs(const void *const *x, int nbr, const float *const *w, const float *const *bias, float *out, int B, int HW,
+                          int K, int O, hipStream_t stream);
+int launch_heads_bwd_ptrs(const void *const *x, int nbr, const float *const *w, const float *g, void *gx, size_t gx_branch_stride,
+                          float *const *gw, float *partial, int B, int HW, int K, int O, hipStream_t stream, float relu_scale = 0.0f,
+                          float *bias_grad = nullptr, void *colsum_ws = nullptr, size_t colsum_ws_bytes = 0);
+int launch_image_nhwc_bf16(const float *x, void *y, int B, int H, int W, hipStream_t stream);
+int launch_sum_bf16(const void *const *g, int n, void *out, size_t numel, hipStream_t stream);
 int launch_add_relu(const void *a, const void *b, void *y, size_t n, hipStream_t stream);
 int launch_aspp_shift_sum(const void *yp, const float *bias, float *out, const int *offsets, int J, int O, int CT, int B, int H, int W,
                           hipStream_t stream);
diff --git a/dsrg_amd/csrc/layers.hip b/dsrg_amd/csrc/layers.hip
--- a/dsrg_amd/csrc/layers.hip
+++ b/dsrg_amd/csrc/layers.hip
@@ -342,7 +342,7 @@
                                                        const double *__restrict__ refined,
                                                        const double *__restrict__ stats,
                                                        float *__restrict__ grad_logits,
-                                                       float *__restrict__ losses) {
+                                                       float *__restrict__ losses, float *__restrict__ total) {
     constexpr int P = kGradParts, LPP = (CT + P - 1) / P;
     const int lane = threadIdx.x & 63, part = threadIdx.x & (P - 1), lane0 = lane & ~(P - 1);
     const int idx = blockIdx.x * kGradPix + (int)(threadIdx.x / P);
@@ -380,8 +380,10 @@
             __syncthreads();
         }
         if (threadIdx.x == 0) {
-            losses[0] = (float)ls;
-            losses[1] = (float)(lc / ((double)B * (double)HW));
+            const float l0 = (float)ls, l1 = (float)(lc / ((double)B * (double)HW));
+            losses[0] = l0;
+            losses[1] = l1;
+            if (total) *total = (0.0f + l0) + l1;
         }
     }
     const float dbg = (float)(cnt_bg > 1e-4 ? cnt_bg : 1e-4), dfg = (float)(cnt_fg > 1e-4 ? cnt_fg : 1e-4);
@@ -429,17 +431,17 @@
 }
 int launch_sup_loss_backward(int B, int C, int HW, const float *logits, const float *probs, const float *seeds,
                              const float *logq, const double *refined, double *stats, float *grad_logits,
-                             float *losses, hipStream_t stream) {
+                             float *losses, hipStream_t stream, float *total) {
     if (C < 1 || C > kMaxLabels) return set_error(DSRG_ERR_UNSUPPORTED, "1 <= C <= %d required", kMaxLabels);
     hipLaunchKernelGGL(sup_stats_kernel, dim3(B * kStatSplit), dim3(1024), 0, stream, C, HW, probs, seeds, logq, stats);
     DSRG_LAUNCH_CHECK();
     const int threads = kGradParts * kGradPix, blocks = (B * HW + kGradPix - 1) / kGradPix;
     if (C <= 21)
         hipLaunchKernelGGL(sup_grad_kernel<21>, dim3(blocks), dim3(threads), 0, stream, B, C, HW, logits, probs, seeds,
-                           logq, refined, stats, grad_logits, losses);
+                           logq, refined, stats, grad_logits, losses, total);
     else
         hipLaunchKernelGGL(sup_grad_kernel<kMaxLabels>, dim3(blocks), dim3(threads), 0, stream, B, C, HW, logits,
-                           probs, seeds, logq, refined, stats, grad_logits, losses);
+                           probs, seeds, logq, refined, stats, grad_logits, losses, total);
     DSRG_LAUNCH_CHECK();
     return DSRG_OK;
 }
diff --git a/dsrg_amd/csrc/sgd_pack.hip b/dsrg_amd/csrc/sgd_pack.hip
--- a/dsrg_amd/csrc/sgd_pack.hip
+++ b/dsrg_amd/csrc/sgd_pack.hip
@@ -17,6 +17,7 @@
     const float *g;
     float *buf;
     uint16_t *fwd, *dg;
+    uint16_t *cast;
     uint32_t n;
     uint32_t cout, cin, taps;
     uint32_t first_block;
@@ -51,31 +52,44 @@
     const int t = threadIdx.x;
     const float m = a.momentum, lr = T.lr, wd = T.wd;
     if (!T.fwd && !T.dg) {
-        if (!T.g) return;
+        if (!T.g && !T.cast) return;
         const size_t base = (size_t)blk * 4096;
+        auto scalar = [&](size_t q) {
+            float w = T.p[q];
+            if (T.g) {
+                const float d = T.g[q] + wd * w, b = m * T.buf[q] + d;
+                T.buf[q] = b;
+                w = w - lr * b;
+                T.p[q] = w;
+            }
+            if (T.cast) T.cast[q] = (uint16_t)pack2_bf16(w, 0.0f);
+        };
         if (T.plain) {
-            for (size_t q = base + t; q < T.n && q < base + 4096; q += 256) {
-                const float d = T.g[q] + wd * T.p[q], b = m * T.buf[q] + d;
-                T.buf[q] = b;
-                T.p[q] = T.p[q] - lr * b;
-            }
+            for (size_t q = base + t; q < T.n && q < base + 4096; q += 256) scalar(q);
             return;
         }
 #pragma unroll
         for (int i = 0; i < 4; i++) {
             const size_t e = base + (size_t)(i * 256 + t) * 4;
             if (e + 3 < T.n) {
-                const float4 w = *reinterpret_cast<const float4 *>(T.p + e), g = load_grad4(T.g + e, T.g_split);
-                float4 b = *reinterpret_cast<const float4 *>(T.buf + e);
-                const float4 nw = sgd4(w, g, b, m, lr, wd);
-                *reinterpret_cast<float4 *>(T.buf + e) = b;
-                *reinterpret_cast<float4 *>(T.p + e) = nw;
+                float4 w = *reinterpret_cast<const float4 *>(T.p + e);
+                if (T.g) {
+                    const float4 g = load_grad4(T.g + e, T.g_split);
+                    float4 b = *reinterpret_cast<const float4 *>(T.buf + e);
+                    w = sgd4(w, g, b, m, lr, wd);
+                    *reinterpret_cast<float4 *>(T.buf + e) = b;
+                    *reinterpret_cast<float4 *>(T.p + e) = w;
+                }
+                if (T.cast) {
+                    if (reinterpret_cast<uintptr_t>(T.cast) & 7) {
+                        T.cast[e] = (uint16_t)pack2_bf16(w.x, 0.0f); T.cast[e + 1] = (uint16_t)pack2_bf16(w.y, 0.0f);
+                        T.cast[e + 2] = (uint16_t)pack2_bf16(w.z, 0.0f); T.cast[e + 3] = (uint16_t)pack2_bf16(w.w, 0.0f);
+                    } else {
+                        *reinterpret_cast<uint2 *>(T.cast + e) = make_uint2(pack2_bf16(w.x, w.y), pack2_bf16(w.z, w.w));
+                    }
+                }
             } else {
-                for (size_t q = e; q < T.n && q < e + 4; q++) {
-                    const float d = T.g[q] + wd * T.p[q], b = m * T.buf[q] + d;
-                    T.buf[q] = b;
-                    T.p[q] = T.p[q] - lr * b;
-                }
+                for (size_t q = e; q < T.n && q < e + 4; q++) scalar(q);
             }
         }
         return;
@@ -116,7 +130,8 @@
 }
 
 int launch_sgd_pack(int n, float *const *p, const float *const *g, float *const *buf, void *const *fwd, void *const *dg,
-                    const int *shape, const long long *numel, const float *lr, const float *wd, float momentum, hipStream_t stream) {
+                    const int *shape, const long long *numel, const float *lr, const float *wd, float momentum, hipStream_t stream,
+                    void *const *cast) {
     if (n < 0) return set_error(DSRG_ERR_INVALID, "sgd_pack: bad count");
     for (int i0 = 0; i0 < n; i0 += kSgdTensors) {
         SgdArgs a;
@@ -127,12 +142,15 @@
             SgdTensor &T = a.t[a.n++];
             T.p = p[i]; T.g = g ? g[i] : nullptr; T.buf = buf ? buf[i] : nullptr;
             T.fwd = fwd ? static_cast<uint16_t *>(fwd[i]) : nullptr; T.dg = dg ? static_cast<uint16_t *>(dg[i]) : nullptr;
+            T.cast = cast ? static_cast<uint16_t *>(cast[i]) : nullptr;
             T.lr = lr ? lr[i] : 0.0f; T.wd = wd ? wd[i] : 0.0f;
             if (!T.p || numel[i] < 1 || numel[i] > 0x7fffffffLL || (T.g && !T.buf))
                 return set_error(DSRG_ERR_INVALID, "sgd_pack: tensor %d: null parameter, bad size or a gradient without a momentum buffer", i);
             const uintptr_t low = reinterpret_cast<uintptr_t>(T.p) | reinterpret_cast<uintptr_t>(T.buf);
             if (((low | reinterpret_cast<uintptr_t>(T.g)) & 3) || ((low & 15) && (T.fwd || T.dg)))
                 return set_error(DSRG_ERR_INVALID, "sgd_pack: tensor %d is not aligned (4 bytes; parameter and momentum of a packed kernel: 16)", i);
+            if (T.cast && (T.fwd || T.dg || (reinterpret_cast<uintptr_t>(T.cast) & 1)))
+                return set_error(DSRG_ERR_INVALID, "sgd_pack: tensor %d: a bf16 copy goes with a tensor without packed forms, 2-byte aligned", i);
             T.g_split = (reinterpret_cast<uintptr_t>(T.g) & 15) != 0;
             T.n = (uint32_t)numel[i];
             T.first_block = blocks;
diff --git a/dsrg_amd/ops.py b/dsrg_amd/ops.py
--- a/dsrg_amd/ops.py
+++ b/dsrg_amd/ops.py
@@ -545,7 +545,7 @@
 
 
 def supervision_step(logits, images, labels, cues, th1=0.99, th2=0.85, scale_factor=12.0, maxiter=10,
-                     ctx=None, want_blobs=False, prepared=False):
+                     ctx=None, want_blobs=False, prepared=False, want_total=False):
     _f32c(logits, "logits"), _f32c(images, "images"), _f32c(labels, "labels"), _f32c(cues, "cues")
     B, C, H, W = logits.shape
     if images.dim() != 4 or images.shape[0] != B or images.shape[1] != 3:
@@ -560,21 +560,23 @@
         l_con, g_p, g_q = constrain_loss(probs, logq)
         grad = softmax_backward(logits, g_seed + g_p + crf_layer_backward(refined, g_q))
         losses = torch.stack([l_seed.reshape(()), l_con.reshape(())]).float()
-        return losses, grad, (dict(probs=probs, seeds=seeds, logq=logq, refined=refined) if want_blobs else None)
+        blobs = dict(probs=probs, seeds=seeds, logq=logq, refined=refined) if want_blobs else None
+        return (losses, grad, blobs, losses.sum()) if want_total else (losses, grad, blobs)
     ctx = ctx or get_context(B, C, H, W)
-    losses = torch.empty(2, dtype=torch.float32, device=logits.device)
+    out3 = torch.empty(3, dtype=torch.float32, device=logits.device)
+    losses = out3[:2]
     grad = torch.empty_like(logits)
     blobs = None
     if want_blobs:
         blobs = dict(probs=torch.empty_like(logits), seeds=torch.empty_like(logits), logq=torch.empty_like(logits))
     prm = CrfParams.from_crf_args(maxiter, scale_factor)
-    check(_lib.lib().dsrg_supervision_step(
+    check(_lib.lib().dsrg_supervision_step_total(
         ctx._h, B, _ptr(logits), None if prepared else _ptr(images), images.shape[2], images.shape[3],
         _ptr(labels), _ptr(cues),
-        float(th1), float(th2), ctypes.byref(prm), _ptr(losses), _ptr(grad),
+        float(th1), float(th2), ctypes.byref(prm), _ptr(losses), _ptr(out3[2]) if want_total else None, _ptr(grad),
         _ptr(blobs["probs"]) if blobs else None, _ptr(blobs["seeds"]) if blobs else None,
         _ptr(blobs["logq"]) if blobs else None, _stream()))
-    return losses, grad, blobs
+    return (losses, grad, blobs, out3[2]) if want_total else (losses, grad, blobs)
 
 
 def im2col3x3_nhwc(x_nhwc, dilation):
@@ -789,19 +791,23 @@
     if n == 0:
         return
     ptr = lambda ts: np.array([0 if t is None else t.data_ptr() for t in ts], dtype=np.uint64)
-    fwd, dg, shape, entries = [None] * n, [None] * n, np.zeros((n, 4), dtype=np.int32), []
+    fwd, dg, cast, shape, entries = [None] * n, [None] * n, [None] * n, np.zeros((n, 4), dtype=np.int32), []
     for i, p in enumerate(params):
         e = _weight_packs.get(p.data_ptr())
         if e is None or e.ref() is None or e.ref().data_ptr() != p.data_ptr() or e.ref().shape != p.shape:
             continue
-        fwd[i], dg[i] = e.fwd, e.dg
-        shape[i] = (p.shape[0], p.shape[1], p.shape[2] * p.shape[3], e.plain)
+        if e.plain == _PLAIN_CAST:
+            cast[i] = e.fwd
+        else:
+            fwd[i], dg[i] = e.fwd, e.dg
+            shape[i] = (p.shape[0], p.shape[1], p.shape[2] * p.shape[3], e.plain)
         entries.append((e, p))
-    pp, gp, bp, fp, dp = ptr(params), ptr(grads), ptr(bufs), ptr(fwd), ptr(dg)
+    pp, gp, bp, fp, dp, cp = ptr(params), ptr(grads), ptr(bufs), ptr(fwd), ptr(dg), ptr(cast)
     numel = np.array([p.numel() for p in params], dtype=np.int64)
     lr, wd = np.asarray(lrs, dtype=np.float32), np.asarray(wds, dtype=np.float32)
     a = lambda x: x.ctypes.data
-    check(_lib.lib().dsrg_sgd_pack_f32(n, a(pp), a(gp), a(bp), a(fp), a(dp), a(shape), a(numel), a(lr), a(wd), float(momentum), _stream()))
+    check(_lib.lib().dsrg_sgd_pack_cast_f32(n, a(pp), a(gp), a(bp), a(fp), a(dp), a(cp), a(shape), a(numel), a(lr), a(wd),
+                                            float(momentum), _stream()))
     torch.autograd.graph.increment_version(list(params))
     for e, p in entries:
         e.version = p._version
@@ -812,6 +818,23 @@
         g.shape == p.shape and all(n == 1 or (sg == sp and sb == sp) for n, sp, sg, sb in zip(p.shape, p.stride(), g.stride(), b.stride())) and \
         (p.is_contiguous() or (p.dim() == 4 and p.is_contiguous(memory_format=torch.channels_last))) and \
         ((p.data_ptr() | b.data_ptr()) % 16 == 0 or p.data_ptr() not in _weight_packs)
+
+
+_PLAIN_CAST = 2
+
+
+def cast_weight_kept(weight):
+    w = weight.detach()
+    dense = w.is_contiguous() or (w.dim() == 4 and w.is_contiguous(memory_format=torch.channels_last))
+    if not (_packs_kept(weight) and w.dtype == torch.float32 and dense):
+        return w.to(torch.bfloat16)
+    e = _packs_entry(weight, _PLAIN_CAST)
+    if e is not None and e.version == weight._version and e.fwd is not None:
+        _check_kept_packs(weight, e.fwd, None, lambda f, d: f.copy_(w))
+        return e.fwd
+    w16 = w.to(torch.bfloat16)
+    _packs_keep(weight, _PLAIN_CAST, w16, None)
+    return w16
 
 
 def pack_direct_weight_pair(weight, want_dgrad=True):
@@ -1155,6 +1178,91 @@
     return ([gx[k].permute(0, 3, 1, 2) for k in range(n)] if need_gx else None), gw
 
 
+def _vp4(ts):
+    return (ctypes.c_void_p * 4)(*([t.data_ptr() for t in ts] + [None] * (4 - len(ts))))
+
+
+def heads_kernels_in_place(weights, biases=None):
+    if not 1 <= len(weights) <= 4 or weights[0].dim() < 2:
+        return False
+    O, K = weights[0].shape[0], weights[0].shape[1]
+    if not all(w.is_cuda and w.dtype == torch.float32 and w.shape == weights[0].shape and w.numel() == O * K and w.is_contiguous()
+               for w in weights):
+        return False
+    return biases is None or (len(biases) == len(weights) and all(
+        b.is_cuda and b.dtype == torch.float32 and tuple(b.shape) == (O,) and b.is_contiguous() for b in biases))
+
+
+def heads_forward_ptrs(xs, weights, biases):
+    B, K, H, W = xs[0].shape
+    n, O = len(weights), weights[0].shape[0]
+    cl = torch.channels_last
+    xs = [x.contiguous(memory_format=cl) for x in xs]
+    if not all(x.is_cuda and x.dtype == torch.bfloat16 and x.shape == xs[0].shape for x in xs) or len(xs) != n:
+        raise ValueError("heads_forward_ptrs needs n bf16 CUDA activations of one shape")
+    if not heads_kernels_in_place(weights, biases) or weights[0].shape[1] != K:
+        raise ValueError("heads_forward_ptrs needs n float32 CUDA kernels whose memory is (O,K) row-major, and (O) biases")
+    out = torch.empty((B, O, H, W), dtype=torch.float32, device=xs[0].device)
+    check(_lib.lib().dsrg_heads_forward_ptrs_bf16(_vp4(xs), n, _vp4(weights), _vp4(biases) if biases is not None else None, _ptr(out),
+                                                  B, H * W, K, O, _stream()))
+    return out
+
+
+def heads_backward_ptrs(xs, weights, g, need_gx=True, relu_scale=0.0, gw_outs=None):
+    B, K, H, W = xs[0].shape
+    n, O = len(weights), weights[0].shape[0]
+    cl = torch.channels_last
+    xs = [x.contiguous(memory_format=cl) for x in xs]
+    if not heads_kernels_in_place(weights) or weights[0].shape[1] != K:
+        raise ValueError("heads_backward_ptrs needs n float32 CUDA kernels whose memory is (O,K) row-major")
+    g = g.contiguous()
+    _f32c(g, "g")
+    L = _lib.lib()
+    M = B * H * W
+    gx = torch.empty((n, B, H, W, K), dtype=torch.bfloat16, device=g.device) if need_gx else None
+    gws = []
+    for k, w in enumerate(weights):
+        out = gw_outs[k] if gw_outs is not None else None
+        if out is not None and out.dtype == torch.float32 and out.shape == w.shape and out.device == w.device and out.is_contiguous():
+            gws.append(out)
+        else:
+            gws.append(torch.empty_strided(tuple(w.shape), tuple(w.stride()), dtype=torch.float32, device=g.device))
+    part = torch.empty(L.dsrg_heads_backward_chunks(M) * n * O * K, dtype=torch.float32, device=g.device)
+    masked = relu_scale > 0.0 and need_gx
+    gb = _bias_grad_dest(None, (n, K), g.device) if masked else None
+    ws = _reduction_scratch(g.device, L.dsrg_heads_backward_relu_workspace(n, M, K)) if masked else None
+    check(L.dsrg_heads_backward_ptrs_bf16(_vp4(xs), n, _vp4(weights), _ptr(g), _ptr(gx), M * K * 2, _vp4(gws), _ptr(part),
+                                          float(relu_scale) if masked else 0.0, _ptr(gb), _ptr(ws), ws.numel() if masked else 0,
+                                          B, H * W, K, O, _stream()))
+    gxs = [gx[k].permute(0, 3, 1, 2) for k in range(n)] if need_gx else None
+    return (gxs, gws, gb) if masked else (gxs, gws)
+
+
+def image_to_bf16_nhwc(x):
+    if not (x.dim() == 4 and x.shape[1] == 3):
+        raise ValueError("image_to_bf16_nhwc needs a (B,3,H,W) image")
+    _f32c(x, "x")
+    B, _, H, W = x.shape
+    y = torch.empty((B, 3, H, W), dtype=torch.bfloat16, device=x.device, memory_format=torch.channels_last)
+    check(_lib.lib().dsrg_image_nchw_to_nhwc_bf16(_ptr(x), _ptr(y), B, H, W, _stream()))
+    return y
+
+
+def image_takes_fused_cast(x):
+    return x.is_cuda and x.dtype == torch.float32 and x.dim() == 4 and x.shape[1] == 3 and x.is_contiguous() and x.numel() > 0
+
+
+def sum_bf16(ts):
+    t0 = ts[0]
+    if not (2 <= len(ts) <= 4 and all(t.is_cuda and t.dtype == torch.bfloat16 and t.shape == t0.shape and t.stride() == t0.stride()
+                                      for t in ts) and t0.numel() % 8 == 0 and t0.numel() > 0 and
+            (t0.is_contiguous() or (t0.dim() == 4 and t0.is_contiguous(memory_format=torch.channels_last)))):
+        raise ValueError("sum_bf16 needs 2..4 dense bf16 CUDA tensors of one shape and layout, 8 | elements")
+    out = torch.empty_like(t0)
+    check(_lib.lib().dsrg_sum_bf16(_vp4(ts), len(ts), _ptr(out), t0.numel(), _stream()))
+    return out
+
+
 def maxpool3x3_out_size(n, stride, ceil_mode):
     num = n + 2 - 3
     o = (-(-num // stride) if ceil_mode else num // stride) + 1
@@ -1232,16 +1340,17 @@
 
     @staticmethod
     def forward(ctx, logits, images, labels, cues, th1, th2, scale_factor, maxiter, prepared=False):
-        losses, grad, _ = supervision_step(logits.contiguous(), images, labels, cues, th1, th2, scale_factor, maxiter,
-                                           prepared=prepared)
+        losses, grad, _, total = supervision_step(logits.contiguous(), images, labels, cues, th1, th2, scale_factor, maxiter,
+                                                  prepared=prepared, want_total=True)
         ctx.save_for_backward(grad)
         ctx.mark_non_differentiable(losses)
-        return losses.sum(), losses
+        ctx.set_materialize_grads(False)
+        return total, losses
 
     @staticmethod
     def backward(ctx, g_total, _g_losses):
         (grad,) = ctx.saved_tensors
-        return grad * g_total, None, None, None, None, None, None, None, None
+        return (grad * g_total if g_total is not None else None), None, None, None, None, None, None, None, None
 
 
 def dsrg_supervision_loss(logits, images, labels, cues, th1=0.99, th2=0.85, scale_factor=12.0, maxiter=10,
diff --git a/dsrg_amd/trainer.py b/dsrg_amd/trainer.py
--- a/dsrg_amd/trainer.py
+++ b/dsrg_amd/trainer.py
@@ -177,7 +177,11 @@
             self.reducer.prepare()
         else:
             self.opt.zero_grad()
-        x = images.contiguous(memory_format=torch.channels_last) if self.channels_last else images
+        from .ops import image_takes_fused_cast, image_to_bf16_nhwc
+        if self.channels_last and self.amp_dtype == torch.bfloat16 and isinstance(self.net, VGG16ASPP) and image_takes_fused_cast(images):
+            x = image_to_bf16_nhwc(images)
+        else:
+            x = images.contiguous(memory_format=torch.channels_last) if self.channels_last else images
         if self.overlap_build:
             from .ops import crf_prepare
             main = torch.cuda.current_stream()
diff --git a/include/dsrg_hip.h b/include/dsrg_hip.h
--- a/include/dsrg_hip.h
+++ b/include/dsrg_hip.h
@@ -222,6 +222,23 @@
                           double th1, double th2, const dsrg_crf_params *params,
                           float *losses_dev, float *grad_logits_dev,
                           float *probs_dev, float *seeds_dev, float *logq_dev, void *stream);
+int dsrg_supervision_step_total(dsrg_ctx_t ctx, int B, const float *logits_dev, const float *images_dev,
+                                int img_h, int img_w, const float *labels_dev, const float *cues_dev,
+                                double th1, double th2, const dsrg_crf_params *params,
+                                float *losses_dev, float *total_dev, float *grad_logits_dev,
+                                float *probs_dev, float *seeds_dev, float *logq_dev, void *stream);
+
+int dsrg_heads_forward_ptrs_bf16(const void *const *x_dev, int n_branches, const float *const *w_dev, const float *const *bias_dev,
+                                 float *out_dev, int B, int HW, int K, int O, void *stream);
+int dsrg_heads_backward_ptrs_bf16(const void *const *x_dev, int n_branches, const float *const *w_dev, const float *g_dev,
+                                  void *gx_dev, size_t gx_branch_stride_bytes, float *const *gw_dev, float *partial_dev,
+                                  float relu_scale, float *bias_grad_dev, void *workspace_dev, size_t workspace_bytes, int B,
+                                  int HW, int K, int O, void *stream);
+int dsrg_image_nchw_to_nhwc_bf16(const float *x_dev, void *y_dev, int B, int H, int W, void *stream);
+int dsrg_sum_bf16(const void *const *g_dev, int n, void *out_dev, size_t numel, void *stream);
+int dsrg_sgd_pack_cast_f32(int n, float *const *param_dev, const float *const *grad_dev, float *const *momentum_dev,
+                           void *const *fwd_dev, void *const *dgrad_dev, void *const *cast_dev, const int *shape,
+                           const long long *numel, const float *lr, const float *weight_decay, float momentum, void *stream);
 
 #pragma GCC visibility pop
 
```

After: 2041 (median of 6 runs). +1.1%, better.
